# maxsonate/video-diffusion-nnx

Hardware: AMD Instinct MI355X
Metric: denoised frames/sec, 16fx64x64 1000-step DDPM (higher is better)
Workload: dtype bf16; 1 GPU; config_v2_2 (north-star shape): Unet3D dim=64 C=1, 16f x 64x64, DDPM T=1000 p_sample_loop (UNet forward + p_sample per step, hipGraph replay); value = n_gpus*B*F/(T*s_per_step); batch_per_gpu=64, parallelism=dp1 (independent samples, no collective), mfma_operands=bf16, storage=weights fp32 master, activations bf16, fp32 accumulate, process_group=none (single process)

## Files before the change

include/vdx.h:

```cpp
#ifndef VDX_H_
#define VDX_H_

#include <stddef.h>
#include <stdint.h>

#ifdef __cplusplus
extern "C" {
#endif

typedef enum {
    VDX_OK = 0,
    VDX_ERR_INVALID = -1,
    VDX_ERR_HIP = -2,
    VDX_ERR_NOMEM = -3,
    VDX_ERR_STATE = -4
} vdx_status;

typedef enum { VDX_MODE_F32 = 0, VDX_MODE_BF16 = 1, VDX_MODE_F16 = 2 } vdx_mode;

const char* vdx_last_error(void);
int vdx_version(void);


size_t vdx_packed_conv_bytes(int mode, int taps, int cin, int cout);
int vdx_pack_conv_weights(int mode, const float* kernel, void* packed, int taps, int cin, int cout, void* stream);

size_t vdx_gn_stats_bytes(int batch, int groups);

typedef struct {
    const float* x0; const float* x1; int c0, c1;
    const void* packed_w;
    const float* bias;
    float* y;
    int cout;
    int batch, frames, h, w;
    int kind;
    int kh, kw, stride;
    const double* in_stats; const float* gamma; const float* beta; int groups;
    const float* scale_shift; int scale_shift_stride;
    double* out_stats; int out_groups;
    int x_bf16;
    int y_bf16;
    const void* res; int res_bf16;
} vdx_conv_desc;

int vdx_conv_forward(int mode, const vdx_conv_desc* d, void* stream);

typedef struct {
    const char* kernel;
    const char* shape;
    double flops, bytes;
} vdx_launch_info;
typedef void (*vdx_launch_hook)(void* user, int phase, const vdx_launch_info* info, void* stream);
void vdx_set_launch_hook(vdx_launch_hook hook, void* user);

int vdx_resblock_tail(const float* y2, const float* r, float* out, const double* stats, const float* gn_gamma,
                      const float* gn_beta, int groups, const float* ln_gamma, const float* ln_beta, int c, int batch,
                      long pix_per_sample, void* stream);

int vdx_resblock_tail_rc_bf16(const void* y2, const void* x0, const void* x1, int c0, int c1, const void* rc_w_packed,
                              const float* rc_bias, void* out, const double* stats, const float* gn_gamma, const float* gn_beta,
                              int groups, const float* ln_gamma, const float* ln_beta, int c, int batch, long pix_per_sample,
                              void* stream);

int vdx_gn_silu_apply_bf16(void* y, const double* stats, const float* gn_gamma, const float* gn_beta, const float* scale_shift,
                           int ss_stride, int groups, int c, int batch, long pix_per_sample, void* stream);

int vdx_init_conv(const float* x, const float* kernel, const float* bias, float* y, int batch, int cin, int frames,
                  int h, int w, int cout, int k, void* stream);

int vdx_final_conv(const float* x, const float* kernel, const float* bias, float* y, long npix, int d, int cout, void* stream);

int vdx_time_mlp(const int* time, const float* w1, const float* b1, const float* w2, const float* b2, int dim,
                 const float* cond, const float* null_cond_emb, const unsigned char* cond_mask, int null_all, int cond_dim,
                 float* temb, int batch, void* stream);

int vdx_attention_forward(int mode, const float* x, float* y, const void* wqkv_packed, const float* bqkv,
                          const void* wo_packed, const float* bo, int batch, int frames, int h, int w, int c, int heads,
                          int temporal, void* stream);
int vdx_attention_forward_ex(int mode, const float* x, float* y, const void* wqkv_packed, const float* bqkv,
                             const void* wo_packed, const float* bo, int batch, int frames, int h, int w, int c, int heads,
                             int temporal, int fp8_core, void* stream);

int vdx_attention_forward_bf16(const void* x_bf16, void* y_bf16, const void* wqkv_packed, const float* bqkv,
                               const void* wo_packed, const float* bo, int batch, int frames, int h, int w, int c, int heads,
                               int temporal, int fp8_core, void* stream);

size_t vdx_sla_workspace_bytes(int mode, int nframes, int npix, int heads);
int vdx_sla_forward(int mode, const float* x, float* y, const void* wq_packed, const void* wk_packed, const void* wv_packed,
                    const void* wo_packed, void* workspace, int batch, int frames, int h, int w, int c, int heads, void* stream);

int vdx_sla_forward_bf16(const void* x_bf16, void* y_bf16, const void* wq_packed, const void* wk_packed, const void* wv_packed,
                         const void* wo_packed, void* workspace, int batch, int frames, int h, int w, int c, int heads, void* stream);


typedef struct {
    int dim;
    int n_mults; int dim_mults[8];
    int channels;
    int out_dim;
    int cond_dim;
    int attn_heads, attn_dim_head;
    int init_dim;
    int init_kernel_size;
    int use_sparse_linear_attn;
    int resnet_groups;
    int image_size, num_frames;
    int mode;
} vdx_config;

typedef struct vdx_handle vdx_handle;

int vdx_create(const vdx_config* cfg, vdx_handle** out);
void vdx_destroy(vdx_handle* h);

int vdx_set_activation_storage(vdx_handle* h, int bf16);
int vdx_get_activation_storage(const vdx_handle* h);

int vdx_set_attention_fp8(vdx_handle* h, int on);
int vdx_get_attention_fp8(const vdx_handle* h);

int vdx_param_count(const vdx_handle* h);
long vdx_param_total(const vdx_handle* h);
int vdx_param_info(const vdx_handle* h, int index, char* name, int name_cap, int* ndim, long shape[6], long* offset);

size_t vdx_packed_bytes(const vdx_handle* h);
int vdx_pack_params(const vdx_handle* h, const float* params, void* packed, void* stream);

size_t vdx_workspace_bytes(const vdx_handle* h, int batch);
int vdx_slot_count(const vdx_handle* h);
int vdx_slot_info(const vdx_handle* h, int index, char* name, int name_cap, long* floats_per_sample, long* float_offset_per_sample);

int vdx_unet_forward(const vdx_handle* h, const float* params, const void* packed, const float* x, const int* time,
                     const float* cond, const unsigned char* cond_mask, int null_all, float* out, void* workspace,
                     size_t workspace_bytes, int batch, void* stream);


int vdx_randn(float* out, long n, uint64_t seed, uint64_t offset, const uint64_t* dev_offset, void* stream);

int vdx_q_sample(const float* x_start, const int* t, const float* noise, float* out, const float* sqrt_ac,
                 const float* sqrt_one_minus_ac, int batch, long per_sample, float pre_scale, float pre_shift, void* stream);

int vdx_p_sample_step(const float* x, const float* eps_hat, float* out, const int* t, const float* tables, int timesteps,
                      const float* noise, uint64_t seed, uint64_t offset, const uint64_t* dev_offset, const float* thres,
                      int clip_denoised, int batch, int channels, long per_sample, void* stream);

int vdx_loss_sum(const float* eps_hat, const float* noise, double* acc, int batch, int channels, long fhw, int l2, void* stream);

int vdx_affine(const float* x, float* y, long n, float a, float b, void* stream);

int vdx_p_sample_loop(vdx_handle* h, const float* params, const void* packed, float* img, float* eps_buf, int* t_dev,
                      uint64_t* step_dev, const float* tables, int timesteps, int nsteps, const float* cond, uint64_t seed,
                      int clip_denoised, void* workspace, size_t workspace_bytes, int batch, int use_graph, void* stream);

int vdx_dynamic_threshold(const float* x, const float* eps_hat, const int* t, const float* tables, int timesteps, float percentile,
                          float* thres_out, int batch, int channels, long per_sample, void* stream);

int vdx_p_sample_loop_dyn(vdx_handle* h, const float* params, const void* packed, float* img, float* eps_buf, int* t_dev,
                          uint64_t* step_dev, const float* tables, int timesteps, int nsteps, const float* cond, uint64_t seed,
                          int clip_denoised, float percentile, float* thres_buf, void* workspace, size_t workspace_bytes, int batch,
                          int use_graph, void* stream);

int vdx_ddim_step(const float* x, const float* eps_hat, float* out, const float* alphas_cumprod, const int* seq,
                  const uint64_t* step_dev, const float* thres, int clip_denoised, int batch, int channels, long per_sample, void* stream);

int vdx_ddim_sample_loop(vdx_handle* h, const float* params, const void* packed, float* img, float* eps_buf, int* t_dev,
                         uint64_t* step_dev, const float* alphas_cumprod, const int* seq, int seq_len, int nsteps, const float* cond,
                         int clip_denoised, void* workspace, size_t workspace_bytes, int batch, int use_graph, void* stream);

int vdx_ddim_sample_loop_dyn(vdx_handle* h, const float* params, const void* packed, float* img, float* eps_buf, int* t_dev,
                             uint64_t* step_dev, const float* alphas_cumprod, const int* seq, int seq_len, int nsteps, const float* cond,
                             int clip_denoised, const float* tables, int timesteps, float percentile, float* thres_buf, void* workspace,
                             size_t workspace_bytes, int batch, int use_graph, void* stream);

#define VDX_DRAW_KNOWN (1ull << 62)
#define VDX_DRAW_RENOISE (1ull << 63)

int vdx_inpaint_init(float* x, const float* known, const unsigned char* mask, const float* mask_tables, int timesteps, int t0,
                     long n, void* stream);

int vdx_p_sample_step_masked(const float* x, const float* eps_hat, float* out, const int* t, const float* tables, int timesteps,
                             const float* known, const unsigned char* mask, const float* mask_tables, int resample_steps,
                             uint64_t seed, uint64_t step, const uint64_t* step_dev, const float* thres, int clip_denoised,
                             int batch, int channels, long per_sample, void* stream);

int vdx_p_sample_loop_masked(vdx_handle* h, const float* params, const void* packed, float* img, float* eps_buf, int* t_dev,
                             uint64_t* step_dev, const float* tables, int timesteps, int nsteps, const float* cond, uint64_t seed,
                             int clip_denoised, float percentile, float* thres_buf, const float* known, const unsigned char* mask,
                             const float* mask_tables, int resample_steps, void* workspace, size_t workspace_bytes, int batch,
                             int use_graph, void* stream);

int vdx_ddim_step_masked(const float* x, const float* eps_hat, float* out, const float* alphas_cumprod, const int* seq,
                         const uint64_t* step_dev, const float* thres, int clip_denoised, const float* known, const unsigned char* mask,
                         const float* mask_tables, int timesteps, uint64_t seed, int batch, int channels, long per_sample, void* stream);

int vdx_ddim_sample_loop_masked(vdx_handle* h, const float* params, const void* packed, float* img, float* eps_buf, int* t_dev,
                                uint64_t* step_dev, const float* alphas_cumprod, const int* seq, int seq_len, int nsteps, const float* cond,
                                int clip_denoised, const float* tables, int timesteps, float percentile, float* thres_buf,
                                const float* known, const unsigned char* mask, const float* mask_tables, uint64_t seed,
                                void* workspace, size_t workspace_bytes, int batch, int use_graph, void* stream);


int vdx_pack_conv_weights_t(int mode, const float* kernel, void* packed, int taps, int cin, int cout, void* stream);

typedef struct {
    const float* x0; const float* x1; int c0, c1;
    const float* dy; int cout;
    float* dw;
    int batch, frames, h, w;
    int kind, kh, kw, stride;
    const double* in_stats; const float* gamma; const float* beta; int groups;
    const float* scale_shift; int scale_shift_stride;
    int bf16_operands;
} vdx_wgrad_desc;

int vdx_conv_backward_weights(const vdx_wgrad_desc* d, void* stream);

size_t vdx_norm_act_backward_scratch_floats(int c, int batch, long pix_per_sample);
int vdx_norm_act_backward(const float* dact, const float* y, float* dy, const double* stats, const float* gamma, const float* beta,
                          int groups, const float* scale_shift, int scale_shift_stride, float* d_gamma, float* d_beta, float* dss,
                          const float* r, const float* ln_gamma, float* dr, float* d_ln_gamma, float* d_ln_beta, float* scratch,
                          int c, int batch, long pix_per_sample, void* stream);

int vdx_attention_core_backward(const float* qkv, const float* d_o, float* o, float* dq, float* dk, float* dv, int batch, int frames,
                                int h, int w, int heads, int temporal, void* stream);
int vdx_attention_core_backward_ex(const float* qkv, const float* d_o, float* o, float* dq, float* dk, float* dv, int batch, int frames,
                                   int h, int w, int heads, int temporal, int bf16_operands, void* stream);

int vdx_temporal_attention_backward_fused(const float* x, const float* dy, const void* packed_wqkv, const float* bqkv, const void* packed_wo_t,
                                          void* o_bf16, void* dqkv_bf16, float* dx, int batch, int frames, int h, int w, void* stream);

size_t vdx_sla_backward_scratch_floats(int nframes, int heads);
int vdx_sla_core_backward(const float* q, const float* k, const float* v, const float* d_out, float* o, float* dq, float* dk, float* dv,
                          float* scratch, int nframes, int npix, int heads, void* stream);
int vdx_sla_core_backward_ex(const float* q, const float* k, const float* v, const float* d_out, float* o, float* dq, float* dk, float* dv,
                             float* scratch, int nframes, int npix, int heads, int bf16_operands, void* stream);

int vdx_colsum(const float* x, float* out, long rows, int c, void* stream);


typedef struct {
    const void* x0; const void* x1; int c0, c1; int x_bf16;
    const void* dy; int cout; int dy_bf16;
    float* dw; float* dw1; float* dw2; int split;
    float* db; float* db1; float* db2;
    int batch, frames, h, w;
    int kind, kh, kw, stride;
// ... 65 lines not shown
```

video_diffusion_nnx_amd/_lib.py:

```python
from __future__ import annotations

import ctypes as C
import os

_HERE = os.path.dirname(os.path.abspath(__file__))
LIB_PATH = os.environ.get('VDX_LIB') or os.path.join(_HERE, 'libvdx.so')

MODE_F32 = 0
MODE_BF16 = 1
MODE_F16 = 2
MODES = {'f32': MODE_F32, 'fp32': MODE_F32, 'float32': MODE_F32, 'bf16': MODE_BF16, 'bfloat16': MODE_BF16,
         'f16': MODE_F16, 'fp16': MODE_F16, 'float16': MODE_F16}
GN_SLOTS = 32


class VdxError(RuntimeError):
    pass


if not os.path.exists(LIB_PATH):
    raise ImportError(
        f'{LIB_PATH} not found: the HIP extension is required (no CPU fallback exists). '
        'Build it with `python -c "import __graft_entry__ as g; g.build()"` or `make -C video_diffusion_nnx_amd/csrc`.')

lib = C.CDLL(LIB_PATH)

c_void_p, c_int, c_size_t, c_float, c_double = C.c_void_p, C.c_int, C.c_size_t, C.c_float, C.c_double


class ConvDesc(C.Structure):
    _fields_ = [
        ('x0', c_void_p), ('x1', c_void_p), ('c0', c_int), ('c1', c_int),
        ('packed_w', c_void_p), ('bias', c_void_p), ('y', c_void_p), ('cout', c_int),
        ('batch', c_int), ('frames', c_int), ('h', c_int), ('w', c_int),
        ('kind', c_int), ('kh', c_int), ('kw', c_int), ('stride', c_int),
        ('in_stats', c_void_p), ('gamma', c_void_p), ('beta', c_void_p), ('groups', c_int),
        ('scale_shift', c_void_p), ('scale_shift_stride', c_int),
        ('out_stats', c_void_p), ('out_groups', c_int),
        ('x_bf16', c_int), ('y_bf16', c_int),
        ('res', c_void_p), ('res_bf16', c_int),
    ]


def _sig(name, restype, argtypes):
    fn = getattr(lib, name)
    fn.restype = restype
    fn.argtypes = argtypes
    return fn


vdx_last_error = _sig('vdx_last_error', C.c_char_p, [])
vdx_version = _sig('vdx_version', c_int, [])
vdx_packed_conv_bytes = _sig('vdx_packed_conv_bytes', c_size_t, [c_int, c_int, c_int, c_int])
vdx_pack_conv_weights = _sig('vdx_pack_conv_weights', c_int, [c_int, c_void_p, c_void_p, c_int, c_int, c_int, c_void_p])
vdx_gn_stats_bytes = _sig('vdx_gn_stats_bytes', c_size_t, [c_int, c_int])
vdx_conv_forward = _sig('vdx_conv_forward', c_int, [c_int, C.POINTER(ConvDesc), c_void_p])


def check(status: int) -> None:
    if status != 0:
        raise VdxError(f'libvdx status {status}: {vdx_last_error().decode()}')


def ptr(t) -> int:
    if t is None:
        return 0
    assert t.is_contiguous(), 'libvdx needs contiguous tensors'
    return t.data_ptr()


def stream_ptr() -> int:
    import torch
    return torch.cuda.current_stream().cuda_stream

c_long = C.c_long
vdx_resblock_tail = _sig('vdx_resblock_tail', c_int, [c_void_p] * 6 + [c_int, c_void_p, c_void_p, c_int, c_int, c_long, c_void_p])
vdx_gn_silu_apply_bf16 = _sig('vdx_gn_silu_apply_bf16', c_int, [c_void_p] * 5 + [c_int, c_int, c_int, c_int, c_long, c_void_p])
vdx_resblock_tail_rc_bf16 = _sig('vdx_resblock_tail_rc_bf16', c_int, [c_void_p] * 3 + [c_int, c_int] + [c_void_p] * 6 + [c_int, c_void_p, c_void_p, c_int, c_int, c_long, c_void_p])
vdx_init_conv = _sig('vdx_init_conv', c_int, [c_void_p] * 4 + [c_int] * 7 + [c_void_p])
vdx_final_conv = _sig('vdx_final_conv', c_int, [c_void_p] * 4 + [c_long, c_int, c_int, c_void_p])
vdx_time_mlp = _sig('vdx_time_mlp', c_int, [c_void_p] * 5 + [c_int, c_void_p, c_void_p, c_void_p, c_int, c_int, c_void_p, c_int, c_void_p])
vdx_attention_forward = _sig('vdx_attention_forward', c_int, [c_int] + [c_void_p] * 6 + [c_int] * 7 + [c_void_p])
vdx_attention_forward_ex = _sig('vdx_attention_forward_ex', c_int, [c_int] + [c_void_p] * 6 + [c_int] * 8 + [c_void_p])
vdx_attention_forward_bf16 = _sig('vdx_attention_forward_bf16', c_int, [c_void_p] * 6 + [c_int] * 8 + [c_void_p])
vdx_sla_forward_bf16 = _sig('vdx_sla_forward_bf16', c_int, [c_void_p] * 7 + [c_int] * 6 + [c_void_p])
vdx_sla_workspace_bytes = _sig('vdx_sla_workspace_bytes', c_size_t, [c_int] * 4)
vdx_sla_forward = _sig('vdx_sla_forward', c_int, [c_int] + [c_void_p] * 7 + [c_int] * 6 + [c_void_p])
```

video_diffusion_nnx_amd/csrc/elementwise.hip:

```cpp
#include "vdx_common.h"
#include <stdlib.h>
#include "vdx_internal.h"

namespace vdx {

template <int VPL>
__global__ __launch_bounds__(256) void resblock_tail_kernel(TailArgs P) {
    __shared__ float coefA[1024], coefD[1024];
    __shared__ float gm[64];
    const int tid = threadIdx.x;
    const int C = P.C;
    const int b = blockIdx.y;
    gn_mean_rstd_wg(P.stats, b, P.groups, (double)P.pix_per_sample * (C / P.groups), gm, tid, 256);
    __syncthreads();
    for (int c = tid; c < C; c += 256) {
        const int g = c / (C / P.groups);
        const float a = gm[2 * g + 1] * P.gn_gamma[c];
        coefA[c] = a;
        coefD[c] = P.gn_beta[c] - gm[2 * g] * a;
    }
    __syncthreads();
    const int LPP = P.lpp;
    const int ppb = 256 / LPP;
    const int sub = tid % LPP, pl = tid / LPP;
    const float invC = 1.0f / (float)C;
    for (long pix = (long)blockIdx.x * ppb + pl; pix < P.pix_per_sample; pix += (long)gridDim.x * ppb) {
        const size_t base = ((size_t)b * P.pix_per_sample + pix) * C;
        float4 r[VPL];
        float s = 0.f, ss = 0.f;
#pragma unroll
        for (int v = 0; v < VPL; ++v) {
            const int c = (v * LPP + sub) * 4;
            r[v] = make_float4(0.f, 0.f, 0.f, 0.f);
            if (c < C) {
                r[v] = load4_f32_or_bf16(P.r, base + c, P.r_bf16);
                s += r[v].x + r[v].y + r[v].z + r[v].w;
                ss += r[v].x * r[v].x + r[v].y * r[v].y + r[v].z * r[v].z + r[v].w * r[v].w;
            }
        }
        for (int o = 1; o < LPP; o <<= 1) { s += __shfl_xor(s, o); ss += __shfl_xor(ss, o); }
        const float mean = s * invC;
        const float var = fmaxf(ss * invC - mean * mean, 0.f);
        const float rstd = rsqrtf(var + NORM_EPS);
#pragma unroll
        for (int v = 0; v < VPL; ++v) {
            const int c = (v * LPP + sub) * 4;
            if (c < C) {
                const float4 y = load4_f32_or_bf16(P.y2, base + c, P.y2_bf16);
                const float4 a = *reinterpret_cast<const float4*>(coefA + c);
                const float4 d = *reinterpret_cast<const float4*>(coefD + c);
                const float4 lg = *reinterpret_cast<const float4*>(P.ln_gamma + c);
                const float4 lb = *reinterpret_cast<const float4*>(P.ln_beta + c);
                float4 o;
                o.x = silu_f(fmaf(y.x, a.x, d.x)) + fmaf((r[v].x - mean) * rstd, lg.x, lb.x);
                o.y = silu_f(fmaf(y.y, a.y, d.y)) + fmaf((r[v].y - mean) * rstd, lg.y, lb.y);
                o.z = silu_f(fmaf(y.z, a.z, d.z)) + fmaf((r[v].z - mean) * rstd, lg.z, lb.z);
                o.w = silu_f(fmaf(y.w, a.w, d.w)) + fmaf((r[v].w - mean) * rstd, lg.w, lb.w);
                store4_f32_or_bf16(P.out, base + c, o, P.out_bf16);
            }
        }
    }
}

__device__ __forceinline__ void unpack8(const uint4& u, float (&f)[8]) {
    f[0] = __uint_as_float(u.x << 16); f[1] = __uint_as_float(u.x & 0xFFFF0000u);
    f[2] = __uint_as_float(u.y << 16); f[3] = __uint_as_float(u.y & 0xFFFF0000u);
    f[4] = __uint_as_float(u.z << 16); f[5] = __uint_as_float(u.z & 0xFFFF0000u);
    f[6] = __uint_as_float(u.w << 16); f[7] = __uint_as_float(u.w & 0xFFFF0000u);
}

template <int VPL>
__global__ __launch_bounds__(256) void resblock_tail16_kernel(TailArgs P) {
    __shared__ float coefA[1024], coefD[1024];
    __shared__ float gm[64];
    const int tid = threadIdx.x;
    const int C = P.C;
    const int b = blockIdx.y;
    gn_mean_rstd_wg(P.stats, b, P.groups, (double)P.pix_per_sample * (C / P.groups), gm, tid, 256);
    __syncthreads();
    for (int c = tid; c < C; c += 256) {
        const int g = c / (C / P.groups);
        const float a = gm[2 * g + 1] * P.gn_gamma[c];
        coefA[c] = a;
        coefD[c] = P.gn_beta[c] - gm[2 * g] * a;
    }
    __syncthreads();
    const int LPP = P.lpp;
    const int ppb = 256 / LPP;
    const int sub = tid % LPP, pl = tid / LPP;
    const float invC = 1.0f / (float)C;
    const char* rb = reinterpret_cast<const char*>(P.r);
    const char* yb = reinterpret_cast<const char*>(P.y2);
    char* ob = reinterpret_cast<char*>(P.out);
    for (long pix = (long)blockIdx.x * ppb + pl; pix < P.pix_per_sample; pix += (long)gridDim.x * ppb) {
        const size_t base = ((size_t)b * P.pix_per_sample + pix) * C;
        float r[VPL][8];
        float s = 0.f, ss = 0.f;
#pragma unroll
        for (int v = 0; v < VPL; ++v) {
            const int c = (v * LPP + sub) * 8;
#pragma unroll
            for (int k = 0; k < 8; ++k) r[v][k] = 0.f;
            if (c < C) {
                unpack8(*reinterpret_cast<const uint4*>(rb + (base + c) * 2), r[v]);
#pragma unroll
                for (int k = 0; k < 8; ++k) { s += r[v][k]; ss += r[v][k] * r[v][k]; }
            }
        }
        for (int o = 1; o < LPP; o <<= 1) { s += __shfl_xor(s, o); ss += __shfl_xor(ss, o); }
        const float mean = s * invC;
        const float var = fmaxf(ss * invC - mean * mean, 0.f);
        const float rstd = rsqrtf(var + NORM_EPS);
#pragma unroll
        for (int v = 0; v < VPL; ++v) {
            const int c = (v * LPP + sub) * 8;
            if (c < C) {
                float y[8], o[8];
                unpack8(*reinterpret_cast<const uint4*>(yb + (base + c) * 2), y);
#pragma unroll
                for (int k = 0; k < 8; ++k)
                    o[k] = silu_f(fmaf(y[k], coefA[c + k], coefD[c + k])) + fmaf((r[v][k] - mean) * rstd, P.ln_gamma[c + k], P.ln_beta[c + k]);
                *reinterpret_cast<uint4*>(ob + (base + c) * 2) =
                    make_uint4(pack_bf16x2(o[0], o[1]), pack_bf16x2(o[2], o[3]), pack_bf16x2(o[4], o[5]), pack_bf16x2(o[6], o[7]));
            }
        }
    }
}

__global__ __launch_bounds__(256) void gn_silu_apply16_kernel(unsigned* __restrict__ y, const double* __restrict__ stats, const float* __restrict__ gamma,
                                                              const float* __restrict__ beta, const float* __restrict__ ss, int ss_stride, int groups,
                                                              int C, long pix_per_sample) {
    __shared__ float coefA[1024], coefD[1024];
    __shared__ float gm[64];
    const int tid = threadIdx.x, b = blockIdx.y;
    gn_mean_rstd_wg(stats, b, groups, (double)pix_per_sample * (C / groups), gm, tid, 256);
    __syncthreads();
    for (int c = tid; c < C; c += 256) {
        const int g = c / (C / groups);
        const float m = gm[2 * g], rs = gm[2 * g + 1];
        const float ga = gamma[c], be = beta[c];
        float sc = 1.f, sh = 0.f;
        if (ss) { sc = ss[(size_t)b * ss_stride + c] + 1.f; sh = ss[(size_t)b * ss_stride + C + c]; }
        coefA[c] = rs * ga * sc;
        coefD[c] = (be - m * rs * ga) * sc + sh;
    }
    __syncthreads();
    const int octs = C >> 3;
    const long n = pix_per_sample * octs;
    uint4* base = reinterpret_cast<uint4*>(y) + (size_t)b * n;
    for (long i0 = (long)blockIdx.x * 1024 + tid; i0 < n; i0 += (long)gridDim.x * 1024) {
        uint4 v[4];
#pragma unroll
        for (int u = 0; u < 4; ++u) v[u] = (i0 + u * 256 < n) ? base[i0 + u * 256] : make_uint4(0u, 0u, 0u, 0u);
#pragma unroll
        for (int u = 0; u < 4; ++u) {
            if (i0 + u * 256 >= n) continue;
            const int c = (int)((i0 + u * 256) % octs) * 8;
            float f[8], o[8];
            unpack8(v[u], f);
#pragma unroll
            for (int k = 0; k < 8; ++k) o[k] = silu_f(fmaf(f[k], coefA[c + k], coefD[c + k]));
            base[i0 + u * 256] = make_uint4(pack_bf16x2(o[0], o[1]), pack_bf16x2(o[2], o[3]), pack_bf16x2(o[4], o[5]), pack_bf16x2(o[6], o[7]));
        }
    }
}

hipError_t launch_gn_silu_apply16(float* y_bf16, const double* stats, const float* gamma, const float* beta, const float* ss, int ss_stride, int groups,
                                  int C, int batch, long pix_per_sample, hipStream_t st) {
    if (C % 8 || C > 1024 || groups <= 0 || groups > 32 || C % groups) return hipErrorInvalidValue;
    const long n = pix_per_sample * (C / 8);
    const int gx = (int)std::max<long>(1, std::min<long>((n + 1023) / 1024, 2048));
    LaunchScope ls(st, "gn_silu_apply16_kernel", 8.0 * batch * pix_per_sample * C, 4.0 * batch * pix_per_sample * C, "C%d px%ld x %d", C, pix_per_sample, batch);
    hipLaunchKernelGGL(gn_silu_apply16_kernel, dim3(gx, batch), dim3(256), 0, st, reinterpret_cast<unsigned*>(y_bf16), stats, gamma, beta, ss, ss_stride, groups, C, pix_per_sample);
    return hipGetLastError();
}

typedef unsigned tu32x4 __attribute__((ext_vector_type(4)));

template <int CIN, int COUT, bool CAT, bool FIN = false>
__global__ __launch_bounds__(256, (CIN == 128 && COUT == 64) ? 4 : (COUT <= 128 ? 3 : 2)) void resblock_tail_rc16_kernel(TailArgs P) {
    using M = Mma<MODE_BF16>;
    constexpr int NTM = COUT / 16, NKS = CIN / 32, NH = COUT / 32;
    constexpr int C0 = CAT ? CIN / 2 : CIN, NK0 = C0 / 32;
    constexpr int WRS = CIN * 2 + 16;
    extern __shared__ __attribute__((aligned(16))) char smem[];
    char* Wl = smem;
    float* coefA = reinterpret_cast<float*>(Wl + COUT * WRS);
    float* coefD = coefA + COUT;
    float* lng = coefD + COUT;
    float* lnb = lng + COUT;
    float* rcb = lnb + COUT;
    float* gm = rcb + COUT;
    float* finw = gm + 64;
    const int tid = threadIdx.x, lane = tid & 63, wave = tid >> 6, lp = lane & 15, q = lane >> 4;
    const int b = blockIdx.y;
    for (int i = tid; i < COUT * (CIN / 8); i += 256) {
        const int row = i / (CIN / 8), c = i % (CIN / 8);
        const int tm = row >> 4, rr = row & 15;
        const int co = (tm >> 1) * 32 + (rr >> 2) * 8 + (tm & 1) * 4 + (rr & 3);
        *reinterpret_cast<uint4*>(Wl + row * WRS + c * 16) =
            *reinterpret_cast<const uint4*>(reinterpret_cast<const char*>(P.rc_w) + ((size_t)co * ((CIN + 63) / 64 * 64) + c * 8) * 2);
    }
    gn_mean_rstd_wg(P.stats, b, P.groups, (double)P.pix_per_sample * (COUT / P.groups), gm, tid, 256);
    __syncthreads();
    for (int c = tid; c < COUT; c += 256) {
        const int g = c / (COUT / P.groups);
        const float a = gm[2 * g + 1] * P.gn_gamma[c];
        coefA[c] = a;
        coefD[c] = P.gn_beta[c] - gm[2 * g] * a;
        lng[c] = P.ln_gamma[c]; lnb[c] = P.ln_beta[c]; rcb[c] = P.rc_b[c];
        if (FIN) finw[c] = P.fin_w[c];
    }
    __syncthreads();

    const unsigned pps = (unsigned)P.pix_per_sample;
    const char* x0p = reinterpret_cast<const char*>(P.x0) + (size_t)b * pps * C0 * 2;
    const char* x1p = CAT ? reinterpret_cast<const char*>(P.x1) + (size_t)b * pps * C0 * 2 : x0p;
    const char* y2p = reinterpret_cast<const char*>(P.y2) + (size_t)b * pps * COUT * 2;
    char* outp = FIN ? const_cast<char*>(y2p) : reinterpret_cast<char*>(P.out) + (size_t)b * pps * COUT * 2;
    float* const finp = FIN ? P.fin_out + (size_t)b * pps : nullptr;
    const float finb = FIN ? P.fin_b[0] : 0.f;
    const __amdgpu_buffer_rsrc_t rx0 = __builtin_amdgcn_make_buffer_rsrc(const_cast<char*>(x0p), 0, pps * C0 * 2, 0x00020000);
// ... 571 lines not shown
```

video_diffusion_nnx_amd/csrc/model.hip:

```cpp
#include <math.h>
#include <stdio.h>
#include <string.h>
#include <string>
#include <vector>

#include "vdx_common.h"
#include "vdx_internal.h"
#include "model.h"
#include <stdlib.h>

namespace vdx {

static long add_param(Model* m, const std::string& name, std::initializer_list<long> shape) {
    ParamInfo p;
    p.name = name;
    p.ndim = (int)shape.size();
    long n = 1;
    int i = 0;
    for (long s : shape) { p.shape[i++] = s; n *= s; }
    p.offset = m->param_total;
    p.numel = n;
    m->param_total += (n + 3) / 4 * 4;
    m->params.push_back(p);
    return p.offset;
// ... 163 lines not shown
            L.pk_rs = add_packed(m, conv_packed_bytes(m->mode, 16, dims[i + 1], dims[i + 1]));
            L.pt_rs = add_packed_t(m, conv_packed_bytes(m->mode, 16, dims[i + 1], dims[i + 1]));
        }
    }
    const int mid = dims[nl];
    m->mid1 = make_res(m, "mid_block1", mid, mid, true);
    m->mid_sattn = make_attn(m, "mid_spatial_attn", mid);
    m->mid_tattn = make_attn(m, "mid_temporal_attn", mid);
    m->mid2 = make_res(m, "mid_block2", mid, mid, true);
    for (int i = 0; i < nl; ++i) {
        Level& L = m->ups[i];
        const std::string pre = "ups." + std::to_string(i);
        const int din = dims[nl - 1 - i], dout = dims[nl - i];
        L.cin = 2 * dout; L.cout = din;
        L.res0 = make_res(m, pre + ".0", 2 * dout, din, true);
        L.res1 = make_res(m, pre + ".1", din, din, true);
        L.has_sla = c.use_sparse_linear_attn != 0;
        if (L.has_sla) L.sla = make_sla(m, pre + ".2", din);
        L.attn = make_attn(m, pre + ".3", din);
        L.has_resample = i < nl - 1;
        if (L.has_resample) {
            L.rs_w = add_param(m, pre + ".4.kernel", {1, 4, 4, din, din});
            L.rs_b = add_param(m, pre + ".4.bias", {din});
            L.pk_rs = add_packed(m, conv_packed_bytes(m->mode, 16, din, din));
            L.pt_rs = add_packed_t(m, conv_packed_bytes(m->mode, 16, din, din));
        }
    }
    m->fin = make_res(m, "final_conv.layers.0", 2 * c.dim, c.dim, false);
    m->fin_w = add_param(m, "final_conv.layers.1.kernel", {1, c.dim, m->out_dim});
    m->fin_b = add_param(m, "final_conv.layers.1.bias", {m->out_dim});
    if (m->init_dim != c.dim) return vdx_set_error(VDX_ERR_INVALID, "config: init_dim must equal dim (the final concat feeds ResnetBlock(2*dim))", __FILE__, __LINE__);

    const long F = c.num_frames;
    auto pixels = [&](int lvl) { const long s = c.image_size >> lvl; return F * s * s; };
    m->s_init = add_slot(m, "init_conv", pixels(0) * m->init_dim);
    m->s_init_attn = add_slot(m, "init_temporal_attn", pixels(0) * m->init_dim);
    for (int i = 0; i < nl; ++i) {
        Level& L = m->downs[i];
        L.lvl = i;
        res_slots(m, L.res0, pixels(i));
        res_slots(m, L.res1, pixels(i));
        L.s_sla = L.has_sla ? add_slot(m, "downs." + std::to_string(i) + ".2", pixels(i) * L.cout) : -1;
        L.s_attn = add_slot(m, "downs." + std::to_string(i) + ".3", pixels(i) * L.cout);
        L.s_rs = L.has_resample ? add_slot(m, "downs." + std::to_string(i) + ".4", pixels(i + 1) * L.cout) : -1;
    }
    res_slots(m, m->mid1, pixels(nl - 1));
    m->s_mid_sattn = add_slot(m, "mid_spatial_attn", pixels(nl - 1) * mid);
    m->s_mid_tattn = add_slot(m, "mid_temporal_attn", pixels(nl - 1) * mid);
    res_slots(m, m->mid2, pixels(nl - 1));
    for (int i = 0; i < nl; ++i) {
        Level& L = m->ups[i];
        L.lvl = nl - 1 - i;
        res_slots(m, L.res0, pixels(L.lvl));
        res_slots(m, L.res1, pixels(L.lvl));
        L.s_sla = L.has_sla ? add_slot(m, "ups." + std::to_string(i) + ".2", pixels(L.lvl) * L.cout) : -1;
        L.s_attn = add_slot(m, "ups." + std::to_string(i) + ".3", pixels(L.lvl) * L.cout);
        L.s_rs = L.has_resample ? add_slot(m, "ups." + std::to_string(i) + ".4", pixels(L.lvl - 1) * L.cout) : -1;
    }
    res_slots(m, m->fin, pixels(0));
    m->sla_ws_bytes_per_sample = 0;
    for (int l = 0; l < nl; ++l) {
        const long s = c.image_size >> l;
        if (c.use_sparse_linear_attn)
            m->sla_ws_bytes_per_sample = std::max(m->sla_ws_bytes_per_sample, sla_workspace_bytes(m->mode, (int)F, (int)(s * s), H));
        if (c.dim * c.dim_mults[l] >= 256)
            m->sla_ws_bytes_per_sample = std::max(m->sla_ws_bytes_per_sample, (size_t)F * s * s * c.attn_heads * 32 * 2);
    }
    {
        const long s = c.image_size >> (nl - 1);
        if (s * s > 64) m->sla_ws_bytes_per_sample = std::max(m->sla_ws_bytes_per_sample, (size_t)F * s * s * c.attn_heads * 32 * 4 * 4);
    }
    return VDX_OK;
}

size_t model_workspace_bytes(const Model* m, int B) {
    size_t b = 0;
    b += ((size_t)m->act_floats_per_sample * B * 4 + 255) / 256 * 256;
    b += ((size_t)m->temb_dim * B * 4 + 255) / 256 * 256;
    b += 2 * (((size_t)m->ss_floats_per_sample * B * 4 + 255) / 256 * 256);
    b += ((size_t)m->n_stats * B * GN_SLOTS * m->cfg.resnet_groups * 2 * 8 + 255) / 256 * 256;
    b += (m->sla_ws_bytes_per_sample * B + 255) / 256 * 256;
    return b;
}


void model_build_pack_tables(Model* m) {
    const int HD = m->cfg.attn_heads * 32;
    auto pad = [&](int k) { return conv_cin_pad(m->mode, k); };
    auto fwd = [&](long src, size_t dst, int taps, int cin, int cout) {
        PackJob j{}; j.src = src; j.dst = (long)dst; j.taps = taps; j.Cin = cin; j.Cout = cout; j.Pad = pad(cin); j.kind = 0;
        j.n = (long)taps * cout * j.Pad; m->pack_jobs.push_back(j);
    };
    auto cpy = [&](long src, size_t dst, long n) { PackJob j{}; j.src = src; j.dst = (long)dst; j.n = n; j.kind = 2; j.Pad = 1; m->pack_jobs.push_back(j); };
    auto bwd = [&](long src, size_t dst, int taps, int cin, int cout) {
        PackJob j{}; j.src = src; j.dst = (long)dst; j.taps = taps; j.Cin = cin; j.Cout = cout; j.Pad = pad(cout); j.kind = 1;
        j.n = (long)taps * cin * j.Pad; m->pack_t_jobs.push_back(j);
    };
    auto cat3 = [&](const long (&w)[3], size_t dst, int c) {
        PackJob j{}; j.src = w[0]; j.src1 = w[1]; j.src2 = w[2]; j.dst = (long)dst; j.taps = 1; j.Cin = c; j.Cout = HD; j.Pad = pad(3 * HD); j.kind = 3;
        j.n = (long)c * j.Pad; m->pack_t_jobs.push_back(j);
    };
    auto res = [&](const ResP& r) {
        fwd(r.b1_w, r.pk_b1, 9, r.cin, r.cout); fwd(r.b2_w, r.pk_b2, 9, r.cout, r.cout);
        bwd(r.b1_w, r.pt_b1, 9, r.cin, r.cout); bwd(r.b2_w, r.pt_b2, 9, r.cout, r.cout);
        if (r.has_res) { fwd(r.rc_w, r.pk_rc, 1, r.cin, r.cout); bwd(r.rc_w, r.pt_rc, 1, r.cin, r.cout); }
    };
    auto attn = [&](const AttnP& a) {
        const size_t one = conv_packed_bytes(m->mode, 1, a.C, HD);
        for (int i = 0; i < 3; ++i) {
            fwd(a.w[i], a.pk_qkv + i * one, 1, a.C, HD);
            cpy(a.b[i], a.pk_bqkv + (size_t)i * HD * 4, HD);
            bwd(a.w[i], a.pt_w[i], 1, a.C, HD);
        }
        fwd(a.o_w, a.pk_o, 1, HD, a.C); bwd(a.o_w, a.pt_o, 1, HD, a.C);
        cat3(a.w, a.pt_qkv, a.C);
    };
    auto sla = [&](const SlaP& s) {
        for (int i = 0; i < 3; ++i) { fwd(s.w[i], s.pk[i], 1, s.C, HD); bwd(s.w[i], s.pt_w[i], 1, s.C, HD); }
        fwd(s.o_w, s.pk_o, 1, HD, s.C); bwd(s.o_w, s.pt_o, 1, HD, s.C);
        cat3(s.w, s.pt_qkv, s.C);
    };
    m->pack_jobs.clear(); m->pack_t_jobs.clear();
    attn(m->init_attn);
    for (int pass = 0; pass < 2; ++pass) {
        const std::vector<Level>& lv = pass ? m->ups : m->downs;
        for (const Level& L : lv) {
            res(L.res0); res(L.res1);
            if (L.has_sla) sla(L.sla);
            attn(L.attn);
            if (L.has_resample) { fwd(L.rs_w, L.pk_rs, 16, L.cout, L.cout); bwd(L.rs_w, L.pt_rs, 16, L.cout, L.cout); }
        }
    }
    res(m->mid1); attn(m->mid_sattn); attn(m->mid_tattn); res(m->mid2); res(m->fin);
}

hipError_t model_pack(const Model* m, const float* p, void* packed, hipStream_t st) {
    if (!m->d_pack_jobs) return hipErrorInvalidValue;
    return launch_pack_jobs(m->mode, p, packed, m->d_pack_jobs, (int)m->pack_jobs.size(), st);
}


struct Fwd {
    const Model* m; const float* p; const char* pk; int B; hipStream_t st;
    int a16;
    float* act; float* temb; float* ss; float* ss_lin; double* stats; char* sla_ws;
    float* slot(int s) const { return act + (size_t)m->slots[s].offset_per_sample * B; }
    double* stat(int i) const { return stats + (size_t)i * B * GN_SLOTS * m->cfg.resnet_groups * 2; }
};

#ifndef VDX_PREPASS_MIN_C
#define VDX_PREPASS_MIN_C 256
#endif

static hipError_t run_res(const Fwd& f, const ResP& r, const float* x0, int c0, const float* x1, int c1, int lvl, float* head_out = nullptr, bool* head_done = nullptr) {
    const Model* m = f.m;
    const int G = m->cfg.resnet_groups;
    const int S = m->cfg.image_size >> lvl;
    ConvArgs a;
    memset(&a, 0, sizeof(a));
    a.x0 = x0; a.x1 = x1; a.C0 = c0; a.C1 = c1;
    a.wp = f.pk + r.pk_b1; a.bias = f.p + r.b1_b; a.y = f.slot(r.s_y1); a.Cout = r.cout;
    a.NF = f.B * m->cfg.num_frames; a.F = m->cfg.num_frames; a.H = S; a.W = S;
    a.kind = 0; a.kh = a.kw = 3; a.stride = 1; a.pad = 1;
    a.out_stats = f.stat(r.st1); a.out_groups = G;
    const int half = (m->mode == MODE_BF16);
    a.y_bf16 = half; a.x0_bf16 = f.a16; a.x1_bf16 = f.a16;
    hipError_t e = launch_conv(m->mode, a, f.st);
    if (e != hipSuccess) return e;
    ConvArgs b;
    memset(&b, 0, sizeof(b));
    b.x0 = f.slot(r.s_y1); b.C0 = r.cout;
    b.wp = f.pk + r.pk_b2; b.bias = f.p + r.b2_b; b.y = f.slot(r.s_y2); b.Cout = r.cout;
    b.NF = a.NF; b.F = a.F; b.H = S; b.W = S; b.kind = 0; b.kh = b.kw = 3; b.stride = 1; b.pad = 1;
    b.x0_bf16 = half; b.y_bf16 = half;
    b.pro = 1; b.in_stats = f.stat(r.st1); b.gamma = f.p + r.b1_gs; b.beta = f.p + r.b1_gb; b.groups = G;
    if (r.has_mlp) { b.ss = f.ss + (size_t)m->ss_layers[r.ss_index].out_off * f.B; b.ss_stride = 2 * r.cout; }
    b.out_stats = f.stat(r.st2); b.out_groups = G;
    if (half && m->act16 == 1 && r.cout >= VDX_PREPASS_MIN_C) {
        e = launch_gn_silu_apply16(f.slot(r.s_y1), b.in_stats, b.gamma, b.beta, b.ss, b.ss_stride, G, r.cout, f.B, (long)m->cfg.num_frames * S * S, f.st);
        if (e != hipSuccess) return e;
        b.pro = 0; b.in_stats = nullptr; b.gamma = b.beta = nullptr; b.ss = nullptr; b.groups = 0;
    }
    e = launch_conv(m->mode, b, f.st);
    if (e != hipSuccess) return e;
    const float* rsrc = x0;
    const bool fuse_rc = r.has_res && f.a16 && m->act16 == 1 && m->mode == MODE_BF16 &&
                         tail_rc16_supported(c0 + c1, c0, r.cout, (long)m->cfg.num_frames * S * S);
    if (r.has_res && !fuse_rc) {
        ConvArgs c;
        memset(&c, 0, sizeof(c));
        c.x0 = x0; c.x1 = x1; c.C0 = c0; c.C1 = c1;
        c.wp = f.pk + r.pk_rc; c.bias = f.p + r.rc_b; c.y = f.slot(r.s_rc); c.Cout = r.cout;
        c.NF = a.NF; c.F = a.F; c.H = S; c.W = S; c.kind = 0; c.kh = c.kw = 1; c.stride = 1; c.pad = 0;
        c.x0_bf16 = f.a16; c.x1_bf16 = f.a16; c.y_bf16 = f.a16;
        e = launch_conv(m->mode, c, f.st);
        if (e != hipSuccess) return e;
        rsrc = f.slot(r.s_rc);
    }
    TailArgs t;
    memset(&t, 0, sizeof(t));
    t.y2 = f.slot(r.s_y2); t.y2_bf16 = half; t.r = rsrc; t.out = f.slot(r.s_out); t.r_bf16 = f.a16; t.out_bf16 = f.a16;
    t.stats = f.stat(r.st2); t.gn_gamma = f.p + r.b2_gs; t.gn_beta = f.p + r.b2_gb; t.groups = G;
    t.ln_gamma = f.p + r.n2_s; t.ln_beta = f.p + r.n2_b;
    t.C = r.cout; t.batch = f.B; t.pix_per_sample = (long)m->cfg.num_frames * S * S;
    if (fuse_rc) { t.x0 = x0; t.x1 = x1; t.C0 = c0; t.C1 = c1; t.rc_w = f.pk + r.pk_rc; t.rc_b = f.p + r.rc_b; }
    if (head_out && fuse_rc && c1 == c0 && m->out_dim == 1 && ((c0 + c1 == 128 && r.cout == 64) || (c0 + c1 == 64 && r.cout == 32))) {
        t.fin_w = f.p + m->fin_w; t.fin_b = f.p + m->fin_b; t.fin_out = head_out;
        *head_done = true;
    }
    return launch_resblock_tail(t, f.st);
}

static hipError_t run_attn(const Fwd& f, const AttnP& ap, const float* x, float* y, int lvl, bool temporal) {
    const Model* m = f.m;
    const long S = m->cfg.image_size >> lvl, hw = S * S, Fr = m->cfg.num_frames;
    AttnArgs a;
    memset(&a, 0, sizeof(a));
    a.x = x; a.y = y; a.wqkv = f.pk + ap.pk_qkv; a.bqkv = reinterpret_cast<const float*>(f.pk + ap.pk_bqkv);
    a.wo = f.pk + ap.pk_o; a.bo = f.p + ap.o_b; a.C = ap.C; a.heads = m->cfg.attn_heads;
    a.scale = 1.0f / sqrtf((float)m->cfg.attn_dim_head);
    if (temporal) { a.L = (int)Fr; a.nseq = f.B * hw; a.inner = hw; a.inner_stride = ap.C; a.outer_stride = Fr * hw * ap.C; a.tok_stride = hw * ap.C; }
    else { a.L = (int)hw; a.nseq = f.B * Fr; a.inner = 1; a.inner_stride = 0; a.outer_stride = hw * ap.C; a.tok_stride = ap.C; }
    a.io_bf16 = f.a16;
    a.fp8_core = (m->attn_fp8 && m->mode == MODE_BF16) ? 1 : 0;
    if (a.L > 64) {
        if (temporal) return hipErrorInvalidValue;
        const int HD = a.heads * 32;
        float* qkv = reinterpret_cast<float*>(f.sla_ws);
        float* o = qkv + (size_t)f.B * Fr * hw * 3 * HD;
        ConvArgs p;
        memset(&p, 0, sizeof(p));
        p.x0 = x; p.C0 = ap.C; p.x0_bf16 = f.a16; p.wp = f.pk + ap.pk_qkv; p.bias = reinterpret_cast<const float*>(f.pk + ap.pk_bqkv);
        p.y = qkv; p.Cout = 3 * HD;
        p.NF = f.B * (int)Fr; p.F = (int)Fr; p.H = (int)S; p.W = (int)S; p.kind = 0; p.kh = p.kw = 1; p.stride = 1; p.pad = 0;
        hipError_t e = launch_conv(m->mode, p, f.st);
        if (e != hipSuccess) return e;
        e = launch_attention_long_core(qkv, o, a.nseq, a.L, a.heads, a.scale, f.st);
        if (e != hipSuccess) return e;
        ConvArgs c;
        memset(&c, 0, sizeof(c));
        c.x0 = o; c.C0 = HD; c.wp = f.pk + ap.pk_o; c.bias = f.p + ap.o_b; c.y = y; c.Cout = ap.C; c.y_bf16 = f.a16;
        c.res = x; c.res_bf16 = f.a16;
        c.NF = f.B * (int)Fr; c.F = (int)Fr; c.H = (int)S; c.W = (int)S; c.kind = 0; c.kh = c.kw = 1; c.stride = 1; c.pad = 0;
        return launch_conv(m->mode, c, f.st);
    }
    if (m->mode == MODE_BF16 && (temporal ? a.L <= 16 : a.L <= 64) && a.heads == 8 && ap.C >= 256 && ap.C % 128 == 0 &&
        (size_t)96 * (ap.C * 2 + 32) <= 160 * 1024 && (size_t)Fr * S * S * a.heads * 64 <= m->sla_ws_bytes_per_sample) {
        a.oscratch = f.sla_ws;
        hipError_t e = launch_attention_heads(a, f.st);
        if (e != hipSuccess) return e;
        ConvArgs c;
        memset(&c, 0, sizeof(c));
        c.x0 = reinterpret_cast<const float*>(f.sla_ws); c.C0 = a.heads * 32; c.x0_bf16 = 1;
        c.wp = f.pk + ap.pk_o; c.bias = f.p + ap.o_b; c.y = y; c.Cout = ap.C; c.y_bf16 = f.a16;
        c.res = x; c.res_bf16 = f.a16;
        c.NF = f.B * (int)Fr; c.F = (int)Fr; c.H = (int)S; c.W = (int)S; c.kind = 0; c.kh = c.kw = 1; c.stride = 1; c.pad = 0;
        return launch_conv(m->mode, c, f.st);
    }
    return launch_attention(m->mode, a, f.st);
}

static hipError_t run_sla(const Fwd& f, const SlaP& sp, const float* x, float* y, int lvl) {
    const Model* m = f.m;
    const int S = m->cfg.image_size >> lvl;
    SlaArgs a;
    memset(&a, 0, sizeof(a));
    a.x = x; a.y = y; a.wq = f.pk + sp.pk[0]; a.wk = f.pk + sp.pk[1]; a.wv = f.pk + sp.pk[2]; a.wo = f.pk + sp.pk_o;
    a.workspace = f.sla_ws; a.C = sp.C; a.heads = m->cfg.attn_heads; a.NF = f.B * m->cfg.num_frames; a.N = S * S;
    a.io_bf16 = f.a16;
    if (m->mode == MODE_BF16 && a.heads == 8 && sp.C >= 256 && sp.C % 128 == 0 && a.N % 16 == 0 &&
        (size_t)96 * (sp.C * 2 + 32) <= 160 * 1024 && (size_t)m->cfg.num_frames * a.N * a.heads * 64 <= m->sla_ws_bytes_per_sample) {
        hipError_t e = launch_sla_heads(a, f.sla_ws, f.st);
        if (e != hipSuccess) return e;
        ConvArgs c;
        memset(&c, 0, sizeof(c));
        c.x0 = reinterpret_cast<const float*>(f.sla_ws); c.C0 = a.heads * 32; c.x0_bf16 = 1;
        c.wp = f.pk + sp.pk_o; c.y = y; c.Cout = sp.C; c.y_bf16 = f.a16;
        c.res = x; c.res_bf16 = f.a16;
        c.NF = a.NF; c.F = m->cfg.num_frames; c.H = S; c.W = S; c.kind = 0; c.kh = c.kw = 1; c.stride = 1; c.pad = 0;
        return launch_conv(m->mode, c, f.st);
    }
    return launch_sla(m->mode, a, f.st);
}

static hipError_t run_resample(const Fwd& f, const Level& L, const float* x, float* y, int lvl_in, bool up) {
    const Model* m = f.m;
    const int S = m->cfg.image_size >> lvl_in;
    ConvArgs a;
    memset(&a, 0, sizeof(a));
    a.x0 = x; a.C0 = L.cout; a.wp = f.pk + L.pk_rs; a.bias = f.p + L.rs_b; a.y = y; a.Cout = L.cout;
    a.NF = f.B * m->cfg.num_frames; a.F = m->cfg.num_frames; a.H = S; a.W = S;
    if (up) { a.kind = 1; a.kh = a.kw = 4; a.stride = 1; a.pad = 0; }
    else { a.kind = 0; a.kh = a.kw = 4; a.stride = 2; a.pad = 1; }
    a.x0_bf16 = f.a16; a.y_bf16 = f.a16;
    return launch_conv(m->mode, a, f.st);
}

int model_forward(const Model* m, const float* params, const void* packed, const float* x, const int* time,
                  const float* cond, const unsigned char* cond_mask, int null_all, float* out, void* workspace,
                  size_t workspace_bytes, int B, hipStream_t st) {
    if (B < 1) return vdx_set_error(VDX_ERR_INVALID, "forward: batch < 1", __FILE__, __LINE__);
    if (workspace_bytes < model_workspace_bytes(m, B)) return vdx_set_error(VDX_ERR_NOMEM, "forward: workspace too small", __FILE__, __LINE__);
    if (m->cfg.cond_dim && !cond) return vdx_set_error(VDX_ERR_INVALID, "cond must be passed in if cond_dim specified", __FILE__, __LINE__);
    const vdx_config& c = m->cfg;
    Fwd f;
    f.m = m; f.p = params; f.pk = reinterpret_cast<const char*>(packed); f.B = B; f.st = st;
    f.a16 = (m->act16 && m->mode == MODE_BF16) ? 1 : 0;
    char* w = reinterpret_cast<char*>(workspace);
    f.act = reinterpret_cast<float*>(w); w += ((size_t)m->act_floats_per_sample * B * 4 + 255) / 256 * 256;
    f.temb = reinterpret_cast<float*>(w); w += ((size_t)m->temb_dim * B * 4 + 255) / 256 * 256;
    f.ss = reinterpret_cast<float*>(w); w += ((size_t)m->ss_floats_per_sample * B * 4 + 255) / 256 * 256;
    f.ss_lin = reinterpret_cast<float*>(w); w += ((size_t)m->ss_floats_per_sample * B * 4 + 255) / 256 * 256;
    f.stats = reinterpret_cast<double*>(w);
    const size_t stats_bytes = (size_t)m->n_stats * B * GN_SLOTS * c.resnet_groups * 2 * 8;
    w += (stats_bytes + 255) / 256 * 256;
    f.sla_ws = w;
    hipError_t e;
#define VDX_E(x) do { e = (x); if (e != hipSuccess) return vdx_set_error(VDX_ERR_HIP, hipGetErrorString(e), __FILE__, __LINE__); } while (0)
    {
        LaunchScope ls(st, "fillBufferAligned", 0.0, (double)stats_bytes, "GroupNorm statistics slabs %zu B", stats_bytes);
        VDX_E(hipMemsetAsync(f.stats, 0, stats_bytes, st));
    }
    const int S0 = c.image_size, Fr = c.num_frames;
    {
        TimeMlpArgs t;
        memset(&t, 0, sizeof(t));
        t.time = time; t.w1 = params + m->t_w1; t.b1 = params + m->t_b1; t.w2 = params + m->t_w2; t.b2 = params + m->t_b2;
        t.dim = c.dim; t.time_dim = m->time_dim; t.cond = cond; t.null_cond_emb = c.cond_dim ? params + m->null_cond : nullptr;
        t.cond_mask = cond_mask; t.null_all = null_all; t.cond_dim = c.cond_dim; t.temb = f.temb; t.temb_dim = m->temb_dim;
        VDX_E(launch_time_mlp(t, B, st));
        int max_n = 0;
        for (const SsLayer& l : m->ss_layers) max_n = std::max(max_n, l.n);
        VDX_E(launch_resblock_ss(params, f.temb, m->d_ss_layers, (int)m->ss_layers.size(), f.ss, f.ss_lin, m->temb_dim, B, max_n, st));
    }
    VDX_E(launch_init_conv_mode(m->mode, x, params + m->init_w, params + m->init_b, f.slot(m->s_init), B, c.channels, Fr, S0, S0, m->init_dim, c.init_kernel_size, f.a16, st));
    VDX_E(run_attn(f, m->init_attn, f.slot(m->s_init), f.slot(m->s_init_attn), 0, true));
    const float* cur = f.slot(m->s_init_attn);
    int cur_c = m->init_dim;
    const int nl = c.n_mults;
    for (int i = 0; i < nl; ++i) {
        const Level& L = m->downs[i];
        VDX_E(run_res(f, L.res0, cur, cur_c, nullptr, 0, i));
        VDX_E(run_res(f, L.res1, f.slot(L.res0.s_out), L.cout, nullptr, 0, i));
        cur = f.slot(L.res1.s_out);
        if (L.has_sla) { VDX_E(run_sla(f, L.sla, cur, f.slot(L.s_sla), i)); cur = f.slot(L.s_sla); }
        VDX_E(run_attn(f, L.attn, cur, f.slot(L.s_attn), i, true));
        cur = f.slot(L.s_attn); cur_c = L.cout;
        if (L.has_resample) { VDX_E(run_resample(f, L, cur, f.slot(L.s_rs), i, false)); cur = f.slot(L.s_rs); }
    }
    VDX_E(run_res(f, m->mid1, cur, cur_c, nullptr, 0, nl - 1));
    VDX_E(run_attn(f, m->mid_sattn, f.slot(m->mid1.s_out), f.slot(m->s_mid_sattn), nl - 1, false));
    VDX_E(run_attn(f, m->mid_tattn, f.slot(m->s_mid_sattn), f.slot(m->s_mid_tattn), nl - 1, true));
    VDX_E(run_res(f, m->mid2, f.slot(m->s_mid_tattn), cur_c, nullptr, 0, nl - 1));
    cur = f.slot(m->mid2.s_out);
    for (int i = 0; i < nl; ++i) {
        const Level& L = m->ups[i];
        const Level& D = m->downs[nl - 1 - i];
        VDX_E(run_res(f, L.res0, cur, cur_c, f.slot(D.s_attn), D.cout, L.lvl));
        VDX_E(run_res(f, L.res1, f.slot(L.res0.s_out), L.cout, nullptr, 0, L.lvl));
        cur = f.slot(L.res1.s_out);
        if (L.has_sla) { VDX_E(run_sla(f, L.sla, cur, f.slot(L.s_sla), L.lvl)); cur = f.slot(L.s_sla); }
        VDX_E(run_attn(f, L.attn, cur, f.slot(L.s_attn), L.lvl, true));
        cur = f.slot(L.s_attn); cur_c = L.cout;
        if (L.has_resample) { VDX_E(run_resample(f, L, cur, f.slot(L.s_rs), L.lvl, true)); cur = f.slot(L.s_rs); }
    }
    bool head_done = false;
    VDX_E(run_res(f, m->fin, cur, cur_c, f.slot(m->s_init_attn), m->init_dim, 0, out, &head_done));
    if (!head_done) VDX_E(launch_final_conv(f.slot(m->fin.s_out), params + m->fin_w, params + m->fin_b, out, (long)B * Fr * S0 * S0, c.dim, m->out_dim, f.a16, st));
#undef VDX_E
    return VDX_OK;
}

}
```

video_diffusion_nnx_amd/csrc/sla.hip:

```cpp
#include "vdx_common.h"
#include "vdx_internal.h"
#include <stdlib.h>

namespace vdx {

constexpr int SLA_PART = 32 * 32 + 64;

template <int MODE>
__global__ __launch_bounds__(256) void sla_ctx_kernel(const SlaArgs P) {
    using M = Mma<MODE>;
    constexpr int KT = M::KT, KC = M::KC, RS = ROW_STRIDE;
    constexpr int APIECES = KT / 4;
    constexpr int NCHN = 64 / KC;
    constexpr int RSE = NCHN * 64 + 16;

    extern __shared__ __attribute__((aligned(16))) char smem[];
    float* m_run = reinterpret_cast<float*>(smem);
    float* s_run = m_run + 32;
    float* alpha = s_run + 32;
    float* pm = alpha + 32;
    char* xs = smem + 1024;
    char* ws = xs + 64 * RS;
    char* eT = ws + 64 * RS;
    char* vT = eT + 32 * RSE;

    const int tid = threadIdx.x, lane = tid & 63, w = tid >> 6;
    const int lp = lane & 15, q = lane >> 4;
    const int wc = w & 1, wr = w >> 1;
    const int gsz = 8 * P.heads;
    const int grp = blockIdx.x / gsz, j = blockIdx.x % gsz;
    const int h = j >> 3;
    const int cidx = grp * 8 + (j & 7);
    if (cidx >= P.NF * P.nchunk) return;
    const int n = cidx / P.nchunk, chunk = cidx % P.nchunk;
    const int R = P.nsub * 64;
    const size_t xbase = (size_t)n * P.N * P.C;
    const int nkt = P.CPad / KT;
    const char* wk = reinterpret_cast<const char*>(P.wk);
    const char* wv = reinterpret_cast<const char*>(P.wv);

    if (tid < 32) { m_run[tid] = -1e30f; s_run[tid] = 0.f; }
    f32x4 cacc = f32x4{0.f, 0.f, 0.f, 0.f};
    const int dt = w >> 1, et = w & 1;

    const bool w_resident = (nkt == 1);
    auto stage_w = [&](int kt) {
        for (int i = tid; i < 64 * 8; i += 256) {
            const int row = i >> 3, pc = i & 7;
            const char* src = (row < 32 ? wk : wv) + ((size_t)(h * 32 + (row & 31)) * P.CPad + (size_t)kt * KT) * M::ES + pc * 16;
            *reinterpret_cast<uint4*>(ws + row * RS + pc * 16) = *reinterpret_cast<const uint4*>(src);
        }
    };
    constexpr int XP = 64 * APIECES / 256;
    float4 xpre[XP];
    auto xfetch = [&](int r0, int kt) {
#pragma unroll
        for (int u = 0; u < XP; ++u) {
            const int i = tid + 256 * u;
            const int row = i / APIECES, pc = i % APIECES;
            const int c = kt * KT + pc * 4;
            xpre[u] = make_float4(0.f, 0.f, 0.f, 0.f);
            if (r0 + row < P.N && c < P.C) xpre[u] = load4_f32_or_bf16(P.x, xbase + (size_t)(r0 + row) * P.C + c, P.io_bf16);
        }
    };
    auto xput = [&]() {
#pragma unroll
        for (int u = 0; u < XP; ++u) {
            const int i = tid + 256 * u;
            M::store4(xs + (i / APIECES) * RS, (i % APIECES) * 4, xpre[u]);
        }
    };
    if (w_resident) stage_w(0);
    xfetch(chunk * R, 0);

    for (int sub = 0; sub < P.nsub; ++sub) {
        const int r0 = chunk * R + sub * 64;
        if (r0 >= P.N) break;
        f32x4 acc[2][2];
#pragma unroll
        for (int i = 0; i < 2; ++i) { acc[i][0] = f32x4{0.f, 0.f, 0.f, 0.f}; acc[i][1] = f32x4{0.f, 0.f, 0.f, 0.f}; }
        for (int kt = 0; kt < nkt; ++kt) {
            __syncthreads();
            xput();
            if (!w_resident) stage_w(kt);
            __syncthreads();
            {
                int nk = kt + 1, nr0 = r0;
                if (nk == nkt) { nk = 0; nr0 = r0 + 64; }
                if (nr0 < P.N && nr0 < (chunk + 1) * R) xfetch(nr0, nk);
            }
#pragma unroll
            for (int ch = 0; ch < 2; ++ch) {
                uint4 bf[2], af[2];
#pragma unroll
                for (int tn = 0; tn < 2; ++tn) bf[tn] = *reinterpret_cast<const uint4*>(xs + ((wr * 2 + tn) * 16 + lp) * RS + ch * 64 + q * 16);
#pragma unroll
                for (int tm = 0; tm < 2; ++tm) af[tm] = *reinterpret_cast<const uint4*>(ws + ((wc * 2 + tm) * 16 + lp) * RS + ch * 64 + q * 16);
#pragma unroll
                for (int tm = 0; tm < 2; ++tm)
#pragma unroll
                    for (int tn = 0; tn < 2; ++tn) M::mma(acc[tm][tn], af[tm], bf[tn]);
            }
        }
        bool rv[2];
#pragma unroll
        for (int tn = 0; tn < 2; ++tn) rv[tn] = (r0 + (wr * 2 + tn) * 16 + lp) < P.N;
        if (wc == 0) {
#pragma unroll
            for (int tm = 0; tm < 2; ++tm)
#pragma unroll
                for (int r = 0; r < 4; ++r) {
                    float mx = fmaxf(rv[0] ? acc[tm][0][r] : -1e30f, rv[1] ? acc[tm][1][r] : -1e30f);
                    mx = max16(mx);
                    if (lp == 0) pm[wr * 32 + tm * 16 + 4 * q + r] = mx;
                }
        }
        __syncthreads();
        if (tid < 32) {
            const float mc = fmaxf(pm[tid], pm[32 + tid]);
            const float mo = m_run[tid];
            const float mn = fmaxf(mo, mc);
            alpha[tid] = __expf(mo - mn);
            m_run[tid] = mn;
        }
        __syncthreads();
        if (wc == 0) {
#pragma unroll
            for (int tm = 0; tm < 2; ++tm)
#pragma unroll
                for (int r = 0; r < 4; ++r) {
                    const int d = tm * 16 + 4 * q + r;
                    const float mn = m_run[d];
                    float ssum = 0.f;
#pragma unroll
                    for (int tn = 0; tn < 2; ++tn) {
                        const float e = rv[tn] ? __expf(acc[tm][tn][r] - mn) : 0.f;
                        M::store1(eT + d * RSE, (wr * 2 + tn) * 16 + lp, e);
                        ssum += e;
                    }
                    ssum = reduce16(ssum);
                    if (lp == 0) pm[wr * 32 + d] = ssum;
                }
        } else {
#pragma unroll
            for (int tm = 0; tm < 2; ++tm)
#pragma unroll
                for (int r = 0; r < 4; ++r) {
                    const int e = tm * 16 + 4 * q + r;
#pragma unroll
                    for (int tn = 0; tn < 2; ++tn)
                        M::store1(vT + e * RSE, (wr * 2 + tn) * 16 + lp, rv[tn] ? acc[tm][tn][r] : 0.f);
                }
        }
        __syncthreads();
// ... 45 lines not shown
    }
}

template <int MODE, int TMO>
__global__ __launch_bounds__(256) void sla_out_kernel(const SlaArgs P) {
    using M = Mma<MODE>;
    constexpr int KT = M::KT, KC = M::KC, RS = ROW_STRIDE;
    constexpr int APIECES = KT / 4;
    constexpr int NCHD = 32 / KC;
    constexpr int RSQ = (MODE == MODE_F32) ? 160 : 80;
    constexpr int HD = 256;
    constexpr int RSO = HD * M::ES + 16;
    constexpr int NCHO = HD / KC;

    extern __shared__ __attribute__((aligned(16))) char smem[];
    char* xs = smem;
    char* ws = xs + 64 * RS;
    char* qb = smem;
    char* os = qb + 4 * 64 * RSQ;

    const int tid = threadIdx.x, lane = tid & 63, w = tid >> 6;
    const int lp = lane & 15, q = lane >> 4;
    const int tiles = (P.N + 63) / 64;
    const int n = blockIdx.x / tiles, r0 = (blockIdx.x % tiles) * 64;
    const size_t xbase = (size_t)n * P.N * P.C;
    const int nkt = P.CPad / KT;
    const char* wq = reinterpret_cast<const char*>(P.wq);
    const char* wo = reinterpret_cast<const char*>(P.wo);

    f32x4 acc[4][4];
#pragma unroll
    for (int i = 0; i < 4; ++i)
#pragma unroll
        for (int j = 0; j < 4; ++j) acc[i][j] = f32x4{0.f, 0.f, 0.f, 0.f};
    for (int kt = 0; kt < nkt; ++kt) {
        __syncthreads();
        for (int i = tid; i < 64 * APIECES; i += 256) {
            const int row = i / APIECES, pc = i % APIECES;
            const int c = kt * KT + pc * 4;
            float4 v = make_float4(0.f, 0.f, 0.f, 0.f);
            if (r0 + row < P.N && c < P.C) v = load4_f32_or_bf16(P.x, xbase + (size_t)(r0 + row) * P.C + c, P.io_bf16);
            M::store4(xs + row * RS, pc * 4, v);
        }
        for (int i = tid; i < 256 * 8; i += 256) {
            const int row = i >> 3, pc = i & 7;
            *reinterpret_cast<uint4*>(ws + row * RS + pc * 16) =
                *reinterpret_cast<const uint4*>(wq + ((size_t)row * P.CPad + (size_t)kt * KT) * M::ES + pc * 16);
        }
        __syncthreads();
#pragma unroll
        for (int ch = 0; ch < 2; ++ch) {
            uint4 bf[4], af[4];
#pragma unroll
            for (int tn = 0; tn < 4; ++tn) bf[tn] = *reinterpret_cast<const uint4*>(xs + (tn * 16 + lp) * RS + ch * 64 + q * 16);
#pragma unroll
            for (int tm = 0; tm < 4; ++tm) af[tm] = *reinterpret_cast<const uint4*>(ws + ((w * 4 + tm) * 16 + lp) * RS + ch * 64 + q * 16);
#pragma unroll
            for (int tm = 0; tm < 4; ++tm)
#pragma unroll
                for (int tn = 0; tn < 4; ++tn) M::mma(acc[tm][tn], af[tm], bf[tn]);
        }
    }
    __syncthreads();
    char* myq = qb + w * 64 * RSQ;
#pragma unroll
    for (int hh = 0; hh < 2; ++hh) {
        const int h = 2 * w + hh;
#pragma unroll
        for (int tn = 0; tn < 4; ++tn) {
            float mx = -1e30f;
#pragma unroll
            for (int t2 = 0; t2 < 2; ++t2)
#pragma unroll
                for (int r = 0; r < 4; ++r) mx = fmaxf(mx, acc[2 * hh + t2][tn][r]);
            mx = max_q(mx);
            float e[2][4], sum = 0.f;
#pragma unroll
            for (int t2 = 0; t2 < 2; ++t2)
#pragma unroll
                for (int r = 0; r < 4; ++r) { e[t2][r] = __expf(acc[2 * hh + t2][tn][r] - mx); sum += e[t2][r]; }
            sum = reduce_q(sum);
            const float inv = 1.0f / sum;
#pragma unroll
            for (int t2 = 0; t2 < 2; ++t2)
                M::store4(myq + (tn * 16 + lp) * RSQ, t2 * 16 + 4 * q, make_float4(e[t2][0] * inv, e[t2][1] * inv, e[t2][2] * inv, e[t2][3] * inv));
        }
        __syncthreads();
        const char* ct = reinterpret_cast<const char*>(P.ctxT) + (size_t)(n * P.heads + h) * 32 * 32 * M::ES;
#pragma unroll
        for (int et = 0; et < 2; ++et) {
            f32x4 o[4];
#pragma unroll
            for (int tn = 0; tn < 4; ++tn) o[tn] = f32x4{0.f, 0.f, 0.f, 0.f};
#pragma unroll
            for (int ch = 0; ch < NCHD; ++ch) {
                const uint4 a = *reinterpret_cast<const uint4*>(ct + (size_t)(et * 16 + lp) * 32 * M::ES + ch * 64 + q * 16);
#pragma unroll
                for (int tn = 0; tn < 4; ++tn) {
                    const uint4 bq = *reinterpret_cast<const uint4*>(myq + (tn * 16 + lp) * RSQ + ch * 64 + q * 16);
                    M::mma(o[tn], a, bq);
                }
            }
#pragma unroll
            for (int tn = 0; tn < 4; ++tn)
                M::store4(os + (tn * 16 + lp) * RSO, h * 32 + et * 16 + 4 * q, make_float4(o[tn][0], o[tn][1], o[tn][2], o[tn][3]));
        }
        __syncthreads();
    }
    f32x4 oacc[TMO][4];
#pragma unroll
    for (int i = 0; i < TMO; ++i)
#pragma unroll
        for (int j = 0; j < 4; ++j) oacc[i][j] = f32x4{0.f, 0.f, 0.f, 0.f};
    for (int ch = 0; ch < NCHO; ++ch) {
        uint4 bf[4];
#pragma unroll
        for (int tn = 0; tn < 4; ++tn) bf[tn] = *reinterpret_cast<const uint4*>(os + (tn * 16 + lp) * RSO + ch * 64 + q * 16);
#pragma unroll
        for (int tmo = 0; tmo < TMO; ++tmo) {
            const int co = (w * TMO + tmo) * 16 + lp;
            uint4 a = make_uint4(0, 0, 0, 0);
            if (co < P.C) a = *reinterpret_cast<const uint4*>(wo + (size_t)co * HD * M::ES + ch * 64 + q * 16);
#pragma unroll
            for (int tn = 0; tn < 4; ++tn) M::mma(oacc[tmo][tn], a, bf[tn]);
        }
    }
#pragma unroll
    for (int tmo = 0; tmo < TMO; ++tmo) {
        const int co = (w * TMO + tmo) * 16 + 4 * q;
        if (co >= P.C) continue;
#pragma unroll
        for (int tn = 0; tn < 4; ++tn) {
            const int row = r0 + tn * 16 + lp;
            if (row >= P.N) continue;
            const float4 xr = load4_f32_or_bf16(P.x, xbase + (size_t)row * P.C + co, P.io_bf16);
            float4 v;
            v.x = oacc[tmo][tn][0] + xr.x; v.y = oacc[tmo][tn][1] + xr.y;
            v.z = oacc[tmo][tn][2] + xr.z; v.w = oacc[tmo][tn][3] + xr.w;
            store4_f32_or_bf16(P.y, xbase + (size_t)row * P.C + co, v, P.io_bf16);
        }
    }
}


template <int MODE, int NKT, bool IO16>
struct SlaTile {
    using M = Mma<MODE>;
    static_assert(!IO16 || MODE == MODE_BF16, "bf16 activation storage implies bf16 MFMA operands");
    static constexpr int PCH = IO16 ? 8 : 4;
    static constexpr int APIECES = M::KT / PCH;
    static constexpr int XP = 64 * APIECES * NKT / 512;
    static constexpr int PLANE = 64 * ROW_STRIDE;
    static constexpr int BUF = NKT * PLANE;
    float4 xpre[XP];
    __device__ __forceinline__ void fetch(const float* x, size_t xbase, int io_bf16, int r0, int N, int C, int tid) {
#pragma unroll
        for (int u = 0; u < XP; ++u) {
            const int i = tid + 512 * u;
            const int kt = i / (64 * APIECES), rem = i % (64 * APIECES);
            const int row = rem / APIECES, c = kt * M::KT + (rem % APIECES) * PCH;
            xpre[u] = make_float4(0.f, 0.f, 0.f, 0.f);
            if (r0 + row < N && c < C) {
                if (IO16) xpre[u] = *reinterpret_cast<const float4*>(reinterpret_cast<const char*>(x) + (xbase + (size_t)(r0 + row) * C + c) * 2);
                else xpre[u] = load4_f32_or_bf16(x, xbase + (size_t)(r0 + row) * C + c, io_bf16);
            }
        }
    }
    __device__ __forceinline__ void put(char* xs, int tid) const {
#pragma unroll
        for (int u = 0; u < XP; ++u) {
            const int i = tid + 512 * u;
            const int kt = i / (64 * APIECES), rem = i % (64 * APIECES);
            char* dst = xs + kt * PLANE + (rem / APIECES) * ROW_STRIDE;
            if (IO16) *reinterpret_cast<float4*>(dst + (rem % APIECES) * 16) = xpre[u];
            else M::store4(dst, (rem % APIECES) * 4, xpre[u]);
        }
    }
};

template <bool FULL>
__device__ __forceinline__ void ctx8_softmax_step(f32x4 (&acc)[2][4], float (&m_run)[2], float (&s_run)[2], f32x4 (&cacc)[2][2], int nleft) {
    constexpr float L2E = 1.44269504088896f;
#pragma unroll
    for (int dt = 0; dt < 2; ++dt) {
        if (!FULL) {
#pragma unroll
            for (int tn = 0; tn < 2; ++tn)
#pragma unroll
                for (int r = 0; r < 4; ++r) if (tn * 16 + r >= nleft) acc[tn][dt][r] = -1e30f;
        }
        float mx = fmaxf(fmaxf(fmaxf(acc[0][dt][0], acc[0][dt][1]), fmaxf(acc[0][dt][2], acc[0][dt][3])),
                         fmaxf(fmaxf(acc[1][dt][0], acc[1][dt][1]), fmaxf(acc[1][dt][2], acc[1][dt][3])));
        mx = max_q(mx);
        const float mn = fmaxf(m_run[dt], mx);
        const float alpha = __builtin_amdgcn_exp2f((m_run[dt] - mn) * L2E);
        m_run[dt] = mn;
        const float nb = -mn * L2E;
        float ssum = 0.f;
#pragma unroll
        for (int tn = 0; tn < 2; ++tn)
#pragma unroll
            for (int r = 0; r < 4; ++r) {
                float e = __builtin_amdgcn_exp2f(__builtin_fmaf(acc[tn][dt][r], L2E, nb));
                if (!FULL) e = (tn * 16 + r >= nleft) ? 0.f : e;
                acc[tn][dt][r] = e;
                ssum += e;
            }
        s_run[dt] = s_run[dt] * alpha + reduce_q(ssum);
#pragma unroll
        for (int et = 0; et < 2; ++et)
#pragma unroll
            for (int r = 0; r < 4; ++r) cacc[et][dt][r] *= alpha;
    }
}

template <int MODE, int NKT, bool IO16>
__global__ __launch_bounds__(512) void sla_ctx8_kernel(const SlaArgs P) {
    using M = Mma<MODE>;
    using T = SlaTile<MODE, NKT, IO16>;
    constexpr int RS = ROW_STRIDE;
    extern __shared__ __attribute__((aligned(16))) char smem[];
    const int tid = threadIdx.x, lane = tid & 63, h = tid >> 6;
    const int lp = lane & 15, q = lane >> 4;
    const int n = blockIdx.x / P.nchunk, chunk = blockIdx.x % P.nchunk;
    const int R = P.nsub * 64;
    const size_t xbase = (size_t)n * P.N * P.C;

    uint4 wf[NKT][2][4];
#pragma unroll
    for (int kt = 0; kt < NKT; ++kt)
#pragma unroll
        for (int ch = 0; ch < 2; ++ch)
#pragma unroll
            for (int tm = 0; tm < 4; ++tm) {
                const char* base = reinterpret_cast<const char*>(tm < 2 ? P.wk : P.wv);
                wf[kt][ch][tm] = *reinterpret_cast<const uint4*>(base + ((size_t)(h * 32 + (tm & 1) * 16 + lp) * P.CPad + kt * M::KT) * M::ES + ch * 64 + q * 16);
            }
    float m_run[2] = {-1e30f, -1e30f}, s_run[2] = {0.f, 0.f};
    f32x4 cacc[2][2];
#pragma unroll
    for (int i = 0; i < 2; ++i) { cacc[i][0] = f32x4{0.f, 0.f, 0.f, 0.f}; cacc[i][1] = f32x4{0.f, 0.f, 0.f, 0.f}; }

    T t;
    t.fetch(P.x, xbase, P.io_bf16, chunk * R, P.N, P.C, tid);
    t.put(smem, tid);
    __syncthreads();
    for (int sub = 0; sub < P.nsub; ++sub) {
        const int r0 = chunk * R + sub * 64;
        if (r0 >= P.N) break;
        const char* xs = smem + (sub & 1) * T::BUF;
        const bool more = (sub + 1 < P.nsub) && (r0 + 64 < P.N);
        if (more) t.fetch(P.x, xbase, P.io_bf16, r0 + 64, P.N, P.C, tid);
#pragma unroll
        for (int hf = 0; hf < 2; ++hf) {
            f32x4 acc[2][4];
#pragma unroll
            for (int i = 0; i < 2; ++i)
#pragma unroll
                for (int j = 0; j < 4; ++j) acc[i][j] = f32x4{0.f, 0.f, 0.f, 0.f};
#pragma unroll
            for (int kt = 0; kt < NKT; ++kt)
#pragma unroll
                for (int ch = 0; ch < 2; ++ch) {
                    uint4 xa[2];
#pragma unroll
                    for (int tn = 0; tn < 2; ++tn)
                        xa[tn] = *reinterpret_cast<const uint4*>(xs + kt * T::PLANE + ((hf * 2 + tn) * 16 + lp) * RS + ch * 64 + q * 16);
#pragma unroll
                    for (int tn = 0; tn < 2; ++tn)
#pragma unroll
                        for (int tm = 0; tm < 4; ++tm) M::mma(acc[tn][tm], xa[tn], wf[kt][ch][tm]);
                }
            if (r0 + 64 <= P.N) ctx8_softmax_step<true>(acc, m_run, s_run, cacc, 0);
            else ctx8_softmax_step<false>(acc, m_run, s_run, cacc, P.N - (r0 + hf * 32 + 4 * q));
#pragma unroll
            for (int tn = 0; tn < 2; ++tn)
#pragma unroll
                for (int et = 0; et < 2; ++et)
#pragma unroll
                    for (int dt = 0; dt < 2; ++dt) M::mma16(cacc[et][dt], acc[tn][2 + et], acc[tn][dt]);
        }
        if (more) t.put(smem + ((sub + 1) & 1) * T::BUF, tid);
        __syncthreads();
    }
    if (P.nchunk == 1) {
        char* ct = reinterpret_cast<char*>(P.ctxT) + (size_t)(n * P.heads + h) * 32 * 32 * M::ES;
#pragma unroll
        for (int dt = 0; dt < 2; ++dt) {
            const float inv = 1.0f / s_run[dt];
#pragma unroll
            for (int et = 0; et < 2; ++et)
#pragma unroll
                for (int r = 0; r < 4; ++r) M::store1(ct + (size_t)(et * 16 + 4 * q + r) * 32 * M::ES, dt * 16 + lp, cacc[et][dt][r] * inv);
        }
        return;
    }
    float* part = P.part + ((size_t)(n * P.nchunk + chunk) * P.heads + h) * SLA_PART;
#pragma unroll
    for (int et = 0; et < 2; ++et)
#pragma unroll
        for (int dt = 0; dt < 2; ++dt)
            *reinterpret_cast<float4*>(part + (dt * 16 + lp) * 32 + et * 16 + 4 * q) =
                make_float4(cacc[et][dt][0], cacc[et][dt][1], cacc[et][dt][2], cacc[et][dt][3]);
    if (q == 0) {
#pragma unroll
        for (int dt = 0; dt < 2; ++dt) { part[1024 + dt * 16 + lp] = m_run[dt]; part[1056 + dt * 16 + lp] = s_run[dt]; }
    }
}

template <int MODE, int NKT, int TMO, int TNO, bool IO16>
__global__ __launch_bounds__(512, NKT == 1 ? 4 : 2) void sla_out8_kernel(const SlaArgs P) {
    using M = Mma<MODE>;
    using T = SlaTile<MODE, NKT, IO16>;
    constexpr int RS = ROW_STRIDE, KC = M::KC, HD = 256;
    constexpr int RSO = HD * M::ES + 16;
    constexpr int NCHO = HD / KC;
    constexpr bool WO_RES = (TMO * NCHO <= 16);

    extern __shared__ __attribute__((aligned(16))) char smem[];
    char* os = smem + 2 * T::BUF;
    constexpr int RSY = NKT * M::KT * 4 + 16;
    char* ys = os + 64 * RSO;
    const int tid = threadIdx.x, lane = tid & 63, h = tid >> 6;
    const int lp = lane & 15, q = lane >> 4;
    const int n = blockIdx.x / P.nchunk, chunk = blockIdx.x % P.nchunk;
    const int R = P.nsub * 64;
    const size_t xbase = (size_t)n * P.N * P.C;

    uint4 wqf[NKT][2][2];
#pragma unroll
    for (int kt = 0; kt < NKT; ++kt)
#pragma unroll
        for (int ch = 0; ch < 2; ++ch)
#pragma unroll
            for (int tm = 0; tm < 2; ++tm)
                wqf[kt][ch][tm] = *reinterpret_cast<const uint4*>(reinterpret_cast<const char*>(P.wq) +
                    ((size_t)(h * 32 + tm * 16 + lp) * P.CPad + kt * M::KT) * M::ES + ch * 64 + q * 16);
    f32x4 cf[2][2];
    {
        const char* ct = reinterpret_cast<const char*>(P.ctxT) + (size_t)(n * P.heads + h) * 32 * 32 * M::ES;
#pragma unroll
        for (int et = 0; et < 2; ++et)
#pragma unroll
            for (int dt = 0; dt < 2; ++dt) cf[et][dt] = M::load_w4(ct + ((size_t)(et * 16 + lp) * 32 + dt * 16 + 4 * q) * M::ES);
    }
    const int cot0 = (TNO == 4) ? h * TMO : (TNO == 2) ? (h & 3) : (h & 1);
    const int tn0 = (TNO == 4) ? 0 : (TNO == 2) ? 2 * (h >> 2) : (h >> 1);
    const char* wo = reinterpret_cast<const char*>(P.wo);
    uint4 wof[WO_RES ? TMO : 1][WO_RES ? NCHO : 1];
    if (WO_RES) {
#pragma unroll
        for (int tmo = 0; tmo < TMO; ++tmo)
#pragma unroll
            for (int ch = 0; ch < NCHO; ++ch)
                wof[tmo][ch] = *reinterpret_cast<const uint4*>(wo + (size_t)((cot0 + tmo) * 16 + lp) * HD * M::ES + ch * 64 + q * 16);
    }

    T t;
    t.fetch(P.x, xbase, IO16 ? 1 : P.io_bf16, chunk * R, P.N, P.C, tid);
    t.put(smem, tid);
    __syncthreads();
    for (int sub = 0; sub < P.nsub; ++sub) {
        const int r0 = chunk * R + sub * 64;
        if (r0 >= P.N) break;
        const char* xs = smem + (sub & 1) * T::BUF;
        const bool more = (sub + 1 < P.nsub) && (r0 + 64 < P.N);
        float4 xcur[IO16 ? T::XP : 1];
        if (IO16) {
#pragma unroll
            for (int u = 0; u < T::XP; ++u) xcur[u] = t.xpre[u];
        }
        if (more) t.fetch(P.x, xbase, IO16 ? 1 : P.io_bf16, r0 + 64, P.N, P.C, tid);
        f32x4 acc[2][4];
#pragma unroll
        for (int i = 0; i < 2; ++i)
#pragma unroll
            for (int j = 0; j < 4; ++j) acc[i][j] = f32x4{0.f, 0.f, 0.f, 0.f};
#pragma unroll
        for (int kt = 0; kt < NKT; ++kt)
#pragma unroll
            for (int ch = 0; ch < 2; ++ch) {
                uint4 xb[4];
#pragma unroll
                for (int tn = 0; tn < 4; ++tn) xb[tn] = *reinterpret_cast<const uint4*>(xs + kt * T::PLANE + (tn * 16 + lp) * RS + ch * 64 + q * 16);
#pragma unroll
                for (int tm = 0; tm < 2; ++tm)
#pragma unroll
                    for (int tn = 0; tn < 4; ++tn) M::mma(acc[tm][tn], wqf[kt][ch][tm], xb[tn]);
            }
#pragma unroll
        for (int tn = 0; tn < 4; ++tn) {
            float mx = -1e30f;
#pragma unroll
            for (int tm = 0; tm < 2; ++tm)
#pragma unroll
                for (int r = 0; r < 4; ++r) mx = fmaxf(mx, acc[tm][tn][r]);
            mx = max_q(mx);
            const float nmx = -mx * 1.44269504088896f;
            float sum = 0.f;
#pragma unroll
            for (int tm = 0; tm < 2; ++tm)
#pragma unroll
                for (int r = 0; r < 4; ++r) { acc[tm][tn][r] = __builtin_amdgcn_exp2f(fmaf(acc[tm][tn][r], 1.44269504088896f, nmx)); sum += acc[tm][tn][r]; }
            const float inv = __builtin_amdgcn_rcpf(reduce_q(sum));
#pragma unroll
            for (int tm = 0; tm < 2; ++tm)
#pragma unroll
                for (int r = 0; r < 4; ++r) acc[tm][tn][r] *= inv;
        }
#pragma unroll
        for (int tn = 0; tn < 4; ++tn)
#pragma unroll
            for (int et = 0; et < 2; ++et) {
                f32x4 o = f32x4{0.f, 0.f, 0.f, 0.f};
#pragma unroll
                for (int dt = 0; dt < 2; ++dt) M::mma16(o, cf[et][dt], acc[dt][tn]);
                M::store4(os + (tn * 16 + lp) * RSO, h * 32 + et * 16 + 4 * q, make_float4(o[0], o[1], o[2], o[3]));
            }
        __syncthreads();
        f32x4 oacc[TMO][TNO];
#pragma unroll
        for (int i = 0; i < TMO; ++i)
#pragma unroll
            for (int j = 0; j < TNO; ++j) oacc[i][j] = f32x4{0.f, 0.f, 0.f, 0.f};
#pragma unroll
        for (int ch = 0; ch < NCHO; ++ch) {
            uint4 bf[TNO];
#pragma unroll
            for (int tn = 0; tn < TNO; ++tn) bf[tn] = *reinterpret_cast<const uint4*>(os + ((tn0 + tn) * 16 + lp) * RSO + ch * 64 + q * 16);
#pragma unroll
            for (int tmo = 0; tmo < TMO; ++tmo) {
                uint4 a;
                if (WO_RES) a = wof[tmo][ch];
                else a = *reinterpret_cast<const uint4*>(wo + (size_t)((cot0 + tmo) * 16 + lp) * HD * M::ES + ch * 64 + q * 16);
#pragma unroll
                for (int tn = 0; tn < TNO; ++tn) M::mma(oacc[tmo][tn], a, bf[tn]);
            }
        }
        if constexpr (IO16) {
#pragma unroll
            for (int tmo = 0; tmo < TMO; ++tmo)
#pragma unroll
                for (int tn = 0; tn < TNO; ++tn)
                    *reinterpret_cast<f32x4*>(ys + ((tn0 + tn) * 16 + lp) * RSY + ((cot0 + tmo) * 16 + 4 * q) * 4) = oacc[tmo][tn];
            if (more) t.put(smem + ((sub + 1) & 1) * T::BUF, tid);
            __syncthreads();
#pragma unroll
            for (int u = 0; u < T::XP; ++u) {
                const int i = tid + 512 * u;
                const int kt = i / (64 * T::APIECES), rem = i % (64 * T::APIECES);
                const int row = rem / T::APIECES, c = kt * M::KT + (rem % T::APIECES) * 8;
                if (r0 + row >= P.N || c >= P.C) continue;
                const float4 o4 = *reinterpret_cast<const float4*>(ys + row * RSY + c * 4), o5 = *reinterpret_cast<const float4*>(ys + row * RSY + c * 4 + 16);
                const unsigned x0 = __float_as_uint(xcur[u].x), x1 = __float_as_uint(xcur[u].y), x2 = __float_as_uint(xcur[u].z), x3 = __float_as_uint(xcur[u].w);
                uint4 w;
                w.x = pack_bf16x2(o4.x + __uint_as_float(x0 << 16), o4.y + __uint_as_float(x0 & 0xFFFF0000u));
                w.y = pack_bf16x2(o4.z + __uint_as_float(x1 << 16), o4.w + __uint_as_float(x1 & 0xFFFF0000u));
                w.z = pack_bf16x2(o5.x + __uint_as_float(x2 << 16), o5.y + __uint_as_float(x2 & 0xFFFF0000u));
                w.w = pack_bf16x2(o5.z + __uint_as_float(x3 << 16), o5.w + __uint_as_float(x3 & 0xFFFF0000u));
                *reinterpret_cast<uint4*>(reinterpret_cast<char*>(P.y) + (xbase + (size_t)(r0 + row) * P.C + c) * 2) = w;
// ... 270 lines not shown
            }
            if (tok0 > 0) {
#pragma unroll
                for (int dt = 0; dt < 2; ++dt)
#pragma unroll
                    for (int r = 0; r < 4; ++r) {
                        const float a = __builtin_bit_cast(float, __builtin_amdgcn_ds_bpermute((4 * q + r) * 4, __builtin_bit_cast(int, al[dt])));
                        ctx[dt][0][r] *= a; ctx[dt][1][r] *= a;
                    }
            }
#pragma unroll
            for (int tt = 0; tt < TT; ++tt)
#pragma unroll
                for (int dt = 0; dt < 2; ++dt)
#pragma unroll
                    for (int et = 0; et < 2; ++et) M::mma16(ctx[dt][et], ak[tt][dt], av[tt][et]);
        }
#pragma unroll
        for (int dt = 0; dt < 2; ++dt) {
            const float inv = __builtin_amdgcn_rcpf(srun[dt]);
#pragma unroll
            for (int r = 0; r < 4; ++r) {
                const float a = __builtin_bit_cast(float, __builtin_amdgcn_ds_bpermute((4 * q + r) * 4, __builtin_bit_cast(int, inv)));
                ctx[dt][0][r] *= a; ctx[dt][1][r] *= a;
            }
        }
        const size_t obase = ((size_t)n * P.N + lp) * HD + h * D + 4 * q;
        for (int tok0 = 0; tok0 < P.N; tok0 += 16 * TT) {
            f32x4 aq[TT][2];
#pragma unroll
            for (int tt = 0; tt < TT; ++tt) { aq[tt][0] = f32x4{0.f, 0.f, 0.f, 0.f}; aq[tt][1] = f32x4{0.f, 0.f, 0.f, 0.f}; }
            for (int kt = 0; kt < nkt; kt += 4) {
#pragma unroll
                for (int u = 0; u < 4; ++u) {
#pragma unroll
                    for (int t = 0; t < 2; ++t) {
                        const uint4 wq = *reinterpret_cast<const uint4*>(wrow + (t * 16) * RSW + (kt + u) * 64);
#pragma unroll
                        for (int tt = 0; tt < TT; ++tt) M::mma(aq[tt][t], wq, ring[u][tt]);
                    }
                    fetch(ring[u]);
                }
            }
#pragma unroll
            for (int tt = 0; tt < TT; ++tt) {
                float mx = fmaxf(fmaxf(fmaxf(aq[tt][0][0], aq[tt][0][1]), fmaxf(aq[tt][0][2], aq[tt][0][3])),
                                 fmaxf(fmaxf(aq[tt][1][0], aq[tt][1][1]), fmaxf(aq[tt][1][2], aq[tt][1][3])));
                mx = max_q(mx);
                float sum = 0.f;
#pragma unroll
                for (int t = 0; t < 2; ++t)
#pragma unroll
                    for (int r = 0; r < 4; ++r) { aq[tt][t][r] = __builtin_amdgcn_exp2f((aq[tt][t][r] - mx) * L2E); sum += aq[tt][t][r]; }
                const float inv = __builtin_amdgcn_rcpf(reduce_q(sum));
#pragma unroll
                for (int t = 0; t < 2; ++t)
#pragma unroll
                    for (int r = 0; r < 4; ++r) aq[tt][t][r] *= inv;
#pragma unroll
                for (int et = 0; et < 2; ++et) {
                    f32x4 o = f32x4{0.f, 0.f, 0.f, 0.f};
                    M::mma16(o, ctx[0][et], aq[tt][0]);
                    M::mma16(o, ctx[1][et], aq[tt][1]);
                    *reinterpret_cast<uint2*>(reinterpret_cast<char*>(O) + (obase + (size_t)(tok0 + tt * 16) * HD + et * 16) * 2) =
                        make_uint2(pack_bf16x2(o[0], o[1]), pack_bf16x2(o[2], o[3]));
                }
            }
        }
    }
}

namespace {
struct SlaWork { double flops, bytes; };
SlaWork sla_work(const SlaArgs& a, int es_w, bool ctx_half, bool out_half, bool with_out) {
    const double px = (double)a.NF * a.N, eio = a.io_bf16 ? 2.0 : 4.0, ctx_bytes = (double)a.NF * a.heads * 32 * 32 * 4;
    SlaWork w{0.0, 0.0};
    if (ctx_half) { w.flops += px * (2.0 * a.C * 512 + 2.0 * 256 * 32); w.bytes += px * a.C * eio + ctx_bytes + es_w * 512.0 * a.C; }
    if (out_half) {
        w.flops += px * (2.0 * a.C * 256 + 2.0 * 256 * 32 + (with_out ? 2.0 * 256 * a.C : 0.0));
        w.bytes += px * a.C * eio + (with_out ? px * a.C * eio : px * 256 * 2.0) + (ctx_half ? 0.0 : ctx_bytes) + es_w * (256.0 * a.C + (with_out ? 256.0 * a.C : 0.0));
    }
    return w;
}
}

hipError_t launch_sla_heads(SlaArgs a, void* O, hipStream_t st) {
    a.CPad = conv_cin_pad(MODE_BF16, a.C);
    if (a.heads != 8 || a.C % 128 || a.N % 16 || !O) return hipErrorInvalidValue;
    const size_t lds = (size_t)96 * (a.C * 2 + 32);
    if (lds > 160 * 1024) return hipErrorInvalidValue;
    long fpb = (a.NF * (long)a.heads + 255) / 256;
    fpb = std::max<long>(8, (fpb + 7) / 8 * 8);
    const long chunks = (a.NF + fpb - 1) / fpb;
    auto go = [&](auto kfn) -> hipError_t {
        if (hipError_t e = lds_opt_in(kfn, lds); e != hipSuccess) return e;
        const SlaWork sw = sla_work(a, 2, true, true, false);
        LaunchScope ls(st, "sla_head_kernel", sw.flops, sw.bytes, "<io16 %d, %d> C%d N%d NF%d", a.io_bf16, a.N % 64 == 0 ? 4 : 1, a.C, a.N, a.NF);
        hipLaunchKernelGGL(kfn, dim3((unsigned)((chunks + 7) / 8 * 64)), dim3(512), lds, st, a, O, (int)fpb, (int)chunks);
        return hipGetLastError();
    };
    if (a.N % 64 == 0) return a.io_bf16 ? go(sla_head_kernel<true, 4>) : go(sla_head_kernel<false, 4>);
    return a.io_bf16 ? go(sla_head_kernel<true, 1>) : go(sla_head_kernel<false, 1>);
}


void sla_plan(int N, int& nsub, int& nchunk) {
    const int tiles = (N + 63) / 64;
    nsub = std::min(tiles, 8);
    nchunk = (tiles + nsub - 1) / nsub;
}

size_t sla_workspace_bytes(int mode, int NF, int N, int heads) {
    int nsub, nchunk;
    sla_plan(N, nsub, nchunk);
    const size_t part = (size_t)NF * nchunk * heads * SLA_PART * 4;
    const size_t ctx = (size_t)NF * heads * 32 * 32 * (mode == MODE_F32 ? 4 : 2);
    return ((part + 255) / 256) * 256 + ((ctx + 255) / 256) * 256;
}

template <int MODE, int TMO>
static hipError_t launch_sla_out_t(const SlaArgs& a, hipStream_t st) {
    using M = Mma<MODE>;
    constexpr int RSQ = (MODE == MODE_F32) ? 160 : 80;
    constexpr int RSO = 256 * M::ES + 16;
    const size_t lds = std::max<size_t>((size_t)(64 + 256) * ROW_STRIDE, (size_t)4 * 64 * RSQ + (size_t)64 * RSO);
    auto kfn = sla_out_kernel<MODE, TMO>;
    if (hipError_t e = lds_opt_in(kfn, lds); e != hipSuccess) return e;
    const int tiles = (a.N + 63) / 64;
    const SlaWork sw = sla_work(a, M::ES, false, true, true);
    LaunchScope ls(st, "sla_out_kernel", sw.flops, sw.bytes, "<%d, %d> C%d N%d NF%d io16 %d", MODE, TMO, a.C, a.N, a.NF, a.io_bf16);
    hipLaunchKernelGGL(kfn, dim3(a.NF * tiles), dim3(256), lds, st, a);
    return hipGetLastError();
}

#ifndef VDX_SLA_W_MIN_N
#define VDX_SLA_W_MIN_N 2048
#endif
static bool sla_out_w_eligible(const SlaArgs& a) {
    return a.io_bf16 && a.C == 64 && a.CPad == 64 && a.heads == 8 && a.N % 64 == 0 && a.N >= VDX_SLA_W_MIN_N && a.NF >= 128 && (size_t)a.NF * a.N * 128 < (1ull << 40);
}
static hipError_t launch_sla_out_w(const SlaArgs& a, hipStream_t st) {
    const size_t lds = 256 * 128 + 64 * 512 + 2 * 256 * 72;
    auto kfn = sla_out_w_kernel<0>;
    if (hipError_t e = lds_opt_in(kfn, lds); e != hipSuccess) return e;
    const PersistentSplit s = persistent_split(a.NF, device_cus());
    const int fpb = (int)s.per, blocks = (int)s.workers;
    const SlaWork sw = sla_work(a, 2, false, true, true);
    LaunchScope ls(st, "sla_out_w_kernel", sw.flops, sw.bytes, "C%d N%d NF%d", a.C, a.N, a.NF);
    hipLaunchKernelGGL(kfn, dim3(blocks), dim3(512), lds, st, a, fpb);
    return hipGetLastError();
}

template <int MODE, int NKT, int TMO, int TNO, bool IO16>
static hipError_t launch_sla8_t(const SlaArgs& a, hipStream_t st) {
    using M = Mma<MODE>;
    using T = SlaTile<MODE, NKT, IO16>;
    const size_t lds_ctx = 2 * (size_t)T::BUF;
    const size_t lds_out = lds_ctx + (size_t)64 * (256 * M::ES + 16) + (IO16 ? (size_t)64 * (NKT * M::KT * 4 + 16) : 0);
    auto kc = sla_ctx8_kernel<MODE, NKT, IO16>;
    auto ko = sla_out8_kernel<MODE, NKT, TMO, TNO, IO16>;
    hipError_t e;
    if ((e = lds_opt_in(kc, lds_ctx)) != hipSuccess) return e;
    if ((e = lds_opt_in(ko, lds_out)) != hipSuccess) return e;
    {
        const SlaWork sw = sla_work(a, M::ES, true, false, false);
        LaunchScope ls(st, "sla_ctx8_kernel", sw.flops, sw.bytes, "<%d, %d, %d> C%d N%d NF%d nchunk%d", MODE, NKT, (int)IO16, a.C, a.N, a.NF, a.nchunk);
        hipLaunchKernelGGL(kc, dim3(a.NF * a.nchunk), dim3(512), lds_ctx, st, a);
        if ((e = hipGetLastError()) != hipSuccess) return e;
    }
    if (a.nchunk > 1) {
        LaunchScope ls(st, "sla_combine_kernel", 0.0, (double)a.NF * a.nchunk * a.heads * SLA_PART * 4, "<%d> NF%d nchunk%d", MODE, a.NF, a.nchunk);
        hipLaunchKernelGGL(sla_combine_kernel<MODE>, dim3(a.NF * a.heads), dim3(256), 0, st, a.part, a.ctxT, a.nchunk, a.heads);
        if ((e = hipGetLastError()) != hipSuccess) return e;
    }
    if constexpr (MODE == MODE_BF16 && IO16 && NKT == 1 && TNO == 2) {
        if (sla_out_w_eligible(a)) return launch_sla_out_w(a, st);
    }
    const SlaWork sw = sla_work(a, M::ES, false, true, true);
    LaunchScope ls(st, "sla_out8_kernel", sw.flops, sw.bytes, "<%d, %d, %d, %d, %d> C%d N%d NF%d", MODE, NKT, TMO, TNO, (int)IO16, a.C, a.N, a.NF);
    hipLaunchKernelGGL(ko, dim3(a.NF * a.nchunk), dim3(512), lds_out, st, a);
    return hipGetLastError();
}

template <int MODE>
static hipError_t launch_sla_m(SlaArgs a, hipStream_t st) {
    using M = Mma<MODE>;
    constexpr int NCHN = 64 / M::KC;
    constexpr int RSE = NCHN * 64 + 16;
    sla_plan(a.N, a.nsub, a.nchunk);
    {
        const int tiles = (a.N + 63) / 64;
#ifndef VDX_SLA_MIN_WGS
#define VDX_SLA_MIN_WGS 1024
#endif
        const long min_wgs = VDX_SLA_MIN_WGS;
        while (a.nsub * 2 <= tiles && (long)a.NF * ((tiles + 2 * a.nsub - 1) / (2 * a.nsub)) >= min_wgs) a.nsub *= 2;
        a.nchunk = (tiles + a.nsub - 1) / a.nsub;
    }
    const size_t part_bytes = (((size_t)a.NF * a.nchunk * a.heads * SLA_PART * 4) + 255) / 256 * 256;
    a.part = reinterpret_cast<float*>(a.workspace);
    a.ctxT = reinterpret_cast<char*>(a.workspace) + part_bytes;
    const int nkt = a.CPad / M::KT;
    if constexpr (MODE != MODE_F16)
    if (a.heads == 8 && (a.C % 64 == 0 || a.C == 32)) {
        if constexpr (MODE == MODE_BF16) {
            if (a.io_bf16 && a.C == 64) return launch_sla8_t<MODE, 1, 1, 2, true>(a, st);
            if (a.io_bf16 && a.C == 128) return launch_sla8_t<MODE, 2, 1, 4, true>(a, st);
            if (a.io_bf16 && a.C == 32) return launch_sla8_t<MODE, 1, 1, 1, true>(a, st);
        }
        if (nkt == 1 && a.C == 64) return launch_sla8_t<MODE, 1, 1, 2, false>(a, st);
        if (nkt == 2 && a.C == 64) return launch_sla8_t<MODE, 2, 1, 2, false>(a, st);
        if (nkt == 2 && a.C == 128) return launch_sla8_t<MODE, 2, 1, 4, false>(a, st);
    }
    const size_t lds1 = 1024 + (size_t)128 * ROW_STRIDE + (size_t)64 * RSE;
    hipError_t e;
    {
        const SlaWork sw = sla_work(a, M::ES, true, false, false);
        LaunchScope ls(st, "sla_ctx_kernel", sw.flops, sw.bytes, "<%d> C%d N%d NF%d nchunk%d io16 %d", MODE, a.C, a.N, a.NF, a.nchunk, a.io_bf16);
        hipLaunchKernelGGL(sla_ctx_kernel<MODE>, dim3(((a.NF * a.nchunk + 7) / 8) * 8 * a.heads), dim3(256), lds1, st, a);
        if ((e = hipGetLastError()) != hipSuccess) return e;
    }
    {
        LaunchScope ls(st, "sla_combine_kernel", 0.0, (double)a.NF * a.nchunk * a.heads * SLA_PART * 4, "<%d> NF%d nchunk%d", MODE, a.NF, a.nchunk);
        hipLaunchKernelGGL(sla_combine_kernel<MODE>, dim3(a.NF * a.heads), dim3(256), 0, st, a.part, a.ctxT, a.nchunk, a.heads);
        if ((e = hipGetLastError()) != hipSuccess) return e;
    }
    if (a.C <= 64) return launch_sla_out_t<MODE, 1>(a, st);
    if (a.C <= 128) return launch_sla_out_t<MODE, 2>(a, st);
    if (a.C <= 256) return launch_sla_out_t<MODE, 4>(a, st);
    if (a.C <= 512) return launch_sla_out_t<MODE, 8>(a, st);
    if (a.C <= 1024) return launch_sla_out_t<MODE, 16>(a, st);
    return hipErrorInvalidValue;
}

hipError_t launch_sla(int mode, SlaArgs a, hipStream_t st) {
    a.CPad = conv_cin_pad(mode, a.C);
    return mode == MODE_F32 ? launch_sla_m<MODE_F32>(a, st) : mode == MODE_F16 ? launch_sla_m<MODE_F16>(a, st) : launch_sla_m<MODE_BF16>(a, st);
}

}
```

video_diffusion_nnx_amd/csrc/vdx_api.cpp:

```cpp
#include <stdio.h>
#include <string.h>
#include <math.h>
#include "vdx_internal.h"
#include "model.h"
#include "comm.h"

struct vdx_handle {
    vdx::Model model;
    struct GraphKey { const void* p[16]; unsigned long long seed; int i[5]; size_t ws; float f; };
    struct GraphSlot {
        hipGraph_t graph = nullptr; hipGraphExec_t exec = nullptr; GraphKey key; hipStream_t last = nullptr;
        void drop() {
            if (exec && last) (void)hipStreamSynchronize(last);
            if (exec) { (void)hipGraphExecDestroy(exec); exec = nullptr; }
            if (graph) { (void)hipGraphDestroy(graph); graph = nullptr; }
            last = nullptr;
        }
    } gs[4];
    void drop_graphs() { for (GraphSlot& g : gs) g.drop(); }
    vdx::BwdState bwd;
    vdx::Comm comm;
};

namespace vdx {
// ... 107 lines not shown

int vdx_conv_forward(int mode, const vdx_conv_desc* d, void* stream) { return conv_forward_rows(mode, d, 0, 0, stream); }

int vdx_conv_forward_rows(int mode, const vdx_conv_desc* d, int w_rows, int w_row0, void* stream) {
    if (!d) VDX_FAIL(VDX_ERR_INVALID, "conv: null tensor");
    if (w_rows < 1 || w_row0 < 0 || w_row0 + d->cout > w_rows) VDX_FAIL(VDX_ERR_INVALID, "conv_forward_rows: rows [w_row0, w_row0 + cout) must lie inside the w_rows packed rows");
    if (w_rows % 4 || w_row0 % 4) VDX_FAIL(VDX_ERR_INVALID, "conv_forward_rows: w_rows and w_row0 must be multiples of 4");
    return conv_forward_rows(mode, d, w_rows, w_row0, stream);
}

int vdx_resblock_tail(const float* y2, const float* r, float* out, const double* stats, const float* gn_gamma,
                      const float* gn_beta, int groups, const float* ln_gamma, const float* ln_beta, int c, int batch,
                      long pix_per_sample, void* stream) {
    if (!y2 || !r || !out || !stats || !gn_gamma || !gn_beta || !ln_gamma || !ln_beta) VDX_FAIL(VDX_ERR_INVALID, "tail: null tensor");
    if (c % 4 || c > 1024 || groups <= 0 || groups > 32 || c % groups) VDX_FAIL(VDX_ERR_INVALID, "tail: bad channels/groups");
    vdx::TailArgs a;
    memset(&a, 0, sizeof(a));
    a.y2 = y2; a.r = r; a.out = out; a.stats = stats; a.gn_gamma = gn_gamma; a.gn_beta = gn_beta; a.groups = groups;
    a.ln_gamma = ln_gamma; a.ln_beta = ln_beta; a.C = c; a.batch = batch; a.pix_per_sample = pix_per_sample;
    VDX_HIP(vdx::launch_resblock_tail(a, (hipStream_t)stream));
    return VDX_OK;
}

int vdx_resblock_tail_rc_bf16(const void* y2, const void* x0, const void* x1, int c0, int c1, const void* rc_w_packed,
                              const float* rc_bias, void* out, const double* stats, const float* gn_gamma, const float* gn_beta,
                              int groups, const float* ln_gamma, const float* ln_beta, int c, int batch, long pix_per_sample,
                              void* stream) {
    if (!y2 || !x0 || !rc_w_packed || !rc_bias || !out || !stats || !gn_gamma || !gn_beta || !ln_gamma || !ln_beta || (c1 && !x1))
        VDX_FAIL(VDX_ERR_INVALID, "tail_rc: null tensor");
    if (c1 < 0 || batch < 1 || groups <= 0 || groups > 32 || c % groups || !vdx::tail_rc16_supported(c0 + c1, c0, c, pix_per_sample))
        VDX_FAIL(VDX_ERR_INVALID, "tail_rc: shape not served");
    vdx::TailArgs a;
    memset(&a, 0, sizeof(a));
    a.y2 = (const float*)y2; a.y2_bf16 = 1; a.out = (float*)out; a.out_bf16 = 1; a.r_bf16 = 1;
    a.stats = stats; a.gn_gamma = gn_gamma; a.gn_beta = gn_beta; a.groups = groups;
    a.ln_gamma = ln_gamma; a.ln_beta = ln_beta; a.C = c; a.batch = batch; a.pix_per_sample = pix_per_sample;
    a.x0 = (const float*)x0; a.x1 = (const float*)x1; a.C0 = c0; a.C1 = c1; a.rc_w = rc_w_packed; a.rc_b = rc_bias;
    VDX_HIP(vdx::launch_resblock_tail(a, (hipStream_t)stream));
    return VDX_OK;
}

int vdx_gn_silu_apply_bf16(void* y, const double* stats, const float* gn_gamma, const float* gn_beta, const float* scale_shift,
                           int ss_stride, int groups, int c, int batch, long pix_per_sample, void* stream) {
    if (!y || !stats || !gn_gamma || !gn_beta) VDX_FAIL(VDX_ERR_INVALID, "gn_silu_apply: null tensor");
    if (batch < 1 || pix_per_sample < 1 || c < 8 || c % 8 || c > 1024 || groups <= 0 || groups > 32 || c % groups || (scale_shift && ss_stride < 2 * c))
        VDX_FAIL(VDX_ERR_INVALID, "gn_silu_apply: shape not served");
    VDX_HIP(vdx::launch_gn_silu_apply16((float*)y, stats, gn_gamma, gn_beta, scale_shift, ss_stride, groups, c, batch, pix_per_sample, (hipStream_t)stream));
    return VDX_OK;
}

int vdx_init_conv(const float* x, const float* kernel, const float* bias, float* y, int batch, int cin, int frames,
                  int h, int w, int cout, int k, void* stream) {
    if (!x || !kernel || !bias || !y) VDX_FAIL(VDX_ERR_INVALID, "init_conv: null tensor");
    if (k < 1 || k > 15 || !(k & 1) || cin < 1 || cin > 8) VDX_FAIL(VDX_ERR_INVALID, "init_conv: bad kernel size / channels");
    VDX_HIP(vdx::launch_init_conv(x, kernel, bias, y, batch, cin, frames, h, w, cout, k, 0, (hipStream_t)stream));
    return VDX_OK;
}

int vdx_final_conv(const float* x, const float* kernel, const float* bias, float* y, long npix, int d, int cout, void* stream) {
    if (!x || !kernel || !bias || !y || d % 4) VDX_FAIL(VDX_ERR_INVALID, "final_conv: bad argument");
    VDX_HIP(vdx::launch_final_conv(x, kernel, bias, y, npix, d, cout, 0, (hipStream_t)stream));
    return VDX_OK;
}

int vdx_time_mlp(const int* time, const float* w1, const float* b1, const float* w2, const float* b2, int dim,
                 const float* cond, const float* null_cond_emb, const unsigned char* cond_mask, int null_all, int cond_dim,
                 float* temb, int batch, void* stream) {
    if (!time || !w1 || !b1 || !w2 || !b2 || !temb || dim < 4 || (dim % 4)) VDX_FAIL(VDX_ERR_INVALID, "time_mlp: bad argument (dim must be a multiple of 4; Unet3D itself needs dim % 8 == 0)");
    if (cond_dim && (!cond || !null_cond_emb)) VDX_FAIL(VDX_ERR_INVALID, "time_mlp: cond missing");
    vdx::TimeMlpArgs a;
    memset(&a, 0, sizeof(a));
    a.time = time; a.w1 = w1; a.b1 = b1; a.w2 = w2; a.b2 = b2; a.dim = dim; a.time_dim = 4 * dim;
    a.cond = cond; a.null_cond_emb = null_cond_emb; a.cond_mask = cond_mask; a.null_all = null_all; a.cond_dim = cond_dim;
    a.temb = temb; a.temb_dim = 4 * dim + cond_dim;
    VDX_HIP(vdx::launch_time_mlp(a, batch, (hipStream_t)stream));
    return VDX_OK;
}

int vdx_attention_forward(int mode, const float* x, float* y, const void* wqkv_packed, const float* bqkv,
                          const void* wo_packed, const float* bo, int batch, int frames, int h, int w, int c, int heads,
                          int temporal, void* stream) {
    return vdx_attention_forward_ex(mode, x, y, wqkv_packed, bqkv, wo_packed, bo, batch, frames, h, w, c, heads, temporal, 0, stream);
}

int vdx_attention_forward_ex(int mode, const float* x, float* y, const void* wqkv_packed, const float* bqkv,
                             const void* wo_packed, const float* bo, int batch, int frames, int h, int w, int c, int heads,
                             int temporal, int fp8_core, void* stream) {
    if (fp8_core && mode != VDX_MODE_BF16) VDX_FAIL(VDX_ERR_INVALID, "attention: the fp8 core needs VDX_MODE_BF16");
    if (!x || !y || !wqkv_packed || !bqkv || !wo_packed || !bo) VDX_FAIL(VDX_ERR_INVALID, "attention: null tensor");
    if (mode != VDX_MODE_F32 && mode != VDX_MODE_BF16 && mode != VDX_MODE_F16) VDX_FAIL(VDX_ERR_INVALID, "bad mode");
    if (c % 4 || c > 1024 || heads < 1) VDX_FAIL(VDX_ERR_INVALID, "attention: C must be a multiple of 4 and <= 1024");
    vdx::AttnArgs a;
    memset(&a, 0, sizeof(a));
    a.x = x; a.y = y; a.wqkv = wqkv_packed; a.bqkv = bqkv; a.wo = wo_packed; a.bo = bo; a.C = c; a.heads = heads;
    a.scale = 1.0f / sqrtf(32.0f);
    const long hw = (long)h * w;
    if (temporal) {
        a.L = frames; a.nseq = (long)batch * hw; a.inner = hw; a.inner_stride = c; a.outer_stride = (long)frames * hw * c; a.tok_stride = hw * c;
    } else {
        a.L = (int)hw; a.nseq = (long)batch * frames; a.inner = 1; a.inner_stride = 0; a.outer_stride = hw * c; a.tok_stride = c;
    }
    if (a.L > 64) VDX_FAIL(VDX_ERR_INVALID, "attention: more than 64 tokens per sequence is not supported");
    a.fp8_core = fp8_core ? 1 : 0;
    VDX_HIP(vdx::launch_attention(mode, a, (hipStream_t)stream));
    return VDX_OK;
}

int vdx_attention_forward_bf16(const void* x_bf16, void* y_bf16, const void* wqkv_packed, const float* bqkv,
                               const void* wo_packed, const float* bo, int batch, int frames, int h, int w, int c, int heads,
                               int temporal, int fp8_core, void* stream) {
    if (!x_bf16 || !y_bf16 || !wqkv_packed || !bqkv || !wo_packed || !bo) VDX_FAIL(VDX_ERR_INVALID, "attention: null tensor");
    if (c % 8 || c > 1024 || heads < 1) VDX_FAIL(VDX_ERR_INVALID, "attention (bf16 tensors): C must be a multiple of 8 and <= 1024");
    vdx::AttnArgs a;
    memset(&a, 0, sizeof(a));
    a.x = reinterpret_cast<const float*>(x_bf16); a.y = reinterpret_cast<float*>(y_bf16); a.io_bf16 = 1;
    a.wqkv = wqkv_packed; a.bqkv = bqkv; a.wo = wo_packed; a.bo = bo; a.C = c; a.heads = heads;
    a.scale = 1.0f / sqrtf(32.0f);
    const long hw = (long)h * w;
    if (temporal) {
        a.L = frames; a.nseq = (long)batch * hw; a.inner = hw; a.inner_stride = c; a.outer_stride = (long)frames * hw * c; a.tok_stride = hw * c;
    } else {
        a.L = (int)hw; a.nseq = (long)batch * frames; a.inner = 1; a.inner_stride = 0; a.outer_stride = hw * c; a.tok_stride = c;
    }
    if (a.L > 64) VDX_FAIL(VDX_ERR_INVALID, "attention: more than 64 tokens per sequence is not supported");
    a.fp8_core = fp8_core ? 1 : 0;
    VDX_HIP(vdx::launch_attention(VDX_MODE_BF16, a, (hipStream_t)stream));
    return VDX_OK;
}

size_t vdx_sla_workspace_bytes(int mode, int nframes, int npix, int heads) { return vdx::sla_workspace_bytes(mode, nframes, npix, heads); }

int vdx_sla_forward(int mode, const float* x, float* y, const void* wq_packed, const void* wk_packed, const void* wv_packed,
                    const void* wo_packed, void* workspace, int batch, int frames, int h, int w, int c, int heads, void* stream) {
    if (!x || !y || !wq_packed || !wk_packed || !wv_packed || !wo_packed || !workspace) VDX_FAIL(VDX_ERR_INVALID, "sla: null tensor");
    if (mode != VDX_MODE_F32 && mode != VDX_MODE_BF16 && mode != VDX_MODE_F16) VDX_FAIL(VDX_ERR_INVALID, "bad mode");
    if (heads != 8 || c % 4 || c > 1024) VDX_FAIL(VDX_ERR_INVALID, "sla: needs 8 heads, C multiple of 4 and <= 1024");
    vdx::SlaArgs a;
    memset(&a, 0, sizeof(a));
    a.x = x; a.y = y; a.wq = wq_packed; a.wk = wk_packed; a.wv = wv_packed; a.wo = wo_packed; a.workspace = workspace;
    a.C = c; a.heads = heads; a.NF = batch * frames; a.N = h * w;
    VDX_HIP(vdx::launch_sla(mode, a, (hipStream_t)stream));
    return VDX_OK;
}

int vdx_sla_forward_bf16(const void* x_bf16, void* y_bf16, const void* wq_packed, const void* wk_packed, const void* wv_packed,
                         const void* wo_packed, void* workspace, int batch, int frames, int h, int w, int c, int heads, void* stream) {
    if (!x_bf16 || !y_bf16 || !wq_packed || !wk_packed || !wv_packed || !wo_packed || !workspace) VDX_FAIL(VDX_ERR_INVALID, "sla: null tensor");
    if (heads != 8 || c % 8 || c > 1024) VDX_FAIL(VDX_ERR_INVALID, "sla (bf16 tensors): needs 8 heads, C multiple of 8 and <= 1024");
    vdx::SlaArgs a;
    memset(&a, 0, sizeof(a));
    a.x = reinterpret_cast<const float*>(x_bf16); a.y = reinterpret_cast<float*>(y_bf16); a.io_bf16 = 1;
    a.wq = wq_packed; a.wk = wk_packed; a.wv = wv_packed; a.wo = wo_packed; a.workspace = workspace;
    a.C = c; a.heads = heads; a.NF = batch * frames; a.N = h * w;
    VDX_HIP(vdx::launch_sla(VDX_MODE_BF16, a, (hipStream_t)stream));
    return VDX_OK;
}

int vdx_create(const vdx_config* cfg, vdx_handle** out) {
    if (!cfg || !out) VDX_FAIL(VDX_ERR_INVALID, "create: null argument");
    if (cfg->mode != VDX_MODE_F32 && cfg->mode != VDX_MODE_BF16 && cfg->mode != VDX_MODE_F16) VDX_FAIL(VDX_ERR_INVALID, "bad mode");
    vdx_handle* h = new vdx_handle();
    h->model.cfg = *cfg;
    int rc = vdx::model_build(&h->model);
    if (rc != VDX_OK) { delete h; return rc; }
    const size_t tb = h->model.ss_layers.size() * sizeof(vdx::SsLayer);
    if (tb) {
        int ndev = 0;
        if (hipGetDeviceCount(&ndev) == hipSuccess && ndev > 0) {
            hipError_t e = hipMalloc(reinterpret_cast<void**>(&h->model.d_ss_layers), tb);
            if (e == hipSuccess) e = hipMemcpy(h->model.d_ss_layers, h->model.ss_layers.data(), tb, hipMemcpyHostToDevice);
            if (e != hipSuccess) { delete h; return vdx_set_error(VDX_ERR_HIP, hipGetErrorString(e), __FILE__, __LINE__); }
            vdx::model_build_pack_tables(&h->model);
            for (int k = 0; k < 2 && e == hipSuccess; ++k) {
                const std::vector<vdx::PackJob>& v = k ? h->model.pack_t_jobs : h->model.pack_jobs;
                vdx::PackJob** d = k ? &h->model.d_pack_t_jobs : &h->model.d_pack_jobs;
                e = hipMalloc(reinterpret_cast<void**>(d), v.size() * sizeof(vdx::PackJob));
                if (e == hipSuccess) e = hipMemcpy(*d, v.data(), v.size() * sizeof(vdx::PackJob), hipMemcpyHostToDevice);
            }
            if (e != hipSuccess) { vdx_destroy(h); return vdx_set_error(VDX_ERR_HIP, hipGetErrorString(e), __FILE__, __LINE__); }
        }
    }
    *out = h;
    return VDX_OK;
}

void vdx_destroy(vdx_handle* h) {
    if (!h) return;
    h->drop_graphs();
    vdx::comm_destroy(&h->comm);
    vdx::bwd_state_free(&h->bwd);
    if (h->model.d_ss_layers) (void)hipFree(h->model.d_ss_layers);
    if (h->model.d_pack_jobs) (void)hipFree(h->model.d_pack_jobs);
    if (h->model.d_pack_t_jobs) (void)hipFree(h->model.d_pack_t_jobs);
    delete h;
}

int vdx_set_activation_storage(vdx_handle* h, int bf16) {
    if (!h) VDX_FAIL(VDX_ERR_INVALID, "set_activation_storage: null handle");
    if (bf16 && h->model.mode != VDX_MODE_BF16) VDX_FAIL(VDX_ERR_INVALID, "bf16 activation storage needs a VDX_MODE_BF16 handle");
    if (bf16 < 0 || bf16 > 2) VDX_FAIL(VDX_ERR_INVALID, "set_activation_storage: 0 (fp32), 1 (bf16, inference) or 2 (bf16, training forward)");
    const int v = bf16;
    if (v != h->model.act16) {
        h->drop_graphs();
        h->model.act16 = v;
    }
    return VDX_OK;
}
int vdx_get_activation_storage(const vdx_handle* h) { return h ? h->model.act16 : 0; }

int vdx_set_attention_fp8(vdx_handle* h, int on) {
    if (!h) VDX_FAIL(VDX_ERR_INVALID, "set_attention_fp8: null handle");
    if (on && h->model.mode != VDX_MODE_BF16) VDX_FAIL(VDX_ERR_INVALID, "fp8 attention needs a VDX_MODE_BF16 handle");
    const int v = on ? 1 : 0;
    if (v != h->model.attn_fp8) { h->drop_graphs(); h->model.attn_fp8 = v; }
    return VDX_OK;
}
int vdx_get_attention_fp8(const vdx_handle* h) { return h ? h->model.attn_fp8 : 0; }

int vdx_param_count(const vdx_handle* h) { return h ? (int)h->model.params.size() : 0; }
long vdx_param_total(const vdx_handle* h) { return h ? h->model.param_total : 0; }

int vdx_param_info(const vdx_handle* h, int index, char* name, int name_cap, int* ndim, long shape[6], long* offset) {
    if (!h || index < 0 || index >= (int)h->model.params.size()) VDX_FAIL(VDX_ERR_INVALID, "param_info: bad index");
    const vdx::ParamInfo& p = h->model.params[index];
    if (name && name_cap > 0) snprintf(name, name_cap, "%s", p.name.c_str());
    if (ndim) *ndim = p.ndim;
    if (shape) for (int i = 0; i < 6; ++i) shape[i] = i < p.ndim ? p.shape[i] : 1;
    if (offset) *offset = p.offset;
    return VDX_OK;
}

size_t vdx_packed_bytes(const vdx_handle* h) { return h ? h->model.packed_bytes : 0; }

int vdx_pack_params(const vdx_handle* h, const float* params, void* packed, void* stream) {
    if (!h || !params || !packed) VDX_FAIL(VDX_ERR_INVALID, "pack_params: null argument");
    VDX_HIP(vdx::model_pack(&h->model, params, packed, (hipStream_t)stream));
    return VDX_OK;
}

size_t vdx_workspace_bytes(const vdx_handle* h, int batch) { return h ? vdx::model_workspace_bytes(&h->model, batch) : 0; }
int vdx_slot_count(const vdx_handle* h) { return h ? (int)h->model.slots.size() : 0; }

int vdx_slot_info(const vdx_handle* h, int index, char* name, int name_cap, long* floats_per_sample, long* float_offset_per_sample) {
    if (!h || index < 0 || index >= (int)h->model.slots.size()) VDX_FAIL(VDX_ERR_INVALID, "slot_info: bad index");
    const vdx::Slot& s = h->model.slots[index];
    if (name && name_cap > 0) snprintf(name, name_cap, "%s", s.name.c_str());
    if (floats_per_sample) *floats_per_sample = s.floats_per_sample;
    if (float_offset_per_sample) *float_offset_per_sample = s.offset_per_sample;
    return VDX_OK;
}

int vdx_unet_forward(const vdx_handle* h, const float* params, const void* packed, const float* x, const int* time,
                     const float* cond, const unsigned char* cond_mask, int null_all, float* out, void* workspace,
                     size_t workspace_bytes, int batch, void* stream) {
    if (!h || !params || !packed || !x || !time || !out || !workspace) VDX_FAIL(VDX_ERR_INVALID, "unet_forward: null argument");
    if (!h->model.d_ss_layers) VDX_FAIL(VDX_ERR_STATE, "unet_forward: handle was created without a GPU");
    return vdx::model_forward(&h->model, params, packed, x, time, cond, cond_mask, null_all, out, workspace, workspace_bytes, batch,
                              (hipStream_t)stream);
}

int vdx_randn(float* out, long n, uint64_t seed, uint64_t offset, const uint64_t* dev_offset, void* stream) {
    if (n == 0) return VDX_OK;
    if (!out || n < 0) VDX_FAIL(VDX_ERR_INVALID, "randn: bad argument");
    VDX_HIP(vdx::launch_randn(out, n, seed, offset, reinterpret_cast<const unsigned long long*>(dev_offset), (hipStream_t)stream));
    return VDX_OK;
}

int vdx_q_sample(const float* x_start, const int* t, const float* noise, float* out, const float* sqrt_ac,
                 const float* sqrt_one_minus_ac, int batch, long per_sample, float pre_scale, float pre_shift, void* stream) {
    if (!x_start || !t || !noise || !out || !sqrt_ac || !sqrt_one_minus_ac || batch < 1 || per_sample < 1) VDX_FAIL(VDX_ERR_INVALID, "q_sample: bad argument");
    if (per_sample % 4) VDX_FAIL(VDX_ERR_INVALID, "q_sample: per_sample must be a multiple of 4");
    VDX_HIP(vdx::launch_q_sample(x_start, t, noise, out, sqrt_ac, sqrt_one_minus_ac, batch, per_sample, pre_scale, pre_shift, (hipStream_t)stream));
    return VDX_OK;
}

static int fill_psample(vdx::PSampleArgs& a, const float* x, const float* eps_hat, float* out, const int* t, const float* tables,
                        int timesteps, const float* noise, uint64_t seed, uint64_t offset, const uint64_t* dev_offset,
                        const float* thres, int clip, int channels, long per_sample) {
    memset(&a, 0, sizeof(a));
    a.x = x; a.eps = eps_hat; a.out = out; a.t = t; a.tables = tables; a.T = timesteps; a.noise = noise;
    a.seed = seed; a.offset = offset; a.dev_offset = reinterpret_cast<const unsigned long long*>(dev_offset);
    a.thres = thres; a.clip = clip; a.C = channels; a.per_sample = per_sample; a.post_scale = 1.f; a.post_shift = 0.f;
    return 0;
}

int vdx_p_sample_step(const float* x, const float* eps_hat, float* out, const int* t, const float* tables, int timesteps,
                      const float* noise, uint64_t seed, uint64_t offset, const uint64_t* dev_offset, const float* thres,
                      int clip_denoised, int batch, int channels, long per_sample, void* stream) {
    if (!x || !eps_hat || !out || !t || !tables || timesteps < 1 || batch < 1 || channels < 1) VDX_FAIL(VDX_ERR_INVALID, "p_sample: bad argument");
    if (per_sample % channels) VDX_FAIL(VDX_ERR_INVALID, "p_sample: per_sample must be a multiple of channels");
    if (!noise && per_sample % 4) VDX_FAIL(VDX_ERR_INVALID, "p_sample: generated noise needs per_sample % 4 == 0");
    vdx::PSampleArgs a;
    fill_psample(a, x, eps_hat, out, t, tables, timesteps, noise, seed, offset, dev_offset, thres, clip_denoised, channels, per_sample);
    VDX_HIP(vdx::launch_p_sample(a, batch, (hipStream_t)stream));
    return VDX_OK;
}

int vdx_loss_sum(const float* eps_hat, const float* noise, double* acc, int batch, int channels, long fhw, int l2, void* stream) {
    if (!eps_hat || !noise || !acc) VDX_FAIL(VDX_ERR_INVALID, "loss: null tensor");
    VDX_HIP(vdx::launch_loss(eps_hat, noise, acc, batch, channels, fhw, l2, (hipStream_t)stream));
    return VDX_OK;
}

int vdx_affine(const float* x, float* y, long n, float a, float b, void* stream) {
    if (!x || !y || n < 0) VDX_FAIL(VDX_ERR_INVALID, "affine: bad argument");
    if (n) VDX_HIP(vdx::launch_affine(x, y, n, a, b, (hipStream_t)stream));
// ... 559 lines not shown
```

video_diffusion_nnx_amd/csrc/vdx_common.h:

```cpp
#pragma once
#include <hip/hip_runtime.h>
#include <stdint.h>

namespace vdx {

enum { MODE_F32 = 0, MODE_BF16 = 1, MODE_F16 = 2 };

typedef float f32x4 __attribute__((ext_vector_type(4)));
typedef float f32x2 __attribute__((ext_vector_type(2)));
typedef __bf16 bf16x8 __attribute__((ext_vector_type(8)));
typedef __bf16 bf16x2 __attribute__((ext_vector_type(2)));
typedef short s16x4 __attribute__((ext_vector_type(4)));

constexpr int CHUNK_BYTES = 64;
constexpr int ROW_BYTES = 128;
constexpr int ROW_STRIDE = 160;
constexpr float NORM_EPS = 1e-6f;
constexpr int GN_SLOTS = 32;

__device__ __forceinline__ unsigned pack_bf16x2(float a, float b) {
    f32x2 v = {a, b};
    bf16x2 r = __builtin_convertvector(v, bf16x2);
    return __builtin_bit_cast(unsigned, r);
}

__device__ __forceinline__ float silu_f(float x) { return x * __builtin_amdgcn_rcpf(1.0f + __expf(-x)); }

template <int MODE> struct Mma;

template <> struct Mma<MODE_F32> {
    static constexpr int ES = 4;
    static constexpr int KC = 16;
    static constexpr int KT = 32;
    static __device__ __forceinline__ void mma(f32x4& acc, const uint4& a, const uint4& b) {
        acc = __builtin_amdgcn_mfma_f32_16x16x4f32(__uint_as_float(a.x), __uint_as_float(b.x), acc, 0, 0, 0);
        acc = __builtin_amdgcn_mfma_f32_16x16x4f32(__uint_as_float(a.y), __uint_as_float(b.y), acc, 0, 0, 0);
        acc = __builtin_amdgcn_mfma_f32_16x16x4f32(__uint_as_float(a.z), __uint_as_float(b.z), acc, 0, 0, 0);
        acc = __builtin_amdgcn_mfma_f32_16x16x4f32(__uint_as_float(a.w), __uint_as_float(b.w), acc, 0, 0, 0);
    }
    static __device__ __forceinline__ void mma16(f32x4& acc, const f32x4& a, const f32x4& b) {
        acc = __builtin_amdgcn_mfma_f32_16x16x4f32(a[0], b[0], acc, 0, 0, 0);
        acc = __builtin_amdgcn_mfma_f32_16x16x4f32(a[1], b[1], acc, 0, 0, 0);
        acc = __builtin_amdgcn_mfma_f32_16x16x4f32(a[2], b[2], acc, 0, 0, 0);
        acc = __builtin_amdgcn_mfma_f32_16x16x4f32(a[3], b[3], acc, 0, 0, 0);
    }
    static __device__ __forceinline__ f32x4 load_w4(const char* p) {
        const float4 v = *reinterpret_cast<const float4*>(p);
        return f32x4{v.x, v.y, v.z, v.w};
    }
    static __device__ __forceinline__ void store4(char* row, int k, float4 v) {
        *reinterpret_cast<float4*>(row + k * 4) = v;
    }
    static __device__ __forceinline__ void store1(char* row, int k, float v) {
        *reinterpret_cast<float*>(row + k * 4) = v;
    }
};

template <> struct Mma<MODE_BF16> {
    static constexpr int ES = 2;
    static constexpr int KC = 32;
    static constexpr int KT = 64;
    static __device__ __forceinline__ void mma(f32x4& acc, const uint4& a, const uint4& b) {
        acc = __builtin_amdgcn_mfma_f32_16x16x32_bf16(__builtin_bit_cast(bf16x8, a), __builtin_bit_cast(bf16x8, b), acc, 0, 0, 0);
    }
    static __device__ __forceinline__ void mma16(f32x4& acc, const f32x4& a, const f32x4& b) {
        const uint2 ua = make_uint2(pack_bf16x2(a[0], a[1]), pack_bf16x2(a[2], a[3]));
        const uint2 ub = make_uint2(pack_bf16x2(b[0], b[1]), pack_bf16x2(b[2], b[3]));
        acc = __builtin_amdgcn_mfma_f32_16x16x16bf16_1k(__builtin_bit_cast(s16x4, ua), __builtin_bit_cast(s16x4, ub), acc, 0, 0, 0);
    }
    static __device__ __forceinline__ void mma16_fp8(f32x4& acc, const f32x4& a, const f32x4& b) {
        int ua = __builtin_amdgcn_cvt_pk_fp8_f32(a[0], a[1], 0, false); ua = __builtin_amdgcn_cvt_pk_fp8_f32(a[2], a[3], ua, true);
        int ub = __builtin_amdgcn_cvt_pk_fp8_f32(b[0], b[1], 0, false); ub = __builtin_amdgcn_cvt_pk_fp8_f32(b[2], b[3], ub, true);
        acc = __builtin_amdgcn_mfma_f32_16x16x32_fp8_fp8((long)(unsigned)ua, (long)(unsigned)ub, acc, 0, 0, 0);
    }
    static __device__ __forceinline__ f32x4 load_w4(const char* p) {
        const uint2 u = *reinterpret_cast<const uint2*>(p);
        return f32x4{__uint_as_float(u.x << 16), __uint_as_float(u.x & 0xFFFF0000u), __uint_as_float(u.y << 16), __uint_as_float(u.y & 0xFFFF0000u)};
    }
    static __device__ __forceinline__ void store4(char* row, int k, float4 v) {
        uint2 u;
        u.x = pack_bf16x2(v.x, v.y);
        u.y = pack_bf16x2(v.z, v.w);
        *reinterpret_cast<uint2*>(row + k * 2) = u;
    }
    static __device__ __forceinline__ void store1(char* row, int k, float v) {
        __bf16 h = (__bf16)v;
        *reinterpret_cast<__bf16*>(row + k * 2) = h;
    }
};

typedef _Float16 f16x8 __attribute__((ext_vector_type(8)));
typedef _Float16 f16x4 __attribute__((ext_vector_type(4)));
typedef _Float16 f16x2 __attribute__((ext_vector_type(2)));

__device__ __forceinline__ unsigned pack_f16x2(float a, float b) {
    f32x2 v = {a, b};
    f16x2 r = __builtin_convertvector(v, f16x2);
    return __builtin_bit_cast(unsigned, r);
}

template <> struct Mma<MODE_F16> {
    static constexpr int ES = 2;
    static constexpr int KC = 32;
    static constexpr int KT = 64;
    static __device__ __forceinline__ void mma(f32x4& acc, const uint4& a, const uint4& b) {
        acc = __builtin_amdgcn_mfma_f32_16x16x32_f16(__builtin_bit_cast(f16x8, a), __builtin_bit_cast(f16x8, b), acc, 0, 0, 0);
    }
    static __device__ __forceinline__ void mma16(f32x4& acc, const f32x4& a, const f32x4& b) {
        const uint2 ua = make_uint2(pack_f16x2(a[0], a[1]), pack_f16x2(a[2], a[3]));
        const uint2 ub = make_uint2(pack_f16x2(b[0], b[1]), pack_f16x2(b[2], b[3]));
        acc = __builtin_amdgcn_mfma_f32_16x16x16f16(__builtin_bit_cast(f16x4, ua), __builtin_bit_cast(f16x4, ub), acc, 0, 0, 0);
    }
    static __device__ __forceinline__ f32x4 load_w4(const char* p) {
        const f16x4 h = *reinterpret_cast<const f16x4*>(p);
        return f32x4{(float)h[0], (float)h[1], (float)h[2], (float)h[3]};
    }
    static __device__ __forceinline__ void store4(char* row, int k, float4 v) {
        *reinterpret_cast<uint2*>(row + k * 2) = make_uint2(pack_f16x2(v.x, v.y), pack_f16x2(v.z, v.w));
    }
    static __device__ __forceinline__ void store1(char* row, int k, float v) {
        *reinterpret_cast<_Float16*>(row + k * 2) = (_Float16)v;
    }
};

template <class M, bool F8> __device__ __forceinline__ void core_mma16(f32x4& acc, const f32x4& a, const f32x4& b) {
    if constexpr (F8) M::mma16_fp8(acc, a, b); else M::mma16(acc, a, b);
}

template <int MODE> __device__ __forceinline__ void store_operand(void* dst, size_t i, float v) {
    if (MODE == MODE_F32) reinterpret_cast<float*>(dst)[i] = v;
    else if (MODE == MODE_BF16) reinterpret_cast<__bf16*>(dst)[i] = (__bf16)v;
    else reinterpret_cast<_Float16*>(dst)[i] = (_Float16)v;
}

__device__ __forceinline__ float4 load4_f32_or_bf16(const float* base, size_t i, int is_bf16) {
    if (!is_bf16) return *reinterpret_cast<const float4*>(base + i);
    const uint2 u = *reinterpret_cast<const uint2*>(reinterpret_cast<const char*>(base) + i * 2);
    return make_float4(__uint_as_float(u.x << 16), __uint_as_float(u.x & 0xFFFF0000u), __uint_as_float(u.y << 16), __uint_as_float(u.y & 0xFFFF0000u));
}

__device__ __forceinline__ void store4_f32_or_bf16(float* base, size_t i, float4 v, int is_bf16) {
    if (!is_bf16) *reinterpret_cast<float4*>(base + i) = v;
    else *reinterpret_cast<uint2*>(reinterpret_cast<char*>(base) + i * 2) = make_uint2(pack_bf16x2(v.x, v.y), pack_bf16x2(v.z, v.w));
}

template <int CTRL>
__device__ __forceinline__ float dpp_row(float v) {
    return __uint_as_float(__builtin_amdgcn_update_dpp(0u, __float_as_uint(v), CTRL, 0xF, 0xF, true));
}
__device__ __forceinline__ float reduce16(float v) {
    v += dpp_row<0xB1>(v);
    v += dpp_row<0x4E>(v);
    v += dpp_row<0x141>(v);
    v += dpp_row<0x140>(v);
    return v;
}
__device__ __forceinline__ float reduce_q(float v) {
    const auto a = __builtin_amdgcn_permlane32_swap(__float_as_uint(v), __float_as_uint(v), false, false);
    v = __uint_as_float(a[0]) + __uint_as_float(a[1]);
    const auto b = __builtin_amdgcn_permlane16_swap(__float_as_uint(v), __float_as_uint(v), false, false);
    return __uint_as_float(b[0]) + __uint_as_float(b[1]);
}
__device__ __forceinline__ float max_q(float v) {
    const auto a = __builtin_amdgcn_permlane32_swap(__float_as_uint(v), __float_as_uint(v), false, false);
    v = fmaxf(__uint_as_float(a[0]), __uint_as_float(a[1]));
    const auto b = __builtin_amdgcn_permlane16_swap(__float_as_uint(v), __float_as_uint(v), false, false);
    return fmaxf(__uint_as_float(b[0]), __uint_as_float(b[1]));
}
__device__ __forceinline__ float max16(float v) {
    v = fmaxf(v, dpp_row<0xB1>(v));
    v = fmaxf(v, dpp_row<0x4E>(v));
    v = fmaxf(v, dpp_row<0x141>(v));
    v = fmaxf(v, dpp_row<0x140>(v));
    return v;
}
__device__ __forceinline__ int div_magic(int n, unsigned m) { return (int)__umulhi((unsigned)n, m); }

__device__ __forceinline__ void gn_mean_rstd(const double* stats, int b, int g, int groups, double count,
                                             float& mean, float& rstd) {
    double s = 0.0, ss = 0.0;
    const double* p = stats + (size_t)b * GN_SLOTS * groups * 2 + g * 2;
    static_assert(GN_SLOTS % 8 == 0, "GN_SLOTS");
#pragma unroll 1
    for (int k0 = 0; k0 < GN_SLOTS; k0 += 8) {
        double2 t[8];
#pragma unroll
        for (int k = 0; k < 8; ++k) t[k] = *reinterpret_cast<const double2*>(p + (size_t)(k0 + k) * groups * 2);
#pragma unroll
        for (int k = 0; k < 8; ++k) { s += t[k].x; ss += t[k].y; }
    }
    double m = s / count;
    double var = ss / count - m * m;
    if (var < 0.0) var = 0.0;
    mean = (float)m;
    rstd = (float)(1.0 / sqrt(var + (double)NORM_EPS));
}

__device__ __forceinline__ void gn_mean_rstd_wg(const double* stats, int b, int groups, double count, float* gm, int tid, int nthreads) {
    static_assert(GN_SLOTS == 32, "GN_SLOTS");
    for (int t = tid; t < groups * GN_SLOTS; t += nthreads) {
        const int g = t >> 5, slot = t & 31;
        const double2 v = *reinterpret_cast<const double2*>(stats + (((size_t)b * GN_SLOTS + slot) * groups + g) * 2);
        double s = v.x, ss = v.y;
#pragma unroll
        for (int o = 16; o >= 1; o >>= 1) { s += __shfl_xor(s, o); ss += __shfl_xor(ss, o); }
        if (slot == 0) {
            const double m = s / count;
            double var = ss / count - m * m;
            if (var < 0.0) var = 0.0;
            gm[2 * g] = (float)m;
            gm[2 * g + 1] = (float)(1.0 / sqrt(var + (double)NORM_EPS));
        }
    }
}

}

#define VDX_CHECK_HIP(expr)                                                      \
    do {                                                                         \
        hipError_t _e = (expr);                                                  \
        if (_e != hipSuccess) return vdx_set_error(VDX_ERR_HIP, hipGetErrorString(_e), __FILE__, __LINE__); \
    } while (0)
```

video_diffusion_nnx_amd/csrc/vdx_internal.h:

```cpp
#pragma once
#include <hip/hip_runtime.h>
#include <stdarg.h>
#include <stddef.h>
#include <stdio.h>
#include <algorithm>
#include "../../include/vdx.h"

int vdx_set_error(int code, const char* msg, const char* file, int line);

namespace vdx {

extern vdx_launch_hook g_launch_hook;
extern void* g_launch_hook_user;
struct LaunchScope {
    vdx_launch_info info; char desc[192]; hipStream_t st; bool on;
    LaunchScope(hipStream_t s, const char* kernel, double flops, double bytes, const char* fmt, ...) __attribute__((format(printf, 6, 7))) : st(s), on(g_launch_hook != nullptr) {
        if (!on) return;
        va_list ap;
        va_start(ap, fmt);
        vsnprintf(desc, sizeof(desc), fmt, ap);
        va_end(ap);
        info.kernel = kernel; info.shape = desc; info.flops = flops; info.bytes = bytes;
        g_launch_hook(g_launch_hook_user, 0, &info, st);
    }
    ~LaunchScope() { if (on && g_launch_hook) g_launch_hook(g_launch_hook_user, 1, &info, st); }
    LaunchScope(const LaunchScope&) = delete;
    LaunchScope& operator=(const LaunchScope&) = delete;
};

inline int device_cus() {
    int dev = 0, cus = 256;
    if (hipGetDevice(&dev) == hipSuccess) { int v = 0; if (hipDeviceGetAttribute(&v, hipDeviceAttributeMultiprocessorCount, dev) == hipSuccess && v > 0) cus = v; }
    return cus;
}

struct PersistentSplit { long per, workers; };
inline PersistentSplit persistent_split(long total, long slots) {
    const long n = std::min(total, slots);
    const long per = (total + n - 1) / n;
    return {per, (total + per - 1) / per};
}

template <typename K>
inline hipError_t lds_opt_in(K kfn, size_t lds) {
    if (lds <= 64 * 1024) return hipSuccess;
    return hipFuncSetAttribute(reinterpret_cast<const void*>(kfn), hipFuncAttributeMaxDynamicSharedMemorySize, (int)lds);
}

struct ConvArgs {
    const float* x0; const float* x1; int C0, C1;
    const void* wp;
    const float* bias;
    float* y; int Cout;
    int NF, F;
    int H, W;
    int kind;
    int kh, kw, stride, pad;
    int pro;
    const double* in_stats; const float* gamma; const float* beta; int groups;
    const float* ss; int ss_stride;
    double* out_stats; int out_groups;
    int x0_bf16, y_bf16;
    int x1_bf16;
    const float* res;
    int res_bf16;
    int wrows, wrow0;
    int Ho, Wo, Hy, Wy, CinPad, PH, PW, NP, tiles_y, tiles_x;
    unsigned x0_bytes, x1_bytes, w_bytes;
    unsigned m_ihiw, m_iw, m_phpw, m_pw;
};

struct TailArgs {
    const float* y2; const float* r; float* out;
    int y2_bf16;
    int r_bf16, out_bf16;
    const double* stats; const float* gn_gamma; const float* gn_beta; int groups;
    const float* ln_gamma; const float* ln_beta;
    int C; int batch; long pix_per_sample;
    int lpp;
    const float* x0; const float* x1; int C0, C1;
    const void* rc_w;
    const float* rc_b;
    const float* fin_w; const float* fin_b; float* fin_out;
};
bool tail_rc16_supported(int cin, int c0, int cout, long pix_per_sample);

struct TimeMlpArgs {
    const int* time; int t_is_device_scalar;
    const float* w1; const float* b1; const float* w2; const float* b2;
    int dim, time_dim;
    const float* cond; const float* null_cond_emb; const unsigned char* cond_mask; int null_all; int cond_dim;
    float* temb; int temb_dim;
};

struct SsLayer { long w_off, b_off, g_off, be_off, out_off; int n; int pad_; };

hipError_t launch_resblock_tail(TailArgs a, hipStream_t st);
hipError_t launch_init_conv(const float* x, const float* w, const float* bias, float* y, int B, int Cin, int F, int H, int W,
                            int Cout, int K, int y_bf16, hipStream_t st);
hipError_t launch_init_conv_mode(int mode, const float* x, const float* w, const float* bias, float* y, int B, int Cin, int F, int H, int W,
                                 int Cout, int K, int y_bf16, hipStream_t st);
hipError_t launch_final_conv(const float* x, const float* w, const float* bias, float* y, long npix, int D, int Cout, int x_bf16, hipStream_t st);
hipError_t launch_time_mlp(const TimeMlpArgs& a, int B, hipStream_t st);
hipError_t launch_resblock_ss(const float* params, const float* temb, const SsLayer* layers, int nlayers, float* ss_base,
                              float* lin_base, int temb_dim, int B, int max_n, hipStream_t st);

struct AttnArgs {
    const float* x; float* y;
    const void* wqkv; const float* bqkv;
    const void* wo; const float* bo;
    int C, heads, L;
    long nseq, inner, inner_stride, outer_stride, tok_stride;
    float scale;
    int io_bf16;
    int fp8_core;
    void* oscratch;
    int CPad, HDPad;
};
hipError_t launch_attention(int mode, AttnArgs a, hipStream_t st);
hipError_t launch_attention_heads(AttnArgs a, hipStream_t st);
hipError_t launch_attention_long_core(const float* qkv, float* o, long nseq, int L, int heads, float scale, hipStream_t st);

struct SlaArgs {
    const float* x; float* y;
    const void* wq; const void* wk; const void* wv;
    const void* wo;
    void* workspace;
    int C, heads, NF, N;
    int io_bf16;
    int CPad, nsub, nchunk; float* part; void* ctxT;
};
size_t sla_workspace_bytes(int mode, int NF, int N, int heads);
hipError_t launch_sla(int mode, SlaArgs a, hipStream_t st);
hipError_t launch_sla_heads(SlaArgs a, void* O, hipStream_t st);

struct PSampleArgs {
    const float* x; const float* eps; float* out;
    const int* t; const float* tables; int T;
    const float* noise;
    unsigned long long seed, offset; const unsigned long long* dev_offset;
    const float* thres;
    int clip; int C; long per_sample;
    float post_scale, post_shift;
};
hipError_t launch_randn(float* out, long n, unsigned long long seed, unsigned long long offset, const unsigned long long* dev_offset, hipStream_t st);
hipError_t launch_q_sample(const float* x0, const int* t, const float* noise, float* out, const float* sqrt_ac, const float* sqrt_1mac,
                           int B, long per_sample, float pre_scale, float pre_shift, hipStream_t st);
hipError_t launch_p_sample(const PSampleArgs& a, int B, hipStream_t st);
hipError_t launch_advance(int* t, int B, unsigned long long* dev_offset, hipStream_t st);
struct MaskArgs {
    const float* known; const unsigned char* mask;
    const float* mtab;
    int U;
    unsigned long long step; const unsigned long long* step_dev;
};
hipError_t launch_p_sample_masked(const PSampleArgs& a, const MaskArgs& m, int B, hipStream_t st);
hipError_t launch_resample_advance(int* t, int B, unsigned long long* step_dev, int U, hipStream_t st);
hipError_t launch_ddim_step_masked(const float* x, const float* eps, float* out, const float* ac, const int* seq, const unsigned long long* step_dev,
                                   const float* thres, int clip, int B, int C, long per_sample, const MaskArgs& m, int T, unsigned long long seed,
                                   hipStream_t st);
hipError_t launch_inpaint_init(float* x, const float* known, const unsigned char* mask, const float* mtab, int T, int t0, long n, hipStream_t st);
hipError_t launch_ddim_step(const float* x, const float* eps, float* out, const float* ac, const int* seq, const unsigned long long* step_dev,
                            const float* thres, int clip, int B, int C, long per_sample, hipStream_t st);
hipError_t launch_ddim_advance(int* t, int B, const int* seq, unsigned long long* step_dev, hipStream_t st);
hipError_t launch_dyn_thres(const float* x, const float* eps, const int* t, const float* tables, int T, float q, float* out, int B, int C,
                            long per_sample, hipStream_t st);
hipError_t launch_loss(const float* eps_hat, const float* noise, double* acc, int B, int Cc, long fhw, int l2, hipStream_t st);
hipError_t launch_affine(const float* x, float* y, long n, float a, float b, hipStream_t st);

hipError_t launch_loss_grad(const float* eps_hat, const float* noise, float* d_eps, int B, int Cc, long fhw, int l2, hipStream_t st);
hipError_t launch_adam_ema(float* p, const float* g, float* m, float* v, float* ema, long n, float lr, float b1, float b2, float eps,
                           long step_count, float grad_scale, int do_ema, float decay, hipStream_t st);

struct WgradArgs {
    const float* x0; const float* x1; int C0, C1;
    const float* dy; int Cout;
    float* dW;
    float* db;
    int NF, F, H, W;
    int kind, kh, kw, stride;
    int pro; const double* in_stats; const float* gamma; const float* beta; int groups; const float* ss; int ss_stride;
    int x0_bf16;
    int dy_bf16;
    int split; float* dW1; float* dW2; float* db1; float* db2;
    int bf16_mma;
    float* part; size_t part_cap;
    float* part_b; long part_E;
    int taps, sa, sb, ext, halo, Hm, Wm, Hy, Wy, PH, PW, co_tiles;
    unsigned m_iw, m_bw;
    int pwl;
};
hipError_t launch_conv_wgrad(WgradArgs a, hipStream_t st);
struct PackJob;
hipError_t launch_pack_jobs(int mode, const float* params, void* dst_base, const PackJob* d_jobs, int njobs, hipStream_t st);
hipError_t launch_colsum(const float* x, float* out, long rows, int C, hipStream_t st, float* part = nullptr, size_t part_cap = 0);
hipError_t launch_slot_sum(const float* part, int nslots, size_t slot_stride, long E, int Cout, int split, float* d0, float* d1, float* d2, hipStream_t st);
constexpr size_t WG_PART_FLOATS = (size_t)12 << 20;
hipError_t launch_add_inplace(float* y, const float* x, long n, hipStream_t st);

struct NormBwdArgs {
    const float* dact; const float* y; float* dy;
    int y_bf16;
    int dy_bf16;
    int r_bf16;
    const double* stats; const float* gamma; const float* beta; int groups;
    const float* ss; int ss_stride;
    float* d_gamma; float* d_beta;
    float* dss;
    const float* r; const float* ln_gamma; float* dr; float* d_ln_gamma; float* d_ln_beta;
    float* R; float* G;
    int nwg;
    float* dgp;
    int C, batch; long pix_per_sample;
    int lpp;
};
hipError_t launch_norm_bwd(NormBwdArgs a, hipStream_t st);
size_t norm_bwd_scratch_floats(int C, int batch, long pix_per_sample);

struct AttnBwdArgs {
    const float* qkv; const float* dO; float* O; float* dq; float* dk; float* dv;
    int heads, L; long nseq, inner, outer_p, tok_p; float scale;
    int dstride;
    int io_bf16;
    int bf16_mma;
};
hipError_t launch_attn_core_bwd(const AttnBwdArgs& a, hipStream_t st);
struct AttnBwdXArgs {
    const float* x; const float* g;
    int x_bf16;
    const void* wqkv; const float* bqkv;
    const void* woT;
    void* O; void* dqkv;
    float* dx;
    int L; long nseq, inner, outer_p, tok_p; float scale;
};
hipError_t launch_attn_bwd_fused(const AttnBwdXArgs& a, hipStream_t st);
struct SlaBwdArgs {
    const float* q; const float* k; const float* v; const float* dOut; float* O; float* dq; float* dk; float* dv; float* A;
    int NF, N, heads;
    int dstride;
    int io_bf16;
    int bf16_mma;
};
size_t sla_bwd_scratch_floats(int NF, int heads);
hipError_t launch_sla_bwd(const SlaBwdArgs& a, hipStream_t st);

hipError_t launch_final_conv_bwd(const float* x, const float* dout, const float* w, float* dx, float* dW, float* db, long npix, int D, int Cout, int x_bf16, hipStream_t st, float* part = nullptr, size_t part_cap = 0);
hipError_t launch_init_conv_wgrad(const float* x, const float* dy, float* dW, float* db, int B, int Cin, int F, int H, int W, int Cout, int K, hipStream_t st, float* part = nullptr, size_t part_cap = 0);
hipError_t launch_resblock_ss_bwd(const float* params, float* grads, const float* temb, const SsLayer* layers, int nlayers, const float* lin_base,
                                  float* dss_base, float* dtemb, int temb_dim, int B, hipStream_t st, float* part = nullptr, size_t part_cap = 0);
hipError_t launch_time_mlp_bwd(const TimeMlpArgs& a, const float* dtemb, float* dw1, float* db1, float* dw2, float* db2, float* dnull, int B, hipStream_t st);

size_t conv_packed_bytes(int mode, int taps, int Cin, int Cout);
int conv_cin_pad(int mode, int Cin);
hipError_t launch_pack_weights(int mode, const float* src, void* dst, int taps, int Cin, int Cout, hipStream_t st);
hipError_t launch_conv(int mode, ConvArgs a, hipStream_t st);
int conv3x3_ws_geo(const ConvArgs& a);
bool conv4x4_ws_eligible(int mode, const ConvArgs& a);
hipError_t launch_conv4x4_ws(const ConvArgs& a, hipStream_t st);
hipError_t launch_gn_silu_apply16(float* y_bf16, const double* stats, const float* gamma, const float* beta, const float* ss, int ss_stride, int groups,
                                  int C, int batch, long pix_per_sample, hipStream_t st);
bool resample32_eligible(int mode, const ConvArgs& a);
hipError_t launch_resample32(const ConvArgs& a, hipStream_t st);
bool conv1x1_pw_eligible(int mode, const ConvArgs& a);
hipError_t launch_conv1x1_pw(const ConvArgs& a, hipStream_t st);
int conv1x1_pw_rows(const ConvArgs& a);
bool conv3x3_ws_eligible(int mode, const ConvArgs& a);
hipError_t launch_conv3x3_ws(const ConvArgs& a, hipStream_t st);
hipError_t launch_pack_weights_t(int mode, const float* src, void* dst, int taps, int Cin, int Cout, hipStream_t st);

}
```

video_diffusion_nnx_amd/ops.py:

```python
from __future__ import annotations

import ctypes as C

import torch

from . import _lib as L


def _mode(mode) -> int:
    return L.MODES[mode] if isinstance(mode, str) else int(mode)


def pack_conv_weights(kernel: torch.Tensor, mode) -> torch.Tensor:
    m = _mode(mode)
    cin, cout = kernel.shape[-2], kernel.shape[-1]
    taps = kernel.numel() // (cin * cout)
    k = kernel.contiguous().float()
    n = L.vdx_packed_conv_bytes(m, taps, cin, cout)
    out = torch.empty(n, dtype=torch.uint8, device=k.device)
    L.check(L.vdx_pack_conv_weights(m, L.ptr(k), L.ptr(out), taps, cin, cout, L.stream_ptr()))
    return out


def gn_stats_zeros(batch: int, groups: int, device) -> torch.Tensor:
    return torch.zeros(batch * L.GN_SLOTS * groups * 2, dtype=torch.float64, device=device)


def gn_stats_reduce(stats: torch.Tensor, batch: int, groups: int) -> torch.Tensor:
    return stats.view(batch, L.GN_SLOTS, groups, 2).sum(1)


def conv_forward(x0, packed_w, cout, *, mode, bias=None, x1=None, kind=0, k=3, stride=1,
                 in_stats=None, gamma=None, beta=None, groups=8, scale_shift=None,
                 out_stats=None, out_groups=8, y_bf16=False, res=None) -> torch.Tensor:
    B, Fr, H, W, c0 = x0.shape
    c1 = 0 if x1 is None else x1.shape[-1]
    if kind == 1:
        Ho, Wo = 2 * H, 2 * W
    else:
        Ho, Wo = -(-H // stride), -(-W // stride)
    x_bf16 = x0.dtype == torch.bfloat16
    assert x0.dtype in (torch.float32, torch.bfloat16) and (x1 is None or x1.dtype == x0.dtype)
    y = torch.empty(B, Fr, Ho, Wo, cout, dtype=torch.bfloat16 if y_bf16 else torch.float32, device=x0.device)
    d = L.ConvDesc()
    d.x_bf16, d.y_bf16 = int(x_bf16), int(bool(y_bf16))
    d.x0, d.x1, d.c0, d.c1 = L.ptr(x0), L.ptr(x1), c0, c1
    d.packed_w, d.bias, d.y, d.cout = L.ptr(packed_w), L.ptr(bias), L.ptr(y), cout
    d.batch, d.frames, d.h, d.w = B, Fr, H, W
    d.kind, d.kh, d.kw, d.stride = kind, k, k, stride
    d.in_stats, d.gamma, d.beta, d.groups = L.ptr(in_stats), L.ptr(gamma), L.ptr(beta), groups
    d.scale_shift = L.ptr(scale_shift)
    d.scale_shift_stride = 0 if scale_shift is None else scale_shift.shape[-1]
    d.out_stats, d.out_groups = L.ptr(out_stats), out_groups
    d.res, d.res_bf16 = L.ptr(res), int(res is not None and res.dtype == torch.bfloat16)
    L.check(L.vdx_conv_forward(_mode(mode), C.byref(d), L.stream_ptr()))
    return y


def resblock_tail(y2, r, stats, gn_gamma, gn_beta, ln_gamma, ln_beta, groups=8):
    B, C = y2.shape[0], y2.shape[-1]
    pix = y2.numel() // (B * C)
    out = torch.empty_like(y2)
    L.check(L.vdx_resblock_tail(L.ptr(y2), L.ptr(r), L.ptr(out), L.ptr(stats), L.ptr(gn_gamma), L.ptr(gn_beta), groups,
                                L.ptr(ln_gamma), L.ptr(ln_beta), C, B, pix, L.stream_ptr()))
    return out


def resblock_tail_rc_bf16(y2, x0, x1, rc_kernel, rc_bias, stats, gn_gamma, gn_beta, ln_gamma, ln_beta, groups=8):
    B, C = y2.shape[0], y2.shape[-1]
    pix = y2.numel() // (B * C)
    c0, c1 = x0.shape[-1], (0 if x1 is None else x1.shape[-1])
    wp = rc_kernel.t().contiguous().to(torch.bfloat16)
    if (c0 + c1) % 64:
        wp = torch.nn.functional.pad(wp, (0, 64 - (c0 + c1) % 64)).contiguous()
    out = torch.empty_like(y2)
    L.check(L.vdx_resblock_tail_rc_bf16(L.ptr(y2), L.ptr(x0), None if x1 is None else L.ptr(x1), c0, c1, L.ptr(wp), L.ptr(rc_bias),
                                        L.ptr(out), L.ptr(stats), L.ptr(gn_gamma), L.ptr(gn_beta), groups, L.ptr(ln_gamma),
                                        L.ptr(ln_beta), C, B, pix, L.stream_ptr()))
    return out


def gn_silu_apply_bf16(y, stats, gn_gamma, gn_beta, scale_shift=None, groups=8):
    assert y.dtype == torch.bfloat16 and y.is_contiguous()
    B, C = y.shape[0], y.shape[-1]
    pix = y.numel() // (B * C)
    L.check(L.vdx_gn_silu_apply_bf16(L.ptr(y), L.ptr(stats), L.ptr(gn_gamma), L.ptr(gn_beta), None if scale_shift is None else L.ptr(scale_shift),
                                     0 if scale_shift is None else scale_shift.shape[-1], groups, C, B, pix, L.stream_ptr()))
    return y


def init_conv(x, kernel, bias):
    B, Cin, Fr, H, W = x.shape
    k, cout = kernel.shape[1], kernel.shape[-1]
    y = torch.empty(B, Fr, H, W, cout, dtype=torch.float32, device=x.device)
    L.check(L.vdx_init_conv(L.ptr(x), L.ptr(kernel.contiguous()), L.ptr(bias), L.ptr(y), B, Cin, Fr, H, W, cout, k, L.stream_ptr()))
    return y


def final_conv(x, kernel, bias):
    d, cout = kernel.shape[-2], kernel.shape[-1]
    npix = x.numel() // d
    y = torch.empty(*x.shape[:-1], cout, dtype=torch.float32, device=x.device)
    L.check(L.vdx_final_conv(L.ptr(x), L.ptr(kernel.contiguous()), L.ptr(bias), L.ptr(y), npix, d, cout, L.stream_ptr()))
    return y


def time_mlp(time, w1, b1, w2, b2, cond=None, null_cond_emb=None, cond_mask=None, null_all=False):
    B, dim = time.shape[0], w1.shape[0]
    cond_dim = 0 if cond is None else cond.shape[-1]
    temb = torch.empty(B, 4 * dim + cond_dim, dtype=torch.float32, device=w1.device)
    t32 = time.to(torch.int32).contiguous()
    cm = None if cond_mask is None else cond_mask.to(torch.uint8).contiguous()
    L.check(L.vdx_time_mlp(L.ptr(t32), L.ptr(w1), L.ptr(b1), L.ptr(w2), L.ptr(b2), dim, L.ptr(cond), L.ptr(null_cond_emb),
                           L.ptr(cm), int(null_all), cond_dim, L.ptr(temb), B, L.stream_ptr()))
    return temb


def pack_mha(pq, pk, pv, po, mode):
    C_ = pq[0].shape[0]
    wqkv = torch.cat([p[0].reshape(C_, -1) for p in (pq, pk, pv)], dim=1).contiguous()
    bqkv = torch.cat([p[1].reshape(-1) for p in (pq, pk, pv)]).contiguous()
    wo = po[0].reshape(-1, C_).contiguous()
    return pack_conv_weights(wqkv, mode), bqkv, pack_conv_weights(wo, mode), po[1].contiguous()


def attention_forward(x, packed, heads, temporal, mode, fp8_core=False):
    B, Fr, H, W, C_ = x.shape
    y = torch.empty_like(x)
    wqkv, bqkv, wo, bo = packed
    L.check(L.vdx_attention_forward_ex(_mode(mode), L.ptr(x), L.ptr(y), L.ptr(wqkv), L.ptr(bqkv), L.ptr(wo), L.ptr(bo),
                                       B, Fr, H, W, C_, heads, int(temporal), int(bool(fp8_core)), L.stream_ptr()))
    return y


def attention_forward_bf16(x, packed, heads, temporal, fp8_core=False):
    assert x.dtype == torch.bfloat16 and x.is_contiguous()
    B, Fr, H, W, C_ = x.shape
    y = torch.empty_like(x)
    wqkv, bqkv, wo, bo = packed
    L.check(L.vdx_attention_forward_bf16(L.ptr(x), L.ptr(y), L.ptr(wqkv), L.ptr(bqkv), L.ptr(wo), L.ptr(bo),
                                         B, Fr, H, W, C_, heads, int(temporal), int(bool(fp8_core)), L.stream_ptr()))
    return y


def sla_forward(x, wq, wk, wv, wo, heads, mode):
    B, Fr, H, W, C_ = x.shape
    m = _mode(mode)
    y = torch.empty_like(x)
    ws = torch.empty(L.vdx_sla_workspace_bytes(m, B * Fr, H * W, heads), dtype=torch.uint8, device=x.device)
    pk = [pack_conv_weights(t, mode) for t in (wq, wk, wv, wo)]
    L.check(L.vdx_sla_forward(m, L.ptr(x), L.ptr(y), L.ptr(pk[0]), L.ptr(pk[1]), L.ptr(pk[2]), L.ptr(pk[3]), L.ptr(ws),
                              B, Fr, H, W, C_, heads, L.stream_ptr()))
    return y


def sla_forward_bf16(x, wq, wk, wv, wo, heads=8):
    assert x.dtype == torch.bfloat16 and x.is_contiguous()
    B, Fr, H, W, C_ = x.shape
    m = _mode('bf16')
    y = torch.empty_like(x)
    ws = torch.empty(L.vdx_sla_workspace_bytes(m, B * Fr, H * W, heads), dtype=torch.uint8, device=x.device)
    pk = [pack_conv_weights(t, 'bf16') for t in (wq, wk, wv, wo)]
    L.check(L.vdx_sla_forward_bf16(L.ptr(x), L.ptr(y), L.ptr(pk[0]), L.ptr(pk[1]), L.ptr(pk[2]), L.ptr(pk[3]), L.ptr(ws),
                                   B, Fr, H, W, C_, heads, L.stream_ptr()))
    return y




class WgradDesc(C.Structure):
    _fields_ = [('x0', C.c_void_p), ('x1', C.c_void_p), ('c0', C.c_int), ('c1', C.c_int), ('dy', C.c_void_p), ('cout', C.c_int),
                ('dw', C.c_void_p), ('batch', C.c_int), ('frames', C.c_int), ('h', C.c_int), ('w', C.c_int),
                ('kind', C.c_int), ('kh', C.c_int), ('kw', C.c_int), ('stride', C.c_int),
                ('in_stats', C.c_void_p), ('gamma', C.c_void_p), ('beta', C.c_void_p), ('groups', C.c_int),
                ('scale_shift', C.c_void_p), ('scale_shift_stride', C.c_int), ('bf16_operands', C.c_int)]


_pack_t = L._sig('vdx_pack_conv_weights_t', C.c_int, [C.c_int, C.c_void_p, C.c_void_p, C.c_int, C.c_int, C.c_int, C.c_void_p])
_wgrad = L._sig('vdx_conv_backward_weights', C.c_int, [C.POINTER(WgradDesc), C.c_void_p])
_colsum = L._sig('vdx_colsum', C.c_int, [C.c_void_p, C.c_void_p, C.c_long, C.c_int, C.c_void_p])


def pack_conv_weights_t(kernel: torch.Tensor, mode) -> torch.Tensor:
    m = _mode(mode)
    cin, cout = kernel.shape[-2], kernel.shape[-1]
    taps = kernel.numel() // (cin * cout)
    k = kernel.contiguous().float()
    out = torch.empty(L.vdx_packed_conv_bytes(m, taps, cout, cin), dtype=torch.uint8, device=k.device)
    L.check(_pack_t(m, L.ptr(k), L.ptr(out), taps, cin, cout, L.stream_ptr()))
    return out


def conv_backward_weights(x0, dy, kshape, *, x1=None, kind=0, k=3, stride=1, in_stats=None, gamma=None, beta=None, groups=8,
                          scale_shift=None, dw=None, bf16_operands=False) -> torch.Tensor:
    B, Fr, H, W, c0 = x0.shape
    c1 = 0 if x1 is None else x1.shape[-1]
    cout = dy.shape[-1]
    if dw is None:
        dw = torch.zeros(kshape, dtype=torch.float32, device=x0.device)
    d = WgradDesc()
    d.x0, d.x1, d.c0, d.c1, d.dy, d.cout, d.dw = L.ptr(x0), L.ptr(x1), c0, c1, L.ptr(dy), cout, L.ptr(dw)
    d.batch, d.frames, d.h, d.w = B, Fr, H, W
    d.kind, d.kh, d.kw, d.stride = kind, k, k, stride
    d.in_stats, d.gamma, d.beta, d.groups = L.ptr(in_stats), L.ptr(gamma), L.ptr(beta), groups
    d.scale_shift = L.ptr(scale_shift)
    d.scale_shift_stride = 0 if scale_shift is None else scale_shift.shape[-1]
    d.bf16_operands = int(bool(bf16_operands))
    L.check(_wgrad(C.byref(d), L.stream_ptr()))
    return dw


def colsum(x: torch.Tensor) -> torch.Tensor:
    c = x.shape[-1]
    out = torch.zeros(c, dtype=torch.float32, device=x.device)
    L.check(_colsum(L.ptr(x), L.ptr(out), x.numel() // c, c, L.stream_ptr()))
    return out


_norm_bwd = L._sig('vdx_norm_act_backward', C.c_int, [C.c_void_p] * 6 + [C.c_int, C.c_void_p, C.c_int] + [C.c_void_p] * 9 + [C.c_int, C.c_int, C.c_long, C.c_void_p])


_norm_bwd_scr = L._sig('vdx_norm_act_backward_scratch_floats', C.c_size_t, [C.c_int, C.c_int, C.c_long])


def norm_act_backward(dact, y, stats, gamma, beta, groups=8, scale_shift=None, r=None, ln_gamma=None):
    B, Cc = y.shape[0], y.shape[-1]
    pix = y.numel() // (B * Cc)
    dev = y.device
    z = lambda *s: torch.zeros(*s, dtype=torch.float32, device=dev)
    out = dict(dy=torch.empty_like(y), d_gamma=z(Cc), d_beta=z(Cc), dss=z(B, 2 * Cc) if scale_shift is not None else None,
               dr=torch.empty_like(y) if r is not None else None, d_ln_gamma=z(Cc) if r is not None else None,
               d_ln_beta=z(Cc) if r is not None else None)
    scratch = torch.empty(_norm_bwd_scr(Cc, B, pix), dtype=torch.float32, device=dev)
    L.check(_norm_bwd(L.ptr(dact), L.ptr(y), L.ptr(out['dy']), L.ptr(stats), L.ptr(gamma), L.ptr(beta), groups, L.ptr(scale_shift),
                      0 if scale_shift is None else scale_shift.shape[-1], L.ptr(out['d_gamma']), L.ptr(out['d_beta']), L.ptr(out['dss']),
                      L.ptr(r), L.ptr(ln_gamma), L.ptr(out['dr']), L.ptr(out['d_ln_gamma']), L.ptr(out['d_ln_beta']), L.ptr(scratch),
                      Cc, B, pix, L.stream_ptr()))
    return out


_attn_core_bwd = L._sig('vdx_attention_core_backward_ex', C.c_int, [C.c_void_p] * 6 + [C.c_int] * 7 + [C.c_void_p])
_sla_scr = L._sig('vdx_sla_backward_scratch_floats', C.c_size_t, [C.c_int, C.c_int])
_sla_core_bwd = L._sig('vdx_sla_core_backward_ex', C.c_int, [C.c_void_p] * 9 + [C.c_int] * 4 + [C.c_void_p])


def attention_core_backward(qkv, d_o, B, Fr, H, W, heads, temporal, bf16_operands=False):
    outs = [torch.empty_like(d_o) for _ in range(4)]
    L.check(_attn_core_bwd(L.ptr(qkv), L.ptr(d_o), *[L.ptr(t) for t in outs], B, Fr, H, W, heads, int(temporal), int(bool(bf16_operands)),
                           L.stream_ptr()))
    return outs


_attn_bwd_fused = L._sig('vdx_temporal_attention_backward_fused', C.c_int, [C.c_void_p] * 8 + [C.c_int] * 4 + [C.c_void_p])


def temporal_attention_backward_fused(x, dy, wqkv, bqkv, wo):
    B, Fr, H, W, C_ = x.shape
    assert C_ == 64 and wqkv.shape == (64, 768) and wo.shape == (256, 64)
    pw = pack_conv_weights(wqkv, 'bf16')
    pwo_t = pack_conv_weights_t(wo, 'bf16')
    rows = B * Fr * H * W
    o = torch.empty(rows, 256, dtype=torch.bfloat16, device=x.device)
    dqkv = torch.empty(rows, 768, dtype=torch.bfloat16, device=x.device)
    dx = torch.empty_like(x)
    bq = bqkv.contiguous().float()
    L.check(_attn_bwd_fused(L.ptr(x), L.ptr(dy), L.ptr(pw), L.ptr(bq), L.ptr(pwo_t), L.ptr(o), L.ptr(dqkv), L.ptr(dx), B, Fr, H, W, L.stream_ptr()))
    return dx, o, dqkv


def sla_core_backward(q, k, v, d_out, nframes, npix, heads=8, bf16_operands=False):
    outs = [torch.empty_like(q) for _ in range(4)]
    scr = torch.empty(_sla_scr(nframes, heads), dtype=torch.float32, device=q.device)
    L.check(_sla_core_bwd(L.ptr(q), L.ptr(k), L.ptr(v), L.ptr(d_out), *[L.ptr(t) for t in outs], L.ptr(scr), nframes, npix, heads,
                          int(bool(bf16_operands)), L.stream_ptr()))
    return outs





class WgradExDesc(C.Structure):
    _fields_ = [('x0', C.c_void_p), ('x1', C.c_void_p), ('c0', C.c_int), ('c1', C.c_int), ('x_bf16', C.c_int),
                ('dy', C.c_void_p), ('cout', C.c_int), ('dy_bf16', C.c_int),
                ('dw', C.c_void_p), ('dw1', C.c_void_p), ('dw2', C.c_void_p), ('split', C.c_int),
                ('db', C.c_void_p), ('db1', C.c_void_p), ('db2', C.c_void_p),
                ('batch', C.c_int), ('frames', C.c_int), ('h', C.c_int), ('w', C.c_int),
                ('kind', C.c_int), ('kh', C.c_int), ('kw', C.c_int), ('stride', C.c_int),
                ('in_stats', C.c_void_p), ('gamma', C.c_void_p), ('beta', C.c_void_p), ('groups', C.c_int),
                ('scale_shift', C.c_void_p), ('scale_shift_stride', C.c_int), ('bf16_operands', C.c_int),
                ('scratch', C.c_void_p), ('scratch_floats', C.c_size_t)]


WG_PART_FLOATS = L._sig('vdx_wgrad_scratch_floats', C.c_size_t, [])()
_wgrad_ex = L._sig('vdx_conv_backward_weights_ex', C.c_int, [C.POINTER(WgradExDesc), C.c_void_p])
_slot_sum = L._sig('vdx_slot_sum', C.c_int, [C.c_void_p, C.c_int, C.c_size_t, C.c_long, C.c_int, C.c_int, C.c_void_p, C.c_void_p, C.c_void_p, C.c_void_p])
_norm_bwd_ex = L._sig('vdx_norm_act_backward_ex', C.c_int, [C.c_void_p, C.c_void_p, C.c_int, C.c_void_p, C.c_int, C.c_void_p, C.c_void_p, C.c_void_p, C.c_int,
                                                            C.c_void_p, C.c_int, C.c_void_p, C.c_void_p, C.c_void_p, C.c_void_p, C.c_int] + [C.c_void_p] * 6 +
                      [C.c_int, C.c_int, C.c_long, C.c_void_p])
_attn_core_bwd_io = L._sig('vdx_attention_core_backward_io', C.c_int, [C.c_void_p] * 4 + [C.c_int] * 9 + [C.c_void_p])
_attn_bwd_fused_ex = L._sig('vdx_temporal_attention_backward_fused_ex', C.c_int, [C.c_void_p, C.c_int] + [C.c_void_p] * 7 + [C.c_int] * 4 + [C.c_void_p])
_sla_core_bwd_io = L._sig('vdx_sla_core_backward_io', C.c_int, [C.c_void_p] * 6 + [C.c_int, C.c_int, C.c_void_p] + [C.c_int] * 4 + [C.c_void_p])
_conv_rows = L._sig('vdx_conv_forward_rows', C.c_int, [C.c_int, C.POINTER(L.ConvDesc), C.c_int, C.c_int, C.c_void_p])
_final_bwd = L._sig('vdx_final_conv_backward', C.c_int, [C.c_void_p, C.c_int] + [C.c_void_p] * 5 + [C.c_long, C.c_int, C.c_int, C.c_void_p, C.c_size_t, C.c_void_p])
_init_wgrad = L._sig('vdx_init_conv_backward_weights', C.c_int, [C.c_void_p] * 4 + [C.c_int] * 7 + [C.c_void_p, C.c_size_t, C.c_void_p])
_time_mlp_bwd = L._sig('vdx_time_mlp_backward', C.c_int, [C.c_void_p] * 5 + [C.c_int, C.c_void_p, C.c_int, C.c_int] + [C.c_void_p] * 6 + [C.c_int, C.c_void_p])


def _is16(t) -> int:
    assert t.dtype in (torch.float32, torch.bfloat16)
    return int(t.dtype == torch.bfloat16)


def conv_backward_weights_ex(x0, dy, kshape, *, x1=None, kind=0, k=3, stride=1, in_stats=None, gamma=None, beta=None, groups=8,
                             scale_shift=None, bf16_operands=True, split=0, bias=False, scratch=None):
    B, Fr, H, W, c0 = x0.shape
    c1 = 0 if x1 is None else x1.shape[-1]
    cout = dy.shape[-1]
    assert x1 is None or x1.dtype == x0.dtype
# ... 147 lines not shown
```

Baseline: 50.73 frames/s.

## Fuse resblock tail (GN+SiLU+residual LN) into SLA context kernel prologue

```diff
diff --git a/include/vdx.h b/include/vdx.h
--- a/include/vdx.h
+++ b/include/vdx.h
@@ -93,6 +93,11 @@
 int vdx_sla_forward_bf16(const void* x_bf16, void* y_bf16, const void* wq_packed, const void* wk_packed, const void* wv_packed,
                          const void* wo_packed, void* workspace, int batch, int frames, int h, int w, int c, int heads, void* stream);
 
+int vdx_resblock_tail_sla_bf16(const void* y2_bf16, const void* r_bf16, void* out_bf16, const double* stats, const float* gn_gamma,
+                               const float* gn_beta, int groups, const float* ln_gamma, const float* ln_beta, void* y_bf16,
+                               const void* wq_packed, const void* wk_packed, const void* wv_packed, const void* wo_packed, void* workspace,
+                               int batch, int frames, int h, int w, int c, int heads, int fuse, int* fused, void* stream);
+
 
 typedef struct {
     int dim;
diff --git a/video_diffusion_nnx_amd/_lib.py b/video_diffusion_nnx_amd/_lib.py
--- a/video_diffusion_nnx_amd/_lib.py
+++ b/video_diffusion_nnx_amd/_lib.py
@@ -85,4 +85,5 @@
 vdx_attention_forward_bf16 = _sig('vdx_attention_forward_bf16', c_int, [c_void_p] * 6 + [c_int] * 8 + [c_void_p])
 vdx_sla_forward_bf16 = _sig('vdx_sla_forward_bf16', c_int, [c_void_p] * 7 + [c_int] * 6 + [c_void_p])
 vdx_sla_workspace_bytes = _sig('vdx_sla_workspace_bytes', c_size_t, [c_int] * 4)
+vdx_resblock_tail_sla_bf16 = _sig('vdx_resblock_tail_sla_bf16', c_int, [c_void_p] * 6 + [c_int] + [c_void_p] * 8 + [c_int] * 7 + [c_void_p, c_void_p])
 vdx_sla_forward = _sig('vdx_sla_forward', c_int, [c_int] + [c_void_p] * 7 + [c_int] * 6 + [c_void_p])
diff --git a/video_diffusion_nnx_amd/csrc/elementwise.hip b/video_diffusion_nnx_amd/csrc/elementwise.hip
--- a/video_diffusion_nnx_amd/csrc/elementwise.hip
+++ b/video_diffusion_nnx_amd/csrc/elementwise.hip
@@ -62,12 +62,6 @@
     }
 }
 
-__device__ __forceinline__ void unpack8(const uint4& u, float (&f)[8]) {
-    f[0] = __uint_as_float(u.x << 16); f[1] = __uint_as_float(u.x & 0xFFFF0000u);
-    f[2] = __uint_as_float(u.y << 16); f[3] = __uint_as_float(u.y & 0xFFFF0000u);
-    f[4] = __uint_as_float(u.z << 16); f[5] = __uint_as_float(u.z & 0xFFFF0000u);
-    f[6] = __uint_as_float(u.w << 16); f[7] = __uint_as_float(u.w & 0xFFFF0000u);
-}
 
 template <int VPL>
 __global__ __launch_bounds__(256) void resblock_tail16_kernel(TailArgs P) {
diff --git a/video_diffusion_nnx_amd/csrc/model.hip b/video_diffusion_nnx_amd/csrc/model.hip
--- a/video_diffusion_nnx_amd/csrc/model.hip
+++ b/video_diffusion_nnx_amd/csrc/model.hip
@@ -339,7 +339,8 @@
 #define VDX_PREPASS_MIN_C 256
 #endif
 
-static hipError_t run_res(const Fwd& f, const ResP& r, const float* x0, int c0, const float* x1, int c1, int lvl, float* head_out = nullptr, bool* head_done = nullptr) {
+static hipError_t run_res(const Fwd& f, const ResP& r, const float* x0, int c0, const float* x1, int c1, int lvl, float* head_out = nullptr, bool* head_done = nullptr,
+                          TailArgs* defer_tail = nullptr) {
     const Model* m = f.m;
     const int G = m->cfg.resnet_groups;
     const int S = m->cfg.image_size >> lvl;
@@ -395,6 +396,7 @@
         t.fin_w = f.p + m->fin_w; t.fin_b = f.p + m->fin_b; t.fin_out = head_out;
         *head_done = true;
     }
+    if (defer_tail && !r.has_res && half && f.a16 && m->act16 == 1) { *defer_tail = t; return hipSuccess; }
     return launch_resblock_tail(t, f.st);
 }
 
@@ -447,7 +449,7 @@
     return launch_attention(m->mode, a, f.st);
 }
 
-static hipError_t run_sla(const Fwd& f, const SlaP& sp, const float* x, float* y, int lvl) {
+static hipError_t run_sla(const Fwd& f, const SlaP& sp, const float* x, float* y, int lvl, const TailArgs* tail = nullptr) {
     const Model* m = f.m;
     const int S = m->cfg.image_size >> lvl;
     SlaArgs a;
@@ -457,7 +459,9 @@
     a.io_bf16 = f.a16;
     if (m->mode == MODE_BF16 && a.heads == 8 && sp.C >= 256 && sp.C % 128 == 0 && a.N % 16 == 0 &&
         (size_t)96 * (sp.C * 2 + 32) <= 160 * 1024 && (size_t)m->cfg.num_frames * a.N * a.heads * 64 <= m->sla_ws_bytes_per_sample) {
-        hipError_t e = launch_sla_heads(a, f.sla_ws, f.st);
+        hipError_t e = tail ? launch_resblock_tail(*tail, f.st) : hipSuccess;
+        if (e != hipSuccess) return e;
+        e = launch_sla_heads(a, f.sla_ws, f.st);
         if (e != hipSuccess) return e;
         ConvArgs c;
         memset(&c, 0, sizeof(c));
@@ -467,7 +471,7 @@
         c.NF = a.NF; c.F = m->cfg.num_frames; c.H = S; c.W = S; c.kind = 0; c.kh = c.kw = 1; c.stride = 1; c.pad = 0;
         return launch_conv(m->mode, c, f.st);
     }
-    return launch_sla(m->mode, a, f.st);
+    return tail ? launch_tail_sla(m->mode, *tail, a, f.st) : launch_sla(m->mode, a, f.st);
 }
 
 static hipError_t run_resample(const Fwd& f, const Level& L, const float* x, float* y, int lvl_in, bool up) {
@@ -528,9 +532,11 @@
     for (int i = 0; i < nl; ++i) {
         const Level& L = m->downs[i];
         VDX_E(run_res(f, L.res0, cur, cur_c, nullptr, 0, i));
-        VDX_E(run_res(f, L.res1, f.slot(L.res0.s_out), L.cout, nullptr, 0, i));
+        TailArgs tl;
+        tl.out = nullptr;
+        VDX_E(run_res(f, L.res1, f.slot(L.res0.s_out), L.cout, nullptr, 0, i, nullptr, nullptr, L.has_sla ? &tl : nullptr));
         cur = f.slot(L.res1.s_out);
-        if (L.has_sla) { VDX_E(run_sla(f, L.sla, cur, f.slot(L.s_sla), i)); cur = f.slot(L.s_sla); }
+        if (L.has_sla) { VDX_E(run_sla(f, L.sla, cur, f.slot(L.s_sla), i, tl.out ? &tl : nullptr)); cur = f.slot(L.s_sla); }
         VDX_E(run_attn(f, L.attn, cur, f.slot(L.s_attn), i, true));
         cur = f.slot(L.s_attn); cur_c = L.cout;
         if (L.has_resample) { VDX_E(run_resample(f, L, cur, f.slot(L.s_rs), i, false)); cur = f.slot(L.s_rs); }
@@ -544,9 +550,11 @@
         const Level& L = m->ups[i];
         const Level& D = m->downs[nl - 1 - i];
         VDX_E(run_res(f, L.res0, cur, cur_c, f.slot(D.s_attn), D.cout, L.lvl));
-        VDX_E(run_res(f, L.res1, f.slot(L.res0.s_out), L.cout, nullptr, 0, L.lvl));
+        TailArgs tl;
+        tl.out = nullptr;
+        VDX_E(run_res(f, L.res1, f.slot(L.res0.s_out), L.cout, nullptr, 0, L.lvl, nullptr, nullptr, L.has_sla ? &tl : nullptr));
         cur = f.slot(L.res1.s_out);
-        if (L.has_sla) { VDX_E(run_sla(f, L.sla, cur, f.slot(L.s_sla), L.lvl)); cur = f.slot(L.s_sla); }
+        if (L.has_sla) { VDX_E(run_sla(f, L.sla, cur, f.slot(L.s_sla), L.lvl, tl.out ? &tl : nullptr)); cur = f.slot(L.s_sla); }
         VDX_E(run_attn(f, L.attn, cur, f.slot(L.s_attn), L.lvl, true));
         cur = f.slot(L.s_attn); cur_c = L.cout;
         if (L.has_resample) { VDX_E(run_resample(f, L, cur, f.slot(L.s_rs), L.lvl, true)); cur = f.slot(L.s_rs); }
diff --git a/video_diffusion_nnx_amd/csrc/sla.hip b/video_diffusion_nnx_amd/csrc/sla.hip
--- a/video_diffusion_nnx_amd/csrc/sla.hip
+++ b/video_diffusion_nnx_amd/csrc/sla.hip
@@ -1,5 +1,6 @@
 #include "vdx_common.h"
 #include "vdx_internal.h"
+#include "vdx_glds.h"
 #include <stdlib.h>
 
 namespace vdx {
@@ -351,6 +352,7 @@
     static constexpr int XP = 64 * APIECES * NKT / 512;
     static constexpr int PLANE = 64 * ROW_STRIDE;
     static constexpr int BUF = NKT * PLANE;
+    static constexpr bool WHOLE = false;
     float4 xpre[XP];
     __device__ __forceinline__ void fetch(const float* x, size_t xbase, int io_bf16, int r0, int N, int C, int tid) {
 #pragma unroll
@@ -365,6 +367,7 @@
             }
         }
     }
+    __device__ __forceinline__ void begin(int) {}
     __device__ __forceinline__ void put(char* xs, int tid) const {
 #pragma unroll
         for (int u = 0; u < XP; ++u) {
@@ -413,15 +416,13 @@
     }
 }
 
-template <int MODE, int NKT, bool IO16>
-__global__ __launch_bounds__(512) void sla_ctx8_kernel(const SlaArgs P) {
+template <int MODE, int NKT, class T>
+__device__ __forceinline__ void sla_ctx8_body(const SlaArgs& P, T& t, char* smem) {
     using M = Mma<MODE>;
-    using T = SlaTile<MODE, NKT, IO16>;
     constexpr int RS = ROW_STRIDE;
-    extern __shared__ __attribute__((aligned(16))) char smem[];
     const int tid = threadIdx.x, lane = tid & 63, h = tid >> 6;
     const int lp = lane & 15, q = lane >> 4;
-    const int n = blockIdx.x / P.nchunk, chunk = blockIdx.x % P.nchunk;
+    const int n = T::WHOLE ? blockIdx.x : blockIdx.x / P.nchunk, chunk = T::WHOLE ? 0 : blockIdx.x % P.nchunk;
     const int R = P.nsub * 64;
     const size_t xbase = (size_t)n * P.N * P.C;
 
@@ -440,8 +441,8 @@
 #pragma unroll
     for (int i = 0; i < 2; ++i) { cacc[i][0] = f32x4{0.f, 0.f, 0.f, 0.f}; cacc[i][1] = f32x4{0.f, 0.f, 0.f, 0.f}; }
 
-    T t;
     t.fetch(P.x, xbase, P.io_bf16, chunk * R, P.N, P.C, tid);
+    t.begin(tid);
     t.put(smem, tid);
     __syncthreads();
     for (int sub = 0; sub < P.nsub; ++sub) {
@@ -470,7 +471,7 @@
 #pragma unroll
                         for (int tm = 0; tm < 4; ++tm) M::mma(acc[tn][tm], xa[tn], wf[kt][ch][tm]);
                 }
-            if (r0 + 64 <= P.N) ctx8_softmax_step<true>(acc, m_run, s_run, cacc, 0);
+            if (T::WHOLE || r0 + 64 <= P.N) ctx8_softmax_step<true>(acc, m_run, s_run, cacc, 0);
             else ctx8_softmax_step<false>(acc, m_run, s_run, cacc, P.N - (r0 + hf * 32 + 4 * q));
 #pragma unroll
             for (int tn = 0; tn < 2; ++tn)
@@ -482,7 +483,7 @@
         if (more) t.put(smem + ((sub + 1) & 1) * T::BUF, tid);
         __syncthreads();
     }
-    if (P.nchunk == 1) {
+    if (T::WHOLE || P.nchunk == 1) {
         char* ct = reinterpret_cast<char*>(P.ctxT) + (size_t)(n * P.heads + h) * 32 * 32 * M::ES;
 #pragma unroll
         for (int dt = 0; dt < 2; ++dt) {
@@ -505,6 +506,98 @@
 #pragma unroll
         for (int dt = 0; dt < 2; ++dt) { part[1024 + dt * 16 + lp] = m_run[dt]; part[1056 + dt * 16 + lp] = s_run[dt]; }
     }
+}
+
+template <int MODE, int NKT, bool IO16>
+__global__ __launch_bounds__(512) void sla_ctx8_kernel(const SlaArgs P) {
+    extern __shared__ __attribute__((aligned(16))) char smem[];
+    SlaTile<MODE, NKT, IO16> t;
+    sla_ctx8_body<MODE, NKT>(P, t, smem);
+}
+
+template <int NKT>
+struct SlaTailTile {
+    static constexpr int C = 64 * NKT;
+    static constexpr int LPP = 8 * NKT;
+    static constexpr int PLANE = 64 * ROW_STRIDE;
+    static constexpr int BUF = NKT * PLANE;
+    static constexpr int STAGE = NKT * 2 * 8192;
+    static constexpr bool WHOLE = true;
+    const char* yb; const char* rb; char* ob;
+    char* stage;
+    const float* coef;
+    int r0f;
+    const TailArgs* Q; float* gm; int b;
+    __device__ __forceinline__ void fetch(const float*, size_t, int, int r0, int, int, int tid) {
+        r0f = r0;
+        const unsigned off = (unsigned)r0 * (C * 2) + tid * 16;
+        const unsigned dst = __builtin_amdgcn_readfirstlane(lds_addr(stage) + (tid >> 6) * 1024);
+#pragma unroll
+        for (int u = 0; u < NKT; ++u) {
+            glds16(yb + off + u * 8192, dst + (2 * u) * 8192);
+            glds16(rb + off + u * 8192, dst + (2 * u + 1) * 8192);
+        }
+    }
+    __device__ __forceinline__ void begin(int tid) {
+        float* cf = const_cast<float*>(coef);
+        gn_mean_rstd_wg(Q->stats, b, Q->groups, (double)Q->pix_per_sample * (C / Q->groups), gm, tid, 512);
+        __syncthreads();
+        if (tid < C) {
+            const int c = tid, g = c / (C / Q->groups);
+            const float a = gm[2 * g + 1] * Q->gn_gamma[c];
+            cf[c] = a;
+            cf[C + c] = Q->gn_beta[c] - gm[2 * g] * a;
+            cf[2 * C + c] = Q->ln_gamma[c];
+            cf[3 * C + c] = Q->ln_beta[c];
+        }
+        __syncthreads();
+    }
+    __device__ __forceinline__ void put(char* xs, int tid) const {
+        const int sub = tid % LPP, c = sub * 8;
+        const float invC = 1.0f / (float)C;
+        const unsigned off = (unsigned)r0f * (C * 2) + tid * 16;
+        __builtin_amdgcn_s_waitcnt(0x0F70);
+        asm volatile("" ::: "memory");
+#pragma unroll
+        for (int u = 0; u < NKT; ++u) {
+            float r[8];
+            float s = 0.f, ss = 0.f;
+            unpack8(*reinterpret_cast<const uint4*>(stage + (2 * u + 1) * 8192 + tid * 16), r);
+#pragma unroll
+            for (int k = 0; k < 8; ++k) { s += r[k]; ss += r[k] * r[k]; }
+            s += dpp_row<0xB1>(s); ss += dpp_row<0xB1>(ss);
+            s += dpp_row<0x4E>(s); ss += dpp_row<0x4E>(ss);
+            s += dpp_row<0x141>(s); ss += dpp_row<0x141>(ss);
+            if (LPP == 16) { s += dpp_row<0x140>(s); ss += dpp_row<0x140>(ss); }
+            const float mean = s * invC;
+            const float var = fmaxf(ss * invC - mean * mean, 0.f);
+            const float rstd = rsqrtf(var + NORM_EPS);
+            float y[8], o[8];
+            unpack8(*reinterpret_cast<const uint4*>(stage + (2 * u) * 8192 + tid * 16), y);
+#pragma unroll
+            for (int k = 0; k < 8; ++k)
+                o[k] = silu_f(fmaf(y[k], coef[c + k], coef[C + c + k])) + fmaf((r[k] - mean) * rstd, coef[2 * C + c + k], coef[3 * C + c + k]);
+            const uint4 v = make_uint4(pack_bf16x2(o[0], o[1]), pack_bf16x2(o[2], o[3]), pack_bf16x2(o[4], o[5]), pack_bf16x2(o[6], o[7]));
+            *reinterpret_cast<uint4*>(ob + off + u * 8192) = v;
+            *reinterpret_cast<uint4*>(xs + (sub >> 3) * PLANE + (tid / LPP + u * (512 / LPP)) * ROW_STRIDE + (sub & 7) * 16) = v;
+        }
+    }
+};
+
+template <int NKT>
+__global__ __launch_bounds__(512, NKT == 1 ? 4 : 2) void sla_tail_ctx8_kernel(const SlaArgs P, const TailArgs Q) {
+    using T = SlaTailTile<NKT>;
+    extern __shared__ __attribute__((aligned(16))) char smem[];
+    T t;
+    const size_t fbase = (size_t)blockIdx.x * P.N * T::C * 2;
+    t.yb = reinterpret_cast<const char*>(Q.y2) + fbase;
+    t.rb = reinterpret_cast<const char*>(Q.r) + fbase;
+    t.ob = reinterpret_cast<char*>(Q.out) + fbase;
+    t.stage = smem + 2 * T::BUF;
+    float* cf = reinterpret_cast<float*>(t.stage + T::STAGE);
+    t.coef = cf; t.gm = cf + 4 * T::C; t.Q = &Q;
+    t.b = (int)((long)blockIdx.x * P.N / Q.pix_per_sample);
+    sla_ctx8_body<MODE_BF16, NKT>(P, t, smem);
 }
 
 template <int MODE, int NKT, int TMO, int TNO, bool IO16>
@@ -1081,7 +1174,7 @@
 }
 
 template <int MODE, int NKT, int TMO, int TNO, bool IO16>
-static hipError_t launch_sla8_t(const SlaArgs& a, hipStream_t st) {
+static hipError_t launch_sla8_t(const SlaArgs& a, hipStream_t st, const TailArgs* tail = nullptr) {
     using M = Mma<MODE>;
     using T = SlaTile<MODE, NKT, IO16>;
     const size_t lds_ctx = 2 * (size_t)T::BUF;
@@ -1091,7 +1184,18 @@
     hipError_t e;
     if ((e = lds_opt_in(kc, lds_ctx)) != hipSuccess) return e;
     if ((e = lds_opt_in(ko, lds_out)) != hipSuccess) return e;
-    {
+    if (tail) {
+        if constexpr (MODE == MODE_BF16 && IO16 && TNO >= 2) {
+            const size_t lds_tail = lds_ctx + SlaTailTile<NKT>::STAGE + (size_t)(4 * 64 * NKT + 64) * 4;
+            auto kt = sla_tail_ctx8_kernel<NKT>;
+            if ((e = lds_opt_in(kt, lds_tail)) != hipSuccess) return e;
+            const SlaWork sw = sla_work(a, M::ES, true, false, false);
+            const double el = (double)a.NF * a.N * a.C;
+            LaunchScope ls(st, "sla_tail_ctx8_kernel", sw.flops + 10.0 * el, sw.bytes + 2.0 * el * 2, "<%d> C%d N%d NF%d", NKT, a.C, a.N, a.NF);
+            hipLaunchKernelGGL(kt, dim3(a.NF), dim3(512), lds_tail, st, a, *tail);
+            if ((e = hipGetLastError()) != hipSuccess) return e;
+        } else return hipErrorInvalidValue;
+    } else {
         const SlaWork sw = sla_work(a, M::ES, true, false, false);
         LaunchScope ls(st, "sla_ctx8_kernel", sw.flops, sw.bytes, "<%d, %d, %d> C%d N%d NF%d nchunk%d", MODE, NKT, (int)IO16, a.C, a.N, a.NF, a.nchunk);
         hipLaunchKernelGGL(kc, dim3(a.NF * a.nchunk), dim3(512), lds_ctx, st, a);
@@ -1111,21 +1215,23 @@
     return hipGetLastError();
 }
 
+static void sla_plan_launch(SlaArgs& a) {
+    sla_plan(a.N, a.nsub, a.nchunk);
+    const int tiles = (a.N + 63) / 64;
+#ifndef VDX_SLA_MIN_WGS
+#define VDX_SLA_MIN_WGS 1024
+#endif
+    const long min_wgs = VDX_SLA_MIN_WGS;
+    while (a.nsub * 2 <= tiles && (long)a.NF * ((tiles + 2 * a.nsub - 1) / (2 * a.nsub)) >= min_wgs) a.nsub *= 2;
+    a.nchunk = (tiles + a.nsub - 1) / a.nsub;
+}
+
 template <int MODE>
-static hipError_t launch_sla_m(SlaArgs a, hipStream_t st) {
+static hipError_t launch_sla_m(SlaArgs a, hipStream_t st, const TailArgs* tail = nullptr) {
     using M = Mma<MODE>;
     constexpr int NCHN = 64 / M::KC;
     constexpr int RSE = NCHN * 64 + 16;
-    sla_plan(a.N, a.nsub, a.nchunk);
-    {
-        const int tiles = (a.N + 63) / 64;
-#ifndef VDX_SLA_MIN_WGS
-#define VDX_SLA_MIN_WGS 1024
-#endif
-        const long min_wgs = VDX_SLA_MIN_WGS;
-        while (a.nsub * 2 <= tiles && (long)a.NF * ((tiles + 2 * a.nsub - 1) / (2 * a.nsub)) >= min_wgs) a.nsub *= 2;
-        a.nchunk = (tiles + a.nsub - 1) / a.nsub;
-    }
+    sla_plan_launch(a);
     const size_t part_bytes = (((size_t)a.NF * a.nchunk * a.heads * SLA_PART * 4) + 255) / 256 * 256;
     a.part = reinterpret_cast<float*>(a.workspace);
     a.ctxT = reinterpret_cast<char*>(a.workspace) + part_bytes;
@@ -1133,14 +1239,15 @@
     if constexpr (MODE != MODE_F16)
     if (a.heads == 8 && (a.C % 64 == 0 || a.C == 32)) {
         if constexpr (MODE == MODE_BF16) {
-            if (a.io_bf16 && a.C == 64) return launch_sla8_t<MODE, 1, 1, 2, true>(a, st);
-            if (a.io_bf16 && a.C == 128) return launch_sla8_t<MODE, 2, 1, 4, true>(a, st);
+            if (a.io_bf16 && a.C == 64) return launch_sla8_t<MODE, 1, 1, 2, true>(a, st, tail);
+            if (a.io_bf16 && a.C == 128) return launch_sla8_t<MODE, 2, 1, 4, true>(a, st, tail);
             if (a.io_bf16 && a.C == 32) return launch_sla8_t<MODE, 1, 1, 1, true>(a, st);
         }
         if (nkt == 1 && a.C == 64) return launch_sla8_t<MODE, 1, 1, 2, false>(a, st);
         if (nkt == 2 && a.C == 64) return launch_sla8_t<MODE, 2, 1, 2, false>(a, st);
         if (nkt == 2 && a.C == 128) return launch_sla8_t<MODE, 2, 1, 4, false>(a, st);
     }
+    if (tail) return hipErrorInvalidValue;
     const size_t lds1 = 1024 + (size_t)128 * ROW_STRIDE + (size_t)64 * RSE;
     hipError_t e;
     {
@@ -1162,6 +1269,22 @@
     return hipErrorInvalidValue;
 }
 
+bool tail_sla_fused(int mode, const TailArgs& t, SlaArgs a) {
+    if (mode != MODE_BF16 || !a.io_bf16 || !t.y2_bf16 || !t.r_bf16 || !t.out_bf16 || t.rc_w || t.fin_out) return false;
+    if (t.out != a.x || t.C != a.C || a.heads != 8 || (a.C != 64 && a.C != 128) || a.N % 64) return false;
+    if (t.groups <= 0 || t.groups > 32 || a.C % t.groups) return false;
+    if (t.pix_per_sample % a.N || (long)t.batch * t.pix_per_sample != (long)a.NF * a.N || (size_t)a.N * a.C * 2 >= (1ull << 31)) return false;
+    sla_plan_launch(a);
+    return a.nchunk == 1;
+}
+
+hipError_t launch_tail_sla(int mode, const TailArgs& t, SlaArgs a, hipStream_t st) {
+    a.CPad = conv_cin_pad(mode, a.C);
+    if (tail_sla_fused(mode, t, a)) return launch_sla_m<MODE_BF16>(a, st, &t);
+    if (hipError_t e = launch_resblock_tail(t, st); e != hipSuccess) return e;
+    return launch_sla(mode, a, st);
+}
+
 hipError_t launch_sla(int mode, SlaArgs a, hipStream_t st) {
     a.CPad = conv_cin_pad(mode, a.C);
     return mode == MODE_F32 ? launch_sla_m<MODE_F32>(a, st) : mode == MODE_F16 ? launch_sla_m<MODE_F16>(a, st) : launch_sla_m<MODE_BF16>(a, st);
diff --git a/video_diffusion_nnx_amd/csrc/vdx_api.cpp b/video_diffusion_nnx_amd/csrc/vdx_api.cpp
--- a/video_diffusion_nnx_amd/csrc/vdx_api.cpp
+++ b/video_diffusion_nnx_amd/csrc/vdx_api.cpp
@@ -283,6 +283,31 @@
     a.x = reinterpret_cast<const float*>(x_bf16); a.y = reinterpret_cast<float*>(y_bf16); a.io_bf16 = 1;
     a.wq = wq_packed; a.wk = wk_packed; a.wv = wv_packed; a.wo = wo_packed; a.workspace = workspace;
     a.C = c; a.heads = heads; a.NF = batch * frames; a.N = h * w;
+    VDX_HIP(vdx::launch_sla(VDX_MODE_BF16, a, (hipStream_t)stream));
+    return VDX_OK;
+}
+
+int vdx_resblock_tail_sla_bf16(const void* y2_bf16, const void* r_bf16, void* out_bf16, const double* stats, const float* gn_gamma,
+                               const float* gn_beta, int groups, const float* ln_gamma, const float* ln_beta, void* y_bf16,
+                               const void* wq_packed, const void* wk_packed, const void* wv_packed, const void* wo_packed, void* workspace,
+                               int batch, int frames, int h, int w, int c, int heads, int fuse, int* fused, void* stream) {
+    if (!y2_bf16 || !r_bf16 || !out_bf16 || !stats || !gn_gamma || !gn_beta || !ln_gamma || !ln_beta) VDX_FAIL(VDX_ERR_INVALID, "tail_sla: null tensor");
+    if (!y_bf16 || !wq_packed || !wk_packed || !wv_packed || !wo_packed || !workspace) VDX_FAIL(VDX_ERR_INVALID, "tail_sla: null tensor");
+    if (batch < 1 || frames < 1 || h < 1 || w < 1 || heads != 8 || c % 8 || c > 1024 || groups <= 0 || groups > 32 || c % groups)
+        VDX_FAIL(VDX_ERR_INVALID, "tail_sla: needs 8 heads, C multiple of 8 and of groups, <= 1024");
+    vdx::TailArgs t;
+    memset(&t, 0, sizeof(t));
+    t.y2 = (const float*)y2_bf16; t.r = (const float*)r_bf16; t.out = (float*)out_bf16; t.y2_bf16 = t.r_bf16 = t.out_bf16 = 1;
+    t.stats = stats; t.gn_gamma = gn_gamma; t.gn_beta = gn_beta; t.groups = groups; t.ln_gamma = ln_gamma; t.ln_beta = ln_beta;
+    t.C = c; t.batch = batch; t.pix_per_sample = (long)frames * h * w;
+    vdx::SlaArgs a;
+    memset(&a, 0, sizeof(a));
+    a.x = (const float*)out_bf16; a.y = (float*)y_bf16; a.io_bf16 = 1;
+    a.wq = wq_packed; a.wk = wk_packed; a.wv = wv_packed; a.wo = wo_packed; a.workspace = workspace;
+    a.C = c; a.heads = heads; a.NF = batch * frames; a.N = h * w;
+    if (fused) *fused = (fuse && vdx::tail_sla_fused(VDX_MODE_BF16, t, a)) ? 1 : 0;
+    if (fuse) { VDX_HIP(vdx::launch_tail_sla(VDX_MODE_BF16, t, a, (hipStream_t)stream)); return VDX_OK; }
+    VDX_HIP(vdx::launch_resblock_tail(t, (hipStream_t)stream));
     VDX_HIP(vdx::launch_sla(VDX_MODE_BF16, a, (hipStream_t)stream));
     return VDX_OK;
 }
diff --git a/video_diffusion_nnx_amd/csrc/vdx_common.h b/video_diffusion_nnx_amd/csrc/vdx_common.h
--- a/video_diffusion_nnx_amd/csrc/vdx_common.h
+++ b/video_diffusion_nnx_amd/csrc/vdx_common.h
@@ -137,6 +137,13 @@
     if (!is_bf16) return *reinterpret_cast<const float4*>(base + i);
     const uint2 u = *reinterpret_cast<const uint2*>(reinterpret_cast<const char*>(base) + i * 2);
     return make_float4(__uint_as_float(u.x << 16), __uint_as_float(u.x & 0xFFFF0000u), __uint_as_float(u.y << 16), __uint_as_float(u.y & 0xFFFF0000u));
+}
+
+__device__ __forceinline__ void unpack8(const uint4& u, float (&f)[8]) {
+    f[0] = __uint_as_float(u.x << 16); f[1] = __uint_as_float(u.x & 0xFFFF0000u);
+    f[2] = __uint_as_float(u.y << 16); f[3] = __uint_as_float(u.y & 0xFFFF0000u);
+    f[4] = __uint_as_float(u.z << 16); f[5] = __uint_as_float(u.z & 0xFFFF0000u);
+    f[6] = __uint_as_float(u.w << 16); f[7] = __uint_as_float(u.w & 0xFFFF0000u);
 }
 
 __device__ __forceinline__ void store4_f32_or_bf16(float* base, size_t i, float4 v, int is_bf16) {
diff --git a/video_diffusion_nnx_amd/csrc/vdx_internal.h b/video_diffusion_nnx_amd/csrc/vdx_internal.h
--- a/video_diffusion_nnx_amd/csrc/vdx_internal.h
+++ b/video_diffusion_nnx_amd/csrc/vdx_internal.h
@@ -132,6 +132,8 @@
 };
 size_t sla_workspace_bytes(int mode, int NF, int N, int heads);
 hipError_t launch_sla(int mode, SlaArgs a, hipStream_t st);
+bool tail_sla_fused(int mode, const TailArgs& t, SlaArgs a);
+hipError_t launch_tail_sla(int mode, const TailArgs& t, SlaArgs a, hipStream_t st);
 hipError_t launch_sla_heads(SlaArgs a, void* O, hipStream_t st);
 
 struct PSampleArgs {
diff --git a/video_diffusion_nnx_amd/ops.py b/video_diffusion_nnx_amd/ops.py
--- a/video_diffusion_nnx_amd/ops.py
+++ b/video_diffusion_nnx_amd/ops.py
@@ -164,6 +164,20 @@
     L.check(L.vdx_sla_forward_bf16(L.ptr(x), L.ptr(y), L.ptr(pk[0]), L.ptr(pk[1]), L.ptr(pk[2]), L.ptr(pk[3]), L.ptr(ws),
                                    B, Fr, H, W, C_, heads, L.stream_ptr()))
     return y
+
+
+def resblock_tail_sla_bf16(y2, r, stats, gn_gamma, gn_beta, ln_gamma, ln_beta, wq, wk, wv, wo, groups=8, heads=8, fuse=True):
+    assert y2.dtype == torch.bfloat16 and r.dtype == torch.bfloat16 and y2.is_contiguous() and r.is_contiguous() and y2.shape == r.shape
+    B, Fr, H, W, C_ = y2.shape
+    m = _mode('bf16')
+    out, y = torch.empty_like(y2), torch.empty_like(y2)
+    ws = torch.empty(L.vdx_sla_workspace_bytes(m, B * Fr, H * W, heads), dtype=torch.uint8, device=y2.device)
+    pk = [pack_conv_weights(t, 'bf16') for t in (wq, wk, wv, wo)]
+    fused = C.c_int(0)
+    L.check(L.vdx_resblock_tail_sla_bf16(L.ptr(y2), L.ptr(r), L.ptr(out), L.ptr(stats), L.ptr(gn_gamma), L.ptr(gn_beta), groups, L.ptr(ln_gamma),
+                                         L.ptr(ln_beta), L.ptr(y), L.ptr(pk[0]), L.ptr(pk[1]), L.ptr(pk[2]), L.ptr(pk[3]), L.ptr(ws),
+                                         B, Fr, H, W, C_, heads, int(bool(fuse)), C.addressof(fused), L.stream_ptr()))
+    return out, y, bool(fused.value)
 
 
 
```

Result: no change. 50.50 frames/s, median of 2 (-0.5%).
